# danihae/bio-image-unet

Measured on AMD Instinct MI355X. Metric: voxels/sec fwd+bwd, higher is better.
Workload: dtype bf16; 1 GPU; cfg4: UNet3D(in_channels=1, out_channels=1, n_filter=32) input (4, 1, 128, 128, 128) per GPU, train step = forward + reference loss + backward + Adam; parallelism=dp1

## Files before the change

### bio_image_unet_amd/_lib.py

```python
from __future__ import annotations

import ctypes as C
import os

import torch

_HERE = os.path.dirname(os.path.abspath(__file__))
LIB_PATH = os.environ.get("BIU_LIB_PATH") or os.path.join(_HERE, "libbiu_hip.so")

BIU_F32, BIU_BF16 = 0, 1
BN_MAX_PARTIALS = 1024


class BiuError(RuntimeError):
    pass


class biu_act(C.Structure):
    _fields_ = [("p", C.c_void_p), ("n", C.c_int32), ("d", C.c_int32), ("h", C.c_int32), ("w", C.c_int32),
                ("c", C.c_int32), ("pitch", C.c_int32)]


class biu_pack_job(C.Structure):
    _fields_ = [("w", C.c_void_p), ("packed", C.c_void_p), ("transposed", C.c_int32), ("kind", C.c_int32), ("cin", C.c_int32),
                ("cout", C.c_int32), ("kd", C.c_int32), ("kh", C.c_int32), ("kw", C.c_int32), ("reserved", C.c_int32)]


class biu_xform(C.Structure):
    _fields_ = [("scale", C.c_void_p), ("shift", C.c_void_p), ("slope", C.c_void_p)]


class biu_mo2d_term(C.Structure):
    _fields_ = [("kind", C.c_int32), ("nb", C.c_int32), ("partial_off", C.c_longlong), ("numel", C.c_longlong), ("pixels", C.c_longlong),
                ("p0", C.c_float), ("p1", C.c_float), ("p2", C.c_float), ("weight", C.c_float)]


class biu_aug_params(C.Structure):
    _fields_ = [("flags", C.c_uint32), ("rot_k", C.c_uint32), ("blur_k", C.c_uint32), ("index", C.c_uint32), ("m", C.c_double * 6),
                ("alpha", C.c_float), ("beta", C.c_float), ("noise_a", C.c_float), ("noise_b", C.c_float),
                ("angle", C.c_float), ("scale", C.c_float), ("dx", C.c_float), ("dy", C.c_float)]


class biu_augf_params(C.Structure):
    _fields_ = [("flags", C.c_uint32), ("rot_k", C.c_uint32), ("blur_k", C.c_uint32), ("index", C.c_uint32), ("m", C.c_double * 6),
                ("cos_t", C.c_float), ("sin_t", C.c_float), ("alpha", C.c_float), ("beta", C.c_float), ("shot_s", C.c_float),
                ("gauss_sigma", C.c_float), ("angle", C.c_float), ("scale", C.c_float), ("dx", C.c_float), ("dy", C.c_float)]


_P = C.c_void_p
_A = C.POINTER(biu_act)
_X = C.POINTER(biu_xform)
_I = C.c_int
_F = C.c_float
_D = C.c_double
_Z = C.c_size_t

SIGNATURES = {
    "biu_last_error": (C.c_char_p, []),
    "biu_version": (_I, []),
    "biu_set_fp32_products": (_I, [_I]),
    "biu_set_fp32_products_3d": (_I, [_I]),
    "biu_conv_packed_bytes": (_Z, [_I, _I, _I, _I, _I, _I, _I, _I]),
    "biu_conv_pack": (_I, [_I, _P, _I, _I, _I, _I, _I, _I, _P, _P]),
    "biu_pack_batch": (_I, [_P, _I, _I, _P]),
    "biu_conv_split_workspace": (_Z, [_I, _A, _A, _I, _I, _I, _I, _I]),
    "biu_conv_fwd": (_I, [_A, _X, _P, _P, _P, _I, _I, _I, _I, _A, _P, _Z, _I, _P]),
    "biu_conv_fwd_stats_floats": (_Z, [_A, _I]),
    "biu_conv_fwd_stats": (_I, [_A, _X, _P, _P, _P, _I, _I, _I, _I, _A, _P, _Z, C.POINTER(C.c_int), _P, _Z, _I, _P]),
    "biu_conv_bwd_data": (_I, [_A, _P, _P, _I, _I, _I, _I, _A, _I, _P, _Z, _I, _P]),
    "biu_bwd_data_bnred_floats": (_Z, [_A, _I, _I]),
    "biu_conv_bwd_data_bnred": (_I, [_A, _P, _P, _I, _I, _I, _I, _A, _A, _P, _P, _P, _P, _P, _P, _Z, C.POINTER(C.c_int), _P, _Z, _I, _P]),
    "biu_convt_bwd_data_bnred": (_I, [_A, _P, _P, _I, _A, _A, _P, _P, _P, _P, _P, _P, _Z, C.POINTER(C.c_int), _I, _P]),
    "biu_conv_bwd_weight_workspace": (_Z, [_I, _I, _I, _I, _I, _I]),
    "biu_conv_bwd_weight": (_I, [_A, _X, _A, _I, _I, _I, _I, _P, _P, _P, _Z, _I, _P]),
    "biu_conv_bwd_weight_bn": (_I, [_A, _X, _A, _A, _P, _P, _P, _P, _P, _P, _I, _I, _I, _I, _P, _P, _Z, _I, _P]),
    "biu_bn_stats": (_I, [_A, _P, C.POINTER(C.c_int), _I, _P]),
    "biu_bn_finalize": (_I, [_P, _I, _I, _D, _P, _P, _P, _P, _F, _F, _P, _P, _P, _P, _P]),
    "biu_bn_eval_affine": (_I, [_I, _P, _P, _P, _P, _F, _P, _P, _P]),
    "biu_xform_apply": (_I, [_A, _X, _A, _I, _P]),
    "biu_bn_bwd_reduce": (_I, [_A, _A, _P, _P, _P, _P, _P, _P, C.POINTER(C.c_int), _I, _P]),
    "biu_bn_bwd_finalize": (_I, [_P, _I, _I, _D, _P, _P, _P, _P, _P, _P, _P, _P, _P]),
    "biu_bn_bwd_finalize_eval": (_I, [_P, _I, _I, _P, _P, _P, _P, _P, _P, _P, _P]),
    "biu_bn_bwd_apply": (_I, [_A, _A, _P, _P, _P, _P, _P, _P, _A, _I, _P]),
    "biu_maxpool_fwd": (_I, [_A, _X, _A, _I, _P]),
    "biu_maxpool_bwd": (_I, [_A, _X, _A, _A, _I, _I, _P]),
    "biu_maxpool_bwd_bnred": (_I, [_A, _X, _A, _A, _I, _P, _P, _P, _Z, C.POINTER(C.c_int), _I, _P]),
    "biu_nearest_down_fwd": (_I, [_A, _X, _A, _I, _P]),
    "biu_nearest_down_bwd": (_I, [_A, _A, _I, _I, _P]),
    "biu_nearest_up_fwd": (_I, [_A, _X, _A, _I, _P]),
    "biu_upconv_ok": (_I, [_A, _A, _I]),
    "biu_upconv_packed_bytes": (_Z, [_I, _I, _I, _I]),
    "biu_upconv_pack": (_I, [_I, _P, _I, _I, _I, _P, _P]),
    "biu_upconv_bwd_data": (_I, [_A, _P, _A, _I, _I, _P]),
    "biu_upconv_bwd_weight_workspace": (_Z, [_I, _I, _I]),
    "biu_upconv_bwd_weight_bn": (_I, [_A, _X, _A, _A, _P, _P, _P, _P, _P, _P, _P, _P, _Z, _I, _P]),
    "biu_upconv_fwd_stats_floats": (_Z, [_A, _A]),
    "biu_upconv_fwd": (_I, [_A, _X, _P, _P, _A, _P, _Z, C.POINTER(C.c_int), _I, _P]),
    "biu_nearest_up_bwd": (_I, [_A, _A, _I, _I, _P]),
    "biu_bce_dice_blocks": (_I, [C.c_longlong]),
    "biu_bce_dice_fwd": (_I, [_P, _P, _I, C.c_longlong, _P, _P]),
    "biu_bce_dice_bwd": (_I, [_P, _P, _I, C.c_longlong, _P, _P, _I, _P]),
    "biu_pair_smooth_l1_blocks": (_I, [C.c_longlong]),
    "biu_pair_smooth_l1_fwd": (_I, [_P, _I, C.c_longlong, _P, _P]),
    "biu_pair_smooth_l1_bwd": (_I, [_P, _I, C.c_longlong, _P, _P, _I, _P]),
    "biu_seg_loss_finish": (_I, [_P, _I, _I, C.c_longlong, _P, _I, _F, _F, _F, _I, _F, _F, _F, _I, _F, _P, _P]),
    "biu_seg_loss_coef": (_I, [_P, _P, _I, C.c_longlong, _F, _F, _F, _I, _F, _F, _F, _I, _F, _P, _P, _P]),
    "biu_head_dlogits": (_I, [_P, _P, _P, _I, _I, _I, C.c_longlong, _P, _I, _I, _P]),
    "biu_mo2d_loss_blocks": (_I, [C.c_longlong]),
    "biu_mo2d_loss_fwd": (_I, [_I, _F, _F, _P, _I, _P, _I, _I, _I, _I, _P, _P]),
    "biu_mo2d_loss_finish": (_I, [_P, _I, _P, _P, _P]),
    "biu_mo2d_loss_coef": (_I, [_P, _I, _P, _P, _P, _P]),
    "biu_mo2d_loss_bwd": (_I, [_I, _F, _F, _P, _I, _P, _I, _I, _I, _I, _P, _P, _P]),
    "biu_trilinear_up_fwd": (_I, [_A, _X, _A, _I, _P]),
    "biu_trilinear_up_bwd": (_I, [_A, _A, _I, _I, _P]),
    "biu_bilinear_up_fwd": (_I, [_A, _X, _A, _I, _P]),
    "biu_bilinear_up_bwd": (_I, [_A, _A, _I, _I, _P]),
    "biu_xcorr_fwd": (_I, [_A, _X, _A, _X, _A, _I, _P]),
    "biu_xcorr_bwd": (_I, [_A, _X, _A, _X, _A, _A, _A, _I, _I, _P]),
    "biu_conv_cat_ok": (_I, [_A, _A, _A, _I, _I, _I, _I, _I]),
    "biu_conv_fwd_cat": (_I, [_A, _X, _A, _X, _P, _P, _P, _I, _I, _I, _I, _A, _P, _Z, C.POINTER(C.c_int), _P, _Z, _I, _P]),
    "biu_conv_bwd_data_cat": (_I, [_A, _P, _P, _I, _I, _I, _I, _A, _I, _A, _I, _P, _Z, _I, _P]),
    "biu_conv_bwd_weight_cat": (_I, [_A, _X, _A, _X, _A, _A, _P, _P, _P, _P, _P, _P, _I, _I, _I, _I, _P, _P, _Z, _I, _P]),
    "biu_convt_packed_bytes": (_Z, [_I, _I, _I, _I, _I]),
    "biu_convt_pack": (_I, [_I, _P, _I, _I, _I, _I, _P, _P]),
    "biu_foldt_ok": (_I, [_A, _A, _A, _I]),
    "biu_foldt_packed_bytes": (_Z, [_I, _I, _I, _I]),
    "biu_foldt_pack": (_I, [_P, _P, _P, _P, _I, _I, _I, _I, _I, _P, _P]),
    "biu_foldt_fwd_stats_floats": (_Z, [_A, _A]),
    "biu_foldt_fwd_form": (_I, [_A, _A, _A, _I]),
    "biu_foldt_fwd": (_I, [_A, _X, _A, _X, _P, _A, _P, _Z, C.POINTER(C.c_int), _I, _P]),
    "biu_foldt_bwd_data_bnred_floats": (_Z, [_A]),
    "biu_foldt_bwd_data": (_I, [_A, _P, _A, _I, _A, _I, _A, _P, _P, _P, _P, _P, _P, _Z, C.POINTER(C.c_int), _P, _Z, _I, _P]),
    "biu_foldt_bwd_weight_workspace": (_Z, [_I, _I, _I, _I]),
    "biu_foldt_bwd_weight_bn": (_I, [_A, _X, _A, _X, _A, _A, _P, _P, _P, _P, _P, _P, _P, _P, _P, _P, _I, _P, _P, _P, _P, _Z, _I, _P]),
    "biu_foldt_bwd_weight_bn_phase": (_I, [_A, _X, _A, _X, _A, _A, _P, _P, _P, _P, _P, _P, _P, _P, _P, _P, _I, _P, _P, _P, _P, _Z, _I, _I, _P]),
    "biu_convt_fwd": (_I, [_A, _X, _P, _P, _P, _I, _A, _I, _P]),
    "biu_convt_bwd_data": (_I, [_A, _P, _P, _I, _A, _I, _I, _P]),
    "biu_convt_bwd_weight_workspace": (_Z, [_I, _I, _I, _I]),
    "biu_convt_bwd_weight": (_I, [_A, _X, _A, _I, _P, _P, _P, _Z, _I, _P]),
    "biu_head_fwd": (_I, [_A, _X, _P, _P, _I, _I, _P, _P, _I, _P]),
    "biu_head_bwd_workspace": (_Z, [_I]),
    "biu_head_bwd": (_I, [_A, _X, _P, _I, _P, _A, _P, _P, _P, _Z, _I, _P]),
    "biu_head_bwd_bnred": (_I, [_A, _X, _P, _I, _P, _A, _P, _P, _P, _Z, _P, _P, _P, _Z, C.POINTER(C.c_int), _I, _P]),
    "biu_max_join_fwd": (_I, [_A, _X, _A, _X, _A, _I, _P]),
    "biu_max_join_bwd": (_I, [_A, _X, _A, _X, _A, _A, _A, _I, _I, _P]),
    "biu_act_add": (_I, [_A, _A, _I, _I, _P]),
    "biu_add_relu_fwd": (_I, [_A, _X, _A, _X, _A, _I, _P]),
    "biu_add_relu_bwd": (_I, [_A, _A, _A, _A, _I, _I, _P]),
    "biu_gate_fwd": (_I, [_A, _X, _A, _X, _A, _I, _P]),
    "biu_gate_bwd": (_I, [_A, _X, _A, _X, _A, _A, _I, _A, _I, _P]),
    "biu_from_nchw": (_I, [_P, _A, _I, _P]),
    "biu_from_nchw_u8": (_I, [_P, _F, _A, _I, _P]),
    "biu_u8_to_f32": (_I, [_P, _F, _P, C.c_longlong, _P]),
    "biu_quantize_u8": (_I, [_P, _F, _P, C.c_longlong, _P]),
    "biu_stitch_add": (_I, [_P, _I, _P, _I, _I, _I, _I, _P, _P, _I, _I, _I, _I, _I, _I, _I, _P]),
    "biu_stitch_finish": (_I, [_P, _P, _I, _I, C.c_longlong, _P, _I, _P]),
    "biu_to_nchw": (_I, [_A, _X, _P, _I, _P]),
    "biu_augment_u8": (_I, [_P, _P, _I, _I, _I, _I, _I, _P, _I, _I, C.c_ulonglong, C.c_uint, C.c_uint, _P]),
    "biu_augment_f32": (_I, [_P, _I, _P, _I, _I, _I, _I, _I, _P, _I, C.c_ulonglong, C.c_uint, C.c_uint, _P]),
    "biu_philox_u32": (_I, [_P, C.c_longlong, C.c_ulonglong, C.c_uint, C.c_uint, C.c_uint, C.c_uint, _P]),
    "biu_adam_step": (_I, [_I, _P, _P, _P, _P, _P, _F, _F, _F, _F, _I, _F, _P]),
    "biu_adam_set_hyper": (_I, [_P, _F, _F, _F, _F, _I, _F, _P]),
    "biu_adam_step_hyper": (_I, [_I, _P, _P, _P, _P, _P, _P, _P]),
    "biu_grad_clip_scratch_floats": (_Z, [_I]),
    "biu_grad_clip": (_I, [_I, _P, _P, _F, _P, _Z, _P, _P]),
}


def _load():
    if not os.path.exists(LIB_PATH):
        raise ImportError(
            f"{LIB_PATH} is missing: the HIP kernels are not built. Run `python -c 'import __graft_entry__ as g; "
            f"g.build()'` from the repository root (needs hipcc). There is no CPU fallback.")
    lib = C.CDLL(LIB_PATH)
    for name, (res, args) in SIGNATURES.items():
        fn = getattr(lib, name)
        fn.restype = res
        fn.argtypes = args
    return lib


class _Lib:

    def __init__(self, cdll):
        object.__setattr__(self, "_c", cdll)
        object.__setattr__(self, "prof", None)
        object.__setattr__(self, "watch", None)
# ... 33 lines not shown
```

### bio_image_unet_amd/csrc/biu_api.hip

```cpp
#include "biu_common.h"
#include "biu_internal.h"

#include <stdlib.h>
#include <string.h>

static const char* const kOffTokens[] = {
    "conv_fwd", "conv_dgrad", "conv_wgrad", "convt_fwd", "convt_dgrad", "convt_wgrad", "convt_all", "c1", "c1_mfma", "cat",
    "fused_stats", "wgrad_bn", "dgrad_bnred", "pool_pair", "pool_pipe", "pool_bnred", "head_bnred", "ksplit", "m16", "m16x2", "rr16",
    "wroll", "wroll16", "wroll2d", "upconv", "foldt", "foldall", "foldck8", "foldgemm", "croll", "froll", "prepack", "wsplitbn",
    "capturefork", "sidechain",
};
constexpr int kNumOffTokens = sizeof(kOffTokens) / sizeof(kOffTokens[0]);
static_assert(kNumOffTokens <= 64, "BiuEnv::off holds one bit per token");

static int off_index(const char* tok, size_t n) {
    for (int i = 0; i < kNumOffTokens; ++i)
        if (strlen(kOffTokens[i]) == n && strncmp(kOffTokens[i], tok, n) == 0) return i;
    return -1;
}
static void env_unknown(const char* var, const char* val, int n) {
    fprintf(stderr, "[biu] %s: unknown %s '%.*s' ignored\n", var, strcmp(var, "BIU_DISABLE") == 0 ? "token" : "value", n, val);
}
static bool parse_int(const char* s, int* v) {
    char* end = nullptr;
    const long r = strtol(s, &end, 10);
    if (end == s || *end) return false;
    *v = (int)r;
    return true;
}

const BiuEnv& biu_env() {
    static const BiuEnv env = [] {
        BiuEnv v{0, false, false, 0, 2, 0, 128};
        if (const char* p = getenv("BIU_DISABLE")) {
            while (true) {
                const size_t n = strcspn(p, ",");
                const int i = off_index(p, n);
                if (i >= 0) v.off |= 1ull << i;
                else if (n > 0) env_unknown("BIU_DISABLE", p, (int)n);
                if (!p[n]) break;
                p += n + 1;
            }
        }
        if (const char* e = getenv("BIU_ROLL"); e && *e) {
            if (strcmp(e, "always") == 0) v.roll_always = true;
            else env_unknown("BIU_ROLL", e, (int)strlen(e));
        }
        if (const char* e = getenv("BIU_FOLDT"); e && *e) {
            int n = 0;
            if (strcmp(e, "always") == 0) v.foldt_always = true;
            else if (strncmp(e, "cmax:", 5) == 0 && parse_int(e + 5, &n) && n > 0) v.foldt_cmax = n;
            else if (strcmp(e, "size") != 0) env_unknown("BIU_FOLDT", e, (int)strlen(e));
        }
        if (const char* e = getenv("BIU_FP32_PRODUCTS"); e && *e) {
            if (strcmp(e, "exact") == 0) v.fp32_products = 0;
            else if (strcmp(e, "bf16x3") == 0) v.fp32_products = 1;
            else if (strcmp(e, "bf16x6") != 0) env_unknown("BIU_FP32_PRODUCTS", e, (int)strlen(e));
        }
        if (const char* e = getenv("BIU_FP32_PRODUCTS_3D"); e && *e) {
            if (strcmp(e, "bf16x3") == 0) v.fp32_products_3d = 1;
            else if (strcmp(e, "bf16x6") == 0) v.fp32_products_3d = 2;
            else if (strcmp(e, "exact") != 0) env_unknown("BIU_FP32_PRODUCTS_3D", e, (int)strlen(e));
        }
        if (const char* e = getenv("BIU_FALL_MAXCA"); e && *e) {
            int n = 0;
            if (parse_int(e, &n)) v.fall_maxca = n;
            else env_unknown("BIU_FALL_MAXCA", e, (int)strlen(e));
        }
        return v;
    }();
    return env;
}

bool biu_off(const char* token) {
    const int i = off_index(token, strlen(token));
    return i >= 0 && ((biu_env().off >> i) & 1);
}

static void warn_slow_path(const char* op, const biu_act* x, const biu_act* y, int taps) {
    const double macs = (double)nvox(y) * x->c * y->c * taps;
    if (macs < 4e9) return;
    static int shown = 0;
    if (shown++ < 8)
        fprintf(stderr, "[biu] %s: %d->%d channels on %lld voxels takes the any-shape kernel (%.1f GMAC): expect it to be slow; "
                        "the MFMA path needs channel counts that are multiples of 8 (>= 16), dilation 1, 16-byte aligned slices "
                        "and samples under 4 GB\n", op, x->c, y->c, (long long)nvox(y), macs * 1e-9);
}

static bool conv_args_ok(const biu_act* x, const biu_act* y, int kd, int kh, int kw, int dil) {
    if (!valid_act(x) || !valid_act(y) || !same_space(x, y)) return false;
    if (!((kd == 1 || kd == 3) && kh == 3 && kw == 3) && !(kd == 1 && kh == 1 && kw == 1)) return false;
    return dil >= 1;
}
// ... 82 lines not shown
    warn_slow_path("conv_fwd", x, y, kd * kh * kw);
    return biu_conv_fwd_direct(x, xf, w, bias, kd, kh, kw, dilation, y, dtype, (hipStream_t)stream);
}

extern "C" int biu_conv_bwd_data(const biu_act* dy, const float* w, const void* packed, int kd, int kh, int kw,
                                 int dilation, const biu_act* dx, int accumulate, void* ws, size_t ws_bytes, int dtype, biu_stream stream) {
    BIU_REQUIRE(conv_args_ok(dy, dx, kd, kh, kw, dilation), BIU_ERR_SHAPE, "conv_bwd_data: dy/dx extents differ");
    BIU_REQUIRE(w, BIU_ERR_SHAPE, "conv_bwd_data: null weight");
    if (packed && !biu_off("conv_dgrad") && biu_mfma_conv_ok(dy, dx, kd, kh, kw, dilation, dtype))
        return biu_mfma_conv(dy, nullptr, packed, nullptr, kd, kh, kw, dx, accumulate, nullptr, dtype, (hipStream_t)stream, nullptr, nullptr, ws, ws_bytes);
    warn_slow_path("conv_bwd_data", dx, dy, kd * kh * kw);
    return biu_conv_bwd_data_direct(dy, w, kd, kh, kw, dilation, dx, accumulate, dtype, (hipStream_t)stream);
}

extern "C" size_t biu_bwd_data_bnred_floats(const biu_act* dx, int kd, int transposed) {
    size_t a = (size_t)BIU_BN_MAX_PARTIALS * dx->c * 2;
    size_t b = (size_t)(transposed ? biu_mfma_convt_dgrad_bricks(dx, kd) : biu_mfma_conv_bricks(dx, kd == 3 ? 3 : 1)) * dx->c * 2;
    return a > b ? a : b;
}
extern "C" int biu_conv_bwd_data_bnred(const biu_act* dy, const float* w, const void* packed, int kd, int kh, int kw, int dilation,
                                       const biu_act* dx, const biu_act* y_up, const float* scale, const float* shift,
                                       const float* slope, const float* mean, const float* invstd, float* partial,
                                       size_t partial_floats, int* nblk, void* ws, size_t ws_bytes, int dtype, biu_stream stream) {
    BIU_REQUIRE(conv_args_ok(dy, dx, kd, kh, kw, dilation) && valid_act(y_up) && same_space(y_up, dx) && y_up->c == dx->c, BIU_ERR_SHAPE,
                "conv_bwd_data_bnred: extents differ");
    BIU_REQUIRE(w && scale && shift && mean && invstd && partial && nblk, BIU_ERR_SHAPE, "conv_bwd_data_bnred: null pointer");
    const size_t es = dsize(dtype);
    const bool yok = ((uintptr_t)y_up->p % 16) == 0 && ((size_t)y_up->pitch * es) % 16 == 0;
    if (packed && yok && !biu_off("conv_dgrad") && !biu_off("dgrad_bnred") && biu_mfma_conv_ok(dy, dx, kd, kh, kw, dilation, dtype) &&
        !will_split(dy->c, dx, nullptr, kd, dtype, ws, ws_bytes)) {
        const int nb = biu_mfma_conv_stat_rows(dx, kd, dy, dtype, true);
        if ((size_t)nb * dx->c * 2 <= partial_floats) {
            BnRedFuse red{y_up, scale, shift, slope, mean, invstd};
            int rc = biu_mfma_conv(dy, nullptr, packed, nullptr, kd, kh, kw, dx, 0, partial, dtype, (hipStream_t)stream, &red);
            if (rc == BIU_OK) *nblk = nb;
            return rc;
        }
    }
    int rc = biu_conv_bwd_data(dy, w, packed, kd, kh, kw, dilation, dx, 0, ws, ws_bytes, dtype, stream);
    if (rc != BIU_OK) return rc;
    BIU_REQUIRE(partial_floats >= (size_t)BIU_BN_MAX_PARTIALS * dx->c * 2, BIU_ERR_WORKSPACE, "conv_bwd_data_bnred: partial buffer too small");
    return biu_bn_bwd_reduce(dx, y_up, scale, shift, slope, mean, invstd, partial, nblk, dtype, stream);
}
extern "C" int biu_convt_bwd_data_bnred(const biu_act* dy, const float* w, const void* packed, int kd, const biu_act* dx,
                                        const biu_act* y_up, const float* scale, const float* shift, const float* slope,
                                        const float* mean, const float* invstd, float* partial, size_t partial_floats, int* nblk,
                                        int dtype, biu_stream stream) {
    BIU_REQUIRE(valid_act(dx) && valid_act(dy) && w && biu_convt_shapes_ok(dx, dy, kd) && valid_act(y_up) && same_space(y_up, dx) &&
                    y_up->c == dx->c, BIU_ERR_SHAPE, "convt_bwd_data_bnred: extents differ");
    BIU_REQUIRE(scale && shift && mean && invstd && partial && nblk, BIU_ERR_SHAPE, "convt_bwd_data_bnred: null pointer");
    const size_t es = dsize(dtype);
    const bool yok = ((uintptr_t)y_up->p % 16) == 0 && ((size_t)y_up->pitch * es) % 16 == 0;
    if (packed && yok && !biu_off("convt_dgrad") && !biu_off("dgrad_bnred") && biu_mfma_convt_ok(1, dx, dy, kd, dtype) &&
        biu_convt_all_ok(dx, dy, kd, dtype)) {
        const int nb = biu_convt_all_dgrad_rows(dx, dy, kd);
        if ((size_t)nb * dx->c * 2 <= partial_floats) {
            BnRedFuse red{y_up, scale, shift, slope, mean, invstd};
            int rc = biu_convt_all_dgrad(dy, packed, kd, dx, 0, (hipStream_t)stream, partial, &red);
            if (rc == BIU_OK) *nblk = nb;
            return rc;
        }
    }
    if (packed && yok && !biu_off("convt_dgrad") && !biu_off("dgrad_bnred") && biu_mfma_convt_ok(1, dx, dy, kd, dtype)) {
        const int nb = biu_mfma_convt_dgrad_rows(dx, kd, dy->c, dtype);
        if ((size_t)nb * dx->c * 2 <= partial_floats) {
            BnRedFuse red{y_up, scale, shift, slope, mean, invstd};
            int rc = biu_mfma_convt_dgrad(dy, packed, kd, dx, 0, dtype, (hipStream_t)stream, partial, &red);
            if (rc == BIU_OK) *nblk = nb;
            return rc;
        }
    }
    int rc = biu_convt_bwd_data(dy, w, packed, kd, dx, 0, dtype, stream);
    if (rc != BIU_OK) return rc;
    BIU_REQUIRE(partial_floats >= (size_t)BIU_BN_MAX_PARTIALS * dx->c * 2, BIU_ERR_WORKSPACE, "convt_bwd_data_bnred: partial buffer too small");
    return biu_bn_bwd_reduce(dx, y_up, scale, shift, slope, mean, invstd, partial, nblk, dtype, stream);
}

extern "C" size_t biu_conv_bwd_weight_workspace(int cin, int cout, int kd, int kh, int kw, int dtype) {
    if (cin == 1 && kh == 3 && kw == 3) {
        const size_t a = biu_c1_wgrad_workspace(cout, kd), b = biu_c1m_wgrad_workspace(cout, kd);
        return a > b ? a : b;
    }
    return biu_mfma_wgrad_workspace(cin, cout, kd, kh, kw, dtype);
}

extern "C" int biu_conv_bwd_weight(const biu_act* x, const biu_xform* xf, const biu_act* dy, int kd, int kh, int kw,
                                   int dilation, float* dw, float* dbias, void* ws, size_t ws_bytes, int dtype,
                                   biu_stream stream) {
    BIU_REQUIRE(conv_args_ok(x, dy, kd, kh, kw, dilation), BIU_ERR_SHAPE, "conv_bwd_weight: x/dy extents differ");
    BIU_REQUIRE(dw, BIU_ERR_SHAPE, "conv_bwd_weight: null dw");
    if (!biu_off("c1") && biu_c1m_ok(x, dy, kd, kh, kw, dilation, dtype) && ws && ws_bytes >= biu_c1m_wgrad_workspace(dy->c, kd)) {
        int rc = biu_c1m_wgrad(x, xf, dy, nullptr, kd, dw, ws, ws_bytes, (hipStream_t)stream);
        if (rc == BIU_OK && dbias) rc = biu_chan_sum(dy, dbias, dtype, (hipStream_t)stream);
        return rc;
    }
    if (!biu_off("c1") && biu_c1_conv_ok(x, dy, kd, kh, kw, dilation, dtype) && ws && ws_bytes >= biu_c1_wgrad_workspace(dy->c, kd)) {
        int rc = biu_c1_conv_wgrad(x, xf, dy, kd, dw, ws, ws_bytes, dtype, (hipStream_t)stream);
        if (rc == BIU_OK && dbias) rc = biu_chan_sum(dy, dbias, dtype, (hipStream_t)stream);
        return rc;
    }
    if (!biu_off("conv_wgrad") && biu_mfma_wgrad_ok(x, dy, kd, kh, kw, dilation, dtype)) {
        BIU_REQUIRE(ws && ws_bytes >= biu_mfma_wgrad_workspace(x->c, dy->c, kd, kh, kw, dtype), BIU_ERR_WORKSPACE,
                    "conv_bwd_weight: workspace too small");
        return biu_mfma_wgrad(x, xf, dy, kd, kh, kw, dw, dbias, ws, ws_bytes, dtype, (hipStream_t)stream);
    }
    warn_slow_path("conv_bwd_weight", x, dy, kd * kh * kw);
    return biu_conv_bwd_weight_direct(x, xf, dy, kd, kh, kw, dilation, dw, dbias, dtype, (hipStream_t)stream);
}

extern "C" int biu_conv_bwd_weight_bn(const biu_act* x, const biu_xform* xf, const biu_act* da, const biu_act* y,
                                      const float* scale, const float* shift, const float* slope, const float* coefA,
                                      const float* coefB, const float* coefC, int kd, int kh, int kw, int dilation,
                                      float* dw, void* ws, size_t ws_bytes, int dtype, biu_stream stream) {
    BIU_REQUIRE(conv_args_ok(x, da, kd, kh, kw, dilation) && valid_act(y) && same_space(y, da) && y->c == da->c, BIU_ERR_SHAPE,
                "conv_bwd_weight_bn: extents differ");
    BIU_REQUIRE(dw && scale && shift && coefA && coefB && coefC, BIU_ERR_SHAPE, "conv_bwd_weight_bn: null pointer");
    const size_t es = dsize(dtype);
    const bool yok = ((uintptr_t)y->p % 16) == 0 && ((size_t)y->pitch * es) % 16 == 0 &&
                     (i64)y->d * y->h * y->w * y->pitch * (i64)es < (1LL << 32) - 65536;
    if (!biu_off("c1") && !biu_off("wgrad_bn") && yok && biu_c1m_ok(x, da, kd, kh, kw, dilation, dtype) && ws &&
        ws_bytes >= biu_c1m_wgrad_workspace(da->c, kd)) {
        BnBwdFuse bn{y, scale, shift, slope, coefA, coefB, coefC};
        return biu_c1m_wgrad(x, xf, da, &bn, kd, dw, ws, ws_bytes, (hipStream_t)stream);
    }
    if (!biu_off("conv_wgrad") && !biu_off("wgrad_bn") && yok && biu_mfma_wgrad_ok(x, da, kd, kh, kw, dilation, dtype)) {
        BIU_REQUIRE(ws && ws_bytes >= biu_mfma_wgrad_workspace(x->c, da->c, kd, kh, kw, dtype), BIU_ERR_WORKSPACE,
                    "conv_bwd_weight_bn: workspace too small");
        BnBwdFuse bn{y, scale, shift, slope, coefA, coefB, coefC};
        return biu_mfma_wgrad(x, xf, da, kd, kh, kw, dw, nullptr, ws, ws_bytes, dtype, (hipStream_t)stream, &bn);
    }
    int rc = biu_bn_bwd_apply(da, y, scale, shift, slope, coefA, coefB, coefC, da, dtype, stream);
    if (rc != BIU_OK) return rc;
    return biu_conv_bwd_weight(x, xf, da, kd, kh, kw, dilation, dw, nullptr, ws, ws_bytes, dtype, stream);
}

extern "C" int biu_conv_cat_ok(const biu_act* x0, const biu_act* x1, const biu_act* y, int kd, int kh, int kw, int dilation, int dtype) {
    if (!x0 || !x1 || !y || !valid_act(x0) || !valid_act(x1) || !valid_act(y) || !same_space(x0, y) || !same_space(x1, y)) return 0;
    if (biu_off("conv_fwd") || biu_off("conv_dgrad") || biu_off("conv_wgrad") || biu_off("cat")) return 0;
    return biu_mfma_conv_cat_ok(x0, x1, y, kd, kh, kw, dilation, dtype) ? 1 : 0;
}
extern "C" int biu_conv_fwd_cat(const biu_act* x0, const biu_xform* xf0, const biu_act* x1, const biu_xform* xf1, const float* w,
                                const void* packed, const float* bias, int kd, int kh, int kw, int dilation, const biu_act* y,
                                float* bn_partial, size_t bn_partial_floats, int* bn_nblk, void* ws, size_t ws_bytes, int dtype,
                                biu_stream stream) {
    BIU_REQUIRE(biu_conv_cat_ok(x0, x1, y, kd, kh, kw, dilation, dtype) && w && packed, BIU_ERR_UNSUPPORTED,
                "conv_fwd_cat: shapes not served by the two-source kernels (ask biu_conv_cat_ok)");
    ConvCat cat{x1, xf1, nullptr, 0};
    if (bn_partial && will_split(x0->c + x1->c, y, nullptr, kd, dtype, ws, ws_bytes)) {
        BIU_REQUIRE(bn_nblk, BIU_ERR_SHAPE, "conv_fwd_cat: null bn_nblk");
        int rc = biu_mfma_conv(x0, xf0, packed, bias, kd, kh, kw, y, 0, nullptr, dtype, (hipStream_t)stream, nullptr, &cat, ws, ws_bytes);
        if (rc != BIU_OK) return rc;
        BIU_REQUIRE(bn_partial_floats >= (size_t)BIU_BN_MAX_PARTIALS * y->c * 2, BIU_ERR_WORKSPACE, "conv_fwd_cat: partial buffer too small");
        return biu_bn_stats(y, bn_partial, bn_nblk, dtype, stream);
    }
    if (bn_partial) {
        BIU_REQUIRE(bn_nblk, BIU_ERR_SHAPE, "conv_fwd_cat: null bn_nblk");
        const int nb = dtype == BIU_F32 ? biu_mfma_conv_stat_rows(y, kd, x0, dtype, false, x0->c + x1->c) : biu_mfma_conv_stat_rows(y, kd);
        BIU_REQUIRE((size_t)nb * y->c * 2 <= bn_partial_floats, BIU_ERR_WORKSPACE, "conv_fwd_cat: partial buffer too small");
        int rc = biu_mfma_conv(x0, xf0, packed, bias, kd, kh, kw, y, 0, bn_partial, dtype, (hipStream_t)stream, nullptr, &cat);
        if (rc == BIU_OK) *bn_nblk = nb;
        return rc;
    }
    return biu_mfma_conv(x0, xf0, packed, bias, kd, kh, kw, y, 0, nullptr, dtype, (hipStream_t)stream, nullptr, &cat, ws, ws_bytes);
}
extern "C" int biu_conv_bwd_data_cat(const biu_act* dy, const float* w, const void* packed, int kd, int kh, int kw, int dilation,
                                     const biu_act* dx0, int accumulate0, const biu_act* dx1, int accumulate1, void* ws, size_t ws_bytes,
// ... 218 lines not shown
```

### bio_image_unet_amd/csrc/biu_conv_mfma.hip

```cpp
#include "biu_internal.h"
#include <type_traits>
#include <cstring>
#include <mutex>
#include <cstdlib>

typedef float floatx16 __attribute__((ext_vector_type(16)));
typedef float floatx4 __attribute__((ext_vector_type(4)));
typedef __bf16 bf16x8 __attribute__((ext_vector_type(8)));

template <typename T> struct Frag;
template <> struct Frag<bf16_t> {
    static constexpr int PE = 8;
    __device__ static __forceinline__ void mma(const uint4& a, const uint4& b, floatx16& c) {
        c = __builtin_amdgcn_mfma_f32_32x32x16_bf16(__builtin_bit_cast(bf16x8, a), __builtin_bit_cast(bf16x8, b), c, 0, 0, 0);
    }
    __device__ static __forceinline__ void unpack(const uint4& v, float* f) {
        const unsigned u[4] = {v.x, v.y, v.z, v.w};
#pragma unroll
        for (int i = 0; i < 4; ++i) {
            f[2 * i] = __uint_as_float(u[i] << 16);
            f[2 * i + 1] = __uint_as_float(u[i] & 0xffff0000u);
        }
    }
    __device__ static __forceinline__ uint4 pack(const float* f) {
// ... 2235 lines not shown
}
bool biu_mfma_foldt_worth(const biu_act* x_low, const biu_act* y) {
    const double vox = (double)y->n * y->d * y->h * y->w;
    return vox * 19.0 >= 12.0 * 648.0 * x_low->c;
}
size_t biu_mfma_foldt_packed_bytes(int cin_low, int cskip, int cout, int dtype) { return foldt_blob(cin_low, cskip, cout, dtype).total; }
int biu_mfma_foldt_pack(const float* w_conv, const float* b_conv, const float* w_t, const float* b_t, int cin_low, int cup, int cskip, int cout, int dtype,
                        void* packed, hipStream_t st) {
    const FoldtBlob b = foldt_blob(cin_low, cskip, cout, dtype);
    char* base = (char*)packed;
    float* wfold = (float*)(base + b.wfold);
    const int ccat = cup + cskip;
    if (cup <= cin_low && biu_fold_gemm_ok(cin_low, cup, cout)) {
        float* lay = (float*)(base + b.lay);
        int rc = biu_fold_gemm_layouts(w_conv, ccat, cup, cout, w_t, cin_low, lay, st);
        if (rc == BIU_OK) rc = biu_fold_gemm_compose(lay, cin_low, cup, cout, b_t, wfold, (float*)(base + b.wb), st);
        if (rc != BIU_OK) return rc;
    } else {
        hipLaunchKernelGGL(k_foldt_compose, dim3((cin_low + 31) / 32, (cout + 31) / 32, 64), dim3(256), 0, st, w_conv, ccat, 0, cup, cout, w_t, cin_low, wfold);
        hipLaunchKernelGGL(k_foldt_wb, dim3((27 * cout + 127) / 128), dim3(128), 0, st, w_conv, ccat, 0, cup, cout, b_t, (float*)(base + b.wb));
    }
    hipLaunchKernelGGL(k_foldt_fix, dim3((27 * cout + 127) / 128), dim3(128), 0, st, (const float*)(base + b.wb), cout, b_conv, (float*)(base + b.fix),
                       (float*)(base + b.bias));
    BIU_CHECK_LAUNCH("foldt_compose");
    int rc = biu_mfma_upconv_pack(0, nullptr, cin_low, cout, dtype, base + b.fwd, st, wfold);
    if (rc == BIU_OK) rc = biu_mfma_upconv_pack(1, nullptr, cin_low, cout, dtype, base + b.dg, st, wfold);
    if (rc == BIU_OK) rc = mfma_pack_strided(0, w_conv + (size_t)cup * 27, ccat, cskip, cout, 3, 3, 3, dtype, base + b.sfwd, st);
    if (rc == BIU_OK) rc = mfma_pack_strided(1, w_conv + (size_t)cup * 27, ccat, cskip, cout, 3, 3, 3, dtype, base + b.sdg, st);
    return rc;
}
static bool foldt_roll_ok(const biu_act* x_low, const biu_act* skip, const biu_act* y, int dtype) {
    return !biu_off("froll") && skip && biu_fold_roll_ok(x_low, y, dtype) && biu_conv_roll_ok(skip, y, dtype, false, 1, false);
}
int biu_mfma_foldt_form(const biu_act* x_low, const biu_act* skip, const biu_act* y, int dtype) { return foldt_roll_ok(x_low, skip, y, dtype) ? 1 : 0; }
int biu_mfma_foldt_stat_rows(const biu_act* x_low, const biu_act* y, const biu_act* skip, int dtype) {
    if (skip && foldt_roll_ok(x_low, skip, y, dtype)) return biu_conv_roll_rows(skip, y, dtype);
    return biu_mfma_upconv_stat_rows(x_low, y);
}
int biu_mfma_foldt_fwd(const biu_act* x_low, const biu_xform* xf_low, const biu_act* skip, const biu_xform* xf_skip, const void* packed, const biu_act* y,
                       float* bn_partial, int dtype, hipStream_t st) {
    const FoldtBlob b = foldt_blob(x_low->c, skip->c, y->c, dtype);
    const char* base = (const char*)packed;
    if (foldt_roll_ok(x_low, skip, y, dtype)) {
        int rc = biu_fold_roll(x_low, xf_low, base + b.fwd, (const float*)(base + b.bias), (const float*)(base + b.fix), y, st);
        if (rc != BIU_OK) return rc;
        return biu_mfma_conv(skip, xf_skip, base + b.sfwd, nullptr, 3, 3, 3, y, 1, bn_partial, dtype, st, nullptr, nullptr, nullptr, 0);
    }
    int rc = biu_mfma_conv(skip, xf_skip, base + b.sfwd, (const float*)(base + b.bias), 3, 3, 3, y, 0, nullptr, dtype, st, nullptr, nullptr, nullptr, 0);
    if (rc != BIU_OK) return rc;
    const ShellDims sh = shell_dims(y->n, y->d, y->h, y->w);
    BIU_DISPATCH_DTYPE(dtype, hipLaunchKernelGGL(k_foldt_border_fix<T>, dim3(2048), dim3(256), 0, st, (char*)y->p,
                                                 sh, y->c, y->pitch, (const float*)(base + b.fix)));
    BIU_CHECK_LAUNCH("foldt_border_fix");
    return biu_mfma_upconv_fwd(x_low, xf_low, base + b.fwd, nullptr, y, bn_partial, dtype, st, 1);
}

typedef __bf16 bf16x4 __attribute__((ext_vector_type(4)));

struct WgradArgs {
    const char* pa;
    const char* pb;
    float* ws;
    const float* as_; const float* ab_; const float* al_;
    const float* bs_; const float* bb_; const float* bl_;
    int apitch, bpitch;
    int N, CA, CB;
    int GD, GH, GW;
    int BD, BH, BW;
    int nbd, nbh, nbw, nbricks;
    int njt;
    int jt_begin, jt_count;
    int write_back;
    unsigned long long* diag;
    const char* pb1; int bpitch1; int bsplit;
    const float* bs1_; const float* bb1_; const float* bl1_;
    int bricks_per_block;
    const char* py;
    int ypitch;
    const float* bn_scale; const float* bn_shift; const float* bn_slope;
    const float* bn_cA; const float* bn_cB; const float* bn_cC;
    float* dbias_out;
    int fold_par;
    size_t fold_slice_f;
};

template <typename T, int PE>
__device__ __forceinline__ uint4 apply_xf16(uint4 v, const float* sc, const float* sh, const float* sl) {
    using F = Frag<T>;
    float f[PE];
    F::unpack(v, f);
    lrelu_affine<PE>(f, sc, sh, sl);
    return F::pack(f);
}


constexpr bool wgrad_tab_in_lds(size_t tile_bytes, int pieces) { return tile_bytes + (size_t)pieces * 512 * 4 <= 150 * 1024; }

template <typename T, int KD, int KHW, int S, int TD, int TH, int TW, int KSPLIT, int NI, bool RR16 = false, bool FALL = false>
__global__ __launch_bounds__(512, 2) void k_wgrad_pipe(WgradArgs a) {
    using F = Frag<T>;
    constexpr int NTHR = 512, NWAVE = 8;
    constexpr int PE = F::PE;
    constexpr int CT = 32;
    constexpr int PPV = CT / PE;
    constexpr int XP = SplitOf<T>::parts;
    constexpr bool X3 = XP > 0;
    constexpr bool BFM = sizeof(T) == 2 || X3;
    constexpr int LES = BFM ? 2 : 4;
    constexpr int NPL = X3 ? XP : 1;
    constexpr int CTA = CT * NI, PPVA = CTA / PE, RSA = CTA * LES;
    constexpr int PD = (KD == 3) ? 1 : 0;
    constexpr int PHW = (KHW == 3) ? 1 : 0;
    constexpr bool FOLD = (KD == 2 && KHW == 2 && S == 1);
    constexpr int SD = (KD == 1) ? 1 : S;
    static_assert(!FALL || (FOLD && KSPLIT == 8 && NI == 1 && sizeof(T) == 2), "the all-parity form: bf16 fold, one wave per parity class");
    constexpr int HD = (TD - 1) * SD + (FALL ? 3 : KD), HH = (TH - 1) * S + (FALL ? 3 : KHW), HW = (TW - 1) * S + (FALL ? 3 : KHW);
    constexpr int HV = HD * HH * HW;
    constexpr int BVR = TD * TH * TW;
    constexpr int BV = FALL ? 8 * BVR : BVR;
    constexpr int TAPS = KD * KHW * KHW;
    constexpr int WPQ = NWAVE / KSPLIT;
    constexpr int IPW = (TAPS + WPQ - 1) / WPQ;
    static_assert(NWAVE % KSPLIT == 0, "K split must divide the wave count");
    constexpr int RS = CT * LES;
    constexpr int NA = (BV * PPVA + NTHR - 1) / NTHR;
    constexpr int NB = (HV * PPV + NTHR - 1) / NTHR;
    constexpr int KUNIT = BFM ? 16 : 2;
    constexpr int NKG = BV / KUNIT;
    static_assert(TW % 16 == 0 && NKG % KSPLIT == 0, "brick / split mismatch");

    extern __shared__ __attribute__((aligned(16))) uint4 lds[];
    char* at = (char*)lds;
    char* bt = at + NPL * BV * RSA;
    float* lxf = (float*)(bt + NPL * HV * RS);
    constexpr int LA = 0, LB = 3 * CTA, LBN = 3 * CTA + 3 * CT;
    constexpr bool TAB_LDS = wgrad_tab_in_lds((size_t)NPL * ((size_t)HV * RS + (size_t)BV * RSA), NA + NB);
    unsigned* ltab = (unsigned*)(lxf + LBN + 6 * CTA);
    unsigned xa_[TAB_LDS ? 1 : NA], xb_[TAB_LDS ? 1 : NB];

    const int tid = threadIdx.x, lane = tid & 63;
    const int wave = __builtin_amdgcn_readfirstlane(tid >> 6);
    const int it = blockIdx.y / a.jt_count, jt = a.jt_begin + blockIdx.y % a.jt_count;
    const size_t esz = sizeof(T);
    const int piece = tid % PPV, pieceA = tid % PPVA;
    const int ac0 = it * CTA + pieceA * PE, bc0 = jt * CT + piece * PE;
    const bool apiece_ok = ac0 < a.CA, bpiece_ok = bc0 < a.CB;
    const bool b_src1 = a.pb1 && jt * CT >= a.bsplit;
    const char* pb_ = b_src1 ? a.pb1 : a.pb;
    const int bpitch_ = b_src1 ? a.bpitch1 : a.bpitch;
    const int bc_local = bc0 - (b_src1 ? a.bsplit : 0);
    const float* bs_ = b_src1 ? a.bs1_ : a.bs_;
    const float* bb_ = b_src1 ? a.bb1_ : a.bb_;
    const float* bl_ = b_src1 ? a.bl1_ : a.bl_;
    const bool a_xf = a.as_ != nullptr, b_xf = bs_ != nullptr;
    const bool bn_fused = !FALL && a.py != nullptr;
    if (tid < CTA && bn_fused) {
        const int ca = it * CTA + tid;
        const bool ok = ca < a.CA;
        lxf[LBN + 0 * CTA + tid] = ok ? a.bn_scale[ca] : 1.f;
        lxf[LBN + 1 * CTA + tid] = ok ? a.bn_shift[ca] : 0.f;
        lxf[LBN + 2 * CTA + tid] = (ok && a.bn_slope) ? a.bn_slope[ca] : 1.f;
        lxf[LBN + 3 * CTA + tid] = ok ? a.bn_cA[ca] : 0.f;
        lxf[LBN + 4 * CTA + tid] = ok ? a.bn_cB[ca] : 0.f;
        lxf[LBN + 5 * CTA + tid] = ok ? a.bn_cC[ca] : 0.f;
    }
    if (tid < CTA) {
        const int ca = it * CTA + tid;
// ... 457 lines not shown
                if constexpr (HAS_X) fxx[0] = rd(xbase, RS);
#pragma unroll
                for (int j = 0; j < 3; ++j) ring[j] = rd(bbase + j * HW * RS, RS);
#pragma unroll
                for (int g = 0; g < NG; ++g) {
#pragma unroll
                    for (int j = pf_lo(g, NA, NG); j < pf_lo(g + 1, NA, NG); ++j) issue_a(j);
#pragma unroll
                    for (int j = pf_lo(g, NB, NG); j < pf_lo(g + 1, NB, NG); ++j) issue_b(j);
#pragma unroll
                    for (int kk = 0; kk < KPG; ++kk) {
                        const int r = g * KPG + kk, lh = r % TH;
                        const int r1 = r + 1, ld1 = r1 / TH, lh1 = r1 % TH;
                        if (r1 < NROW) {
                            faa[r1 & 1] = rd(abase + r1 * 16 * RSA, RSA);
                            if constexpr (HAS_X) fxx[r1 & 1] = rd(xbase + ((ld1 * HH + lh1) * HW) * RS, RS);
                            if (lh1 != 0) ring[(lh1 + 2) & 3] = rd(bbase + ((ld1 * HH + lh1 + 2) * HW) * RS, RS);
                        }
#pragma unroll
                        for (int tb = 0; tb < 3; ++tb) acc[tb][0] = __builtin_amdgcn_mfma_f32_32x32x16_bf16(faa[r & 1], ring[(lh + tb) & 3], acc[tb][0], 0, 0, 0);
                        if constexpr (HAS_X) acc[3][0] = __builtin_amdgcn_mfma_f32_32x32x16_bf16(faa[r & 1], fxx[r & 1], acc[3][0], 0, 0, 0);
                        if (r1 < NROW && lh1 == 0) {
#pragma unroll
                            for (int j = 0; j < 3; ++j) ring[j] = rd(bbase + ((ld1 * HH + j) * HW) * RS, RS);
                        }
                    }
                    __builtin_amdgcn_sched_barrier(0);
                }
            };
            if constexpr (RR) {
                using Full = std::integral_constant<int, TD * TH>;
                using Half = std::integral_constant<int, TD * TH / 2>;
                if (rr16) {
                    const char* bb = bt + u16_boff + b_lane16 + (u16_r0 / TH) * (HH * HW * RS);
                    const char* ab = at + a_lane + u16_r0 * 16 * RSA;
                    if (u16_half) rr_phase(std::false_type{}, Half{}, bb, ab); else rr_phase(std::false_type{}, Full{}, bb, ab);
                } else if (wave < 3) {
                    rr_phase(std::true_type{}, Full{}, bt + tapoff[0] + b_lane, at + a_lane);
                } else {
                    rr_phase(std::false_type{}, Full{}, bt + tapoff[0] + b_lane, at + a_lane);
                }
            } else if constexpr (TWO_PHASES) {
                if (!last_tap_live) mfma_phase(std::integral_constant<int, (IPW > 1 ? IPW - 1 : 1)>{});
                else mfma_phase(std::integral_constant<int, IPW>{});
            } else {
                mfma_phase(std::integral_constant<int, IPW>{});
            }
            WSTAMP(1);
#ifdef BIU_DIAG
            dsum_[7] += 1;
            if (!have_next && wdiag && tid == 0) {
                for (int q_ = 0; q_ < 8; ++q_) atomicAdd(wdiag + q_, dsum_[q_]);
                atomicAdd(wdiag + 8, __builtin_readcyclecounter() - t0c_);
                atomicAdd(wdiag + 9, __builtin_amdgcn_s_memrealtime() - t0r_);
            }
#endif
            if (!have_next) break;
            __syncthreads();
            WSTAMP(2);
            commit();
            WSTAMP(3);
            __syncthreads();
            WSTAMP(4);
            brick = nbrick;
            ++kround;
        }
    }

    if constexpr (DBIAS) {
        if (a.dbias_out != nullptr && it == 0) {
            __syncthreads();
            float* lsum = (float*)bt;
            if (tid < CT) lsum[tid] = 0.f;
            __syncthreads();
            if (dbias_on) {
#pragma unroll
                for (int e = 0; e < PE; ++e) atomicAdd(&lsum[piece * PE + e], bsum[e]);
            }
            __syncthreads();
            if (tid < CT && jt * CT + tid < a.CB) atomicAdd(a.dbias_out + jt * CT + tid, lsum[tid]);
        }
    }
    const int hf = lane >> 5;
    if (rr16) {
        const int ch = lane & 15, up = (lane >> 4) & 1;
        const int kd = (u16_unit < 3) ? up : 2, kw = (u16_unit < 3) ? u16_unit : u16_unit - 3;
        if (!(up && u16_unit >= 3)) {
#pragma unroll
            for (int tb = 0; tb < 3; ++tb) {
                const int tap = (kd * 3 + tb) * 3 + kw;
#pragma unroll
                for (int e = 0; e < 16; ++e) {
                    const int ii = it * CTA + (e & 3) + 8 * (e >> 2) + 4 * hf;
                    if (ii < a.CA) atomicAdd(a.ws + ((size_t)tap * a.CA + ii) * a.CB + ch, acc[tb][0][e]);
                }
            }
        }
        return;
    }
    const int jj = jt * CT + (lane & 31);
    float* wsp = a.ws + (FALL ? (size_t)wave * a.fold_slice_f : (size_t)0);
    if (jj < a.CB) {
#pragma unroll
        for (int t2 = 0; t2 < IPW; ++t2) {
            const int tap = tapid[t2];
            if (tap < TAPS) {
#pragma unroll
                for (int ni = 0; ni < NI; ++ni)
#pragma unroll
                    for (int e = 0; e < 16; ++e) {
                        const int ii = it * CTA + ni * CT + (e & 3) + 8 * (e >> 2) + 4 * hf;
                        if (ii < a.CA) atomicAdd(wsp + ((size_t)tap * a.CA + ii) * a.CB + jj, acc[t2][ni][e]);
                    }
            }
        }
    }
}

typedef unsigned v4u_t __attribute__((ext_vector_type(4)));
__device__ __forceinline__ void bload_lds16(unsigned voff, v4u_t rsrc, unsigned lds_base_uniform) {
    unsigned keep;
    asm volatile("s_mov_b32 %0, m0\n\ts_mov_b32 m0, %3\n\ts_nop 0\n\tbuffer_load_dwordx4 %1, %2, 0 offen lds\n\ts_mov_b32 m0, %0"
                 : "=&s"(keep)
                 : "v"(voff), "s"(rsrc), "s"(lds_base_uniform)
                 : "memory");
}
__device__ __forceinline__ v4u_t raw_rsrc(const void* base, unsigned bytes) {
    const unsigned long long pa = (unsigned long long)base;
    v4u_t r;
    r[0] = __builtin_amdgcn_readfirstlane((unsigned)pa);
    r[1] = __builtin_amdgcn_readfirstlane((unsigned)(pa >> 32) & 0xffffu);
    r[2] = __builtin_amdgcn_readfirstlane(bytes);
    r[3] = 0x00020000u;
    return r;
}

#ifndef BIU_WROLL_ABL
#define BIU_WROLL_ABL 0
#endif
#ifndef BIU_DIAG_WAVE
#define BIU_DIAG_WAVE 0
#endif
constexpr int WR_TD = 2, WR_TH = 8, WR_TW = 16;
constexpr int WR_HH = WR_TH + 2, WR_HW = WR_TW + 2, WR_PL = WR_HH * WR_HW;
constexpr int WR_RS = 64;
constexpr int WR_PLB = WR_PL * WR_RS;
constexpr int WR_NBI = 24;
constexpr int WR_PAIRB = WR_NBI * 1024;
constexpr int WR_NPAIR = 4;
constexpr int WR_BV = WR_TD * WR_TH * WR_TW;
constexpr int WR_AB = WR_BV * WR_RS;
constexpr int WR_NAI = WR_AB / 1024;
constexpr int WR_NABUF = 3;
constexpr size_t WR_LDS = (size_t)WR_NPAIR * WR_PAIRB + WR_NABUF * WR_AB + 9 * 32 * sizeof(float);

__device__ __forceinline__ unsigned opaque_s(unsigned x) { asm volatile("" : "+s"(x)); return x; }
template <int N> __device__ __forceinline__ void wait_vmcnt() { asm volatile("s_waitcnt vmcnt(%0)" ::"n"(N) : "memory"); }

template <bool BNF, bool K2D, bool A16 = false>
__global__ __launch_bounds__(512, 2) void k_wgrad_roll(WgradArgs a) {
    static_assert(!(K2D && A16), "the 16-channel plain operand form exists for volumes only");
    using T = bf16_t;
    using F = Frag<T>;
    constexpr int TD = WR_TD, TH = WR_TH, TW = WR_TW, HW = WR_HW, PL = WR_PL, RS = WR_RS, PLB = WR_PLB, PAIRB = WR_PAIRB;
    constexpr int CT = 32, PE = 8, TAPS = K2D ? 9 : 27, IPW = K2D ? 3 : 4, NROW = TD * TH;
    constexpr int NBK = WR_NBI / 8, NAK = A16 ? 1 : WR_NAI / 8;
// ... 296 lines not shown
            const int r1 = r + 1, ld1 = r1 / TH, lh1 = r1 % TH;
            if (r1 < NROW && !(BIU_WROLL_ABL & 2)) {
                faa[r1 & 1] = rd(ab + r1 * 16 * RS);
                if constexpr (HAS_X) fxx[r1 & 1] = rd((ld1 ? x1 : x0) + lh1 * HW * RS);
                if (lh1 != 0) ring[(lh1 + 2) & 3] = rd((ld1 ? b1 : b0) + (lh1 + 2) * HW * RS);
            }
#pragma unroll
            for (int tb = 0; tb < 3; ++tb) acc[tb] = __builtin_amdgcn_mfma_f32_32x32x16_bf16(faa[r & 1], ring[(lh + tb) & 3], acc[tb], 0, 0, 0);
            if constexpr (HAS_X) acc[3] = __builtin_amdgcn_mfma_f32_32x32x16_bf16(faa[r & 1], fxx[r & 1], acc[3], 0, 0, 0);
            if (r1 < NROW && lh1 == 0 && !(BIU_WROLL_ABL & 2)) {
#pragma unroll
                for (int j = 0; j < 3; ++j) ring[j] = rd((ld1 ? b1 : b0) + j * HW * RS);
            }
            if (r % 3 == 1 && r / 3 < NBK + NAK) issue(r / 3);
            if ((r & 1) == 1 || r % 3 == 1) __builtin_amdgcn_sched_barrier(0);
        }
    };

    const int G = gridDim.x;
    const int ncols = a.N * a.nbh * a.nbw, nsteps = (a.GD + TD - 1) / TD;
    auto column_of = [&](int k) -> int {
        if ((G & 7) == 0) return k * G + (int)(blockIdx.x & 7) * (G >> 3) + (int)(blockIdx.x >> 3);
        return k * G + (int)blockIdx.x;
    };
#ifdef BIU_DIAG
    unsigned long long* wdiag = a.diag;
    unsigned long long tprev_ = __builtin_readcyclecounter();
    unsigned long long dsum_[8] = {0, 0, 0, 0, 0, 0, 0, 0};
    const unsigned long long t0c_ = tprev_, t0r_ = __builtin_amdgcn_s_memrealtime();
#define RSTAMP(k_) do { if (wdiag && (tid & 63) == 0 && (tid >> 6) == (BIU_DIAG_WAVE)) { unsigned long long now_ = __builtin_readcyclecounter(); dsum_[k_] += now_ - tprev_; tprev_ = now_; } } while (0)
#else
#define RSTAMP(k_) do { } while (0)
#endif
    auto step = [&](Slot& mine, Slot& other, int s) __attribute__((always_inline)) {
        const bool f2 = (s + 2 < nsteps) && !((BIU_WROLL_ABL & 1) && s >= 1);
        const bool f1 = (s + 1 < nsteps) && !((BIU_WROLL_ABL & 1) && s >= 2);
        RSTAMP(0);
        const FetchCtx fc = fetch_ctx((s + 3) & 3, 2 * s + 5, (s + 2) % 3, 2 * s + 4);
        RSTAMP(1);
        auto issue = [&](int i) __attribute__((always_inline)) { if (f2) fetch_piece(mine, fc, i); };
        if (has_x) mfma_step(std::true_type{}, s & 3, s % 3, issue); else mfma_step(std::false_type{}, s & 3, s % 3, issue);
        __builtin_amdgcn_sched_barrier(0);
        RSTAMP(2);
        if (f1) {
            wait_older(f2);
            RSTAMP(3);
            finish(other, (s + 2) & 3, (s + 1) % 3, 2 * s + 2, true);
        }
        RSTAMP(4);
        __syncthreads();
        RSTAMP(5);
#ifdef BIU_DIAG
        dsum_[7] += 1;
#endif
    };
    __syncthreads();
    for (int kc = 0;; ++kc) {
        const int col = column_of(kc);
        if (col >= ncols) break;
        set_column(col);
        fetch_all(sl0, fetch_ctx(0, -1, 0, 0), false);
        wait_vmcnt<0>();
        finish(sl0, 0, 0, 0, false);
        fetch_all(sl0, fetch_ctx(1, 1, 0, 0), true);
        if (nsteps > 1) fetch_all(sl1, fetch_ctx(2, 3, 1, 2), true);
        wait_vmcnt<0>();
        finish(sl0, 1, 0, 0, true);
        __syncthreads();
        for (int s = 0; s < nsteps; s += 2) {
            step(sl0, sl1, s);
            if (s + 1 < nsteps) step(sl1, sl0, s + 1);
        }
    }

#ifdef BIU_DIAG
    if (wdiag && (tid & 63) == 0 && (tid >> 6) == (BIU_DIAG_WAVE)) {
        for (int q_ = 0; q_ < 8; ++q_) atomicAdd(wdiag + q_, dsum_[q_]);
        atomicAdd(wdiag + 8, __builtin_readcyclecounter() - t0c_);
        atomicAdd(wdiag + 9, __builtin_amdgcn_s_memrealtime() - t0r_);
    }
#endif
    const int hf = lane >> 5;
    const int jj = jt * CT + (lane & 31);
    if constexpr (A16) {
        const int uj = wave & 3;
        if (jj < a.CB) {
#pragma unroll
            for (int u = 0; u < 2; ++u) {
                if (u == 1 && !has_x) break;
                const int kw = u ? 2 : (wave >> 2);
#pragma unroll
                for (int tb = 0; tb < 3; ++tb)
#pragma unroll
                    for (int e = 0; e < 16; ++e) {
                        const int kd = uj - (e >> 3), ii = (e & 3) + 8 * ((e >> 2) & 1) + 4 * hf;
                        if (kd >= 0 && kd <= 2 && ii < a.CA) atomicAdd(a.ws + ((size_t)((kd * 3 + tb) * 3 + kw) * a.CA + ii) * a.CB + jj, acc[u * 3 + tb][e]);
                    }
            }
        }
        return;
    }
    if (jj < a.CB) {
#pragma unroll
        for (int t2 = 0; t2 < IPW; ++t2) {
            const int tap = tapid[t2];
            if (tap < TAPS) {
#pragma unroll
                for (int e = 0; e < 16; ++e) {
                    const int ii = it * CT + (e & 3) + 8 * (e >> 2) + 4 * hf;
                    if (ii < a.CA) atomicAdd(a.ws + ((size_t)tap * a.CA + ii) * a.CB + jj, acc[t2][e]);
                }
            }
        }
    }
}

static bool wroll_fits(const WgradArgs& a) {
    const int ncols = a.N * ((a.GH + WR_TH - 1) / WR_TH) * ((a.GW + WR_TW - 1) / WR_TW);
    return a.GD >= 8 && ncols >= 8;
}
static bool wroll2d_fits(const WgradArgs& a, i64 bytesA, i64 bytesB, i64 bytesY) {
    const int ncols = ((a.GH + WR_TH - 1) / WR_TH) * ((a.GW + WR_TW - 1) / WR_TW);
    return a.N >= 8 && ncols >= 8 && a.CA * a.CB > 1024 && bytesA < BIU_MAX_SAMPLE_BYTES && bytesB < BIU_MAX_SAMPLE_BYTES && bytesY < BIU_MAX_SAMPLE_BYTES;
}

static int launch_wgrad_roll(WgradArgs a, hipStream_t st, bool k2d = false) {
    if (k2d) { a.GD = a.BD = a.N; a.N = 1; }
    const bool a16 = !k2d && a.CA == 16 && !biu_off("wroll16");
    a.nbd = 1;
    a.nbh = (a.GH + WR_TH - 1) / WR_TH;
    a.nbw = (a.GW + WR_TW - 1) / WR_TW;
    const int ncols = a.N * a.nbh * a.nbw;
    a.nbricks = ncols;
    const int nit = (a.CA + 31) / 32;
    a.njt = (a.CB + 31) / 32;
    a.bricks_per_block = 0;
#ifdef BIU_DIAG
    a.diag = biu_diag_buffer;
#else
    a.diag = nullptr;
#endif
    static bool attr_set = false;
    if (!attr_set) {
        if (hipFuncSetAttribute((const void*)k_wgrad_roll<false, false>, hipFuncAttributeMaxDynamicSharedMemorySize, (int)WR_LDS) != hipSuccess ||
            hipFuncSetAttribute((const void*)k_wgrad_roll<true, false>, hipFuncAttributeMaxDynamicSharedMemorySize, (int)WR_LDS) != hipSuccess ||
            hipFuncSetAttribute((const void*)k_wgrad_roll<false, true>, hipFuncAttributeMaxDynamicSharedMemorySize, (int)WR_LDS) != hipSuccess ||
            hipFuncSetAttribute((const void*)k_wgrad_roll<true, true>, hipFuncAttributeMaxDynamicSharedMemorySize, (int)WR_LDS) != hipSuccess ||
            hipFuncSetAttribute((const void*)k_wgrad_roll<false, false, true>, hipFuncAttributeMaxDynamicSharedMemorySize, (int)WR_LDS) != hipSuccess ||
            hipFuncSetAttribute((const void*)k_wgrad_roll<true, false, true>, hipFuncAttributeMaxDynamicSharedMemorySize, (int)WR_LDS) != hipSuccess)
            return biu_fail(BIU_ERR_LAUNCH, "wgrad_roll: cannot reserve %zu bytes of LDS", WR_LDS);
        attr_set = true;
    }
    auto launch = [&](int jt_begin, int jt_count, int write_back, bool with_bn) {
        WgradArgs b = a;
        if (!with_bn) b.py = nullptr;
        b.jt_begin = jt_begin; b.jt_count = jt_count; b.write_back = write_back;
        const int pairs = nit * jt_count;
        int g = num_cus() / pairs;
        if (g >= 16) g = grid_per_column(num_cus(), pairs);
        if (g < 1) g = 1;
        if (g > ncols) g = ncols;
        if (k2d) {
            if (with_bn) hipLaunchKernelGGL((k_wgrad_roll<true, true>), dim3(g, pairs), dim3(512), WR_LDS, st, b);
            else hipLaunchKernelGGL((k_wgrad_roll<false, true>), dim3(g, pairs), dim3(512), WR_LDS, st, b);
        } else if (a16) {
            if (with_bn) hipLaunchKernelGGL((k_wgrad_roll<true, false, true>), dim3(g, pairs), dim3(512), WR_LDS, st, b);
            else hipLaunchKernelGGL((k_wgrad_roll<false, false, true>), dim3(g, pairs), dim3(512), WR_LDS, st, b);
        } else {
            if (with_bn) hipLaunchKernelGGL((k_wgrad_roll<true, false>), dim3(g, pairs), dim3(512), WR_LDS, st, b);
            else hipLaunchKernelGGL((k_wgrad_roll<false, false>), dim3(g, pairs), dim3(512), WR_LDS, st, b);
        }
    };
    if (a.py && a.njt > 1) {
        launch(0, 1, 1, true);
        BIU_CHECK_LAUNCH("wgrad_roll");
        launch(1, a.njt - 1, 0, false);
    } else {
        launch(0, a.njt, a.py ? 1 : 0, a.py != nullptr);
    }
    BIU_CHECK_LAUNCH("wgrad_roll");
    return BIU_OK;
}

__global__ void k_wgrad_finalize(const float* __restrict__ ws, int rows, int cols, int taps, float* __restrict__ dw, int ld_cols = 0, int c_off = 0) {
    const size_t total = (size_t)rows * cols * taps;
    for (size_t i = (size_t)blockIdx.x * blockDim.x + threadIdx.x; i < total; i += (size_t)gridDim.x * blockDim.x) {
        const int tap = (int)(i % taps);
        const size_t r = i / taps;
        const int c = (int)(r % cols);
        const int rr = (int)(r / cols);
        const size_t o = ld_cols > 0 ? ((size_t)rr * ld_cols + c_off + c) * taps + tap : i;
        dw[o] = ws[((size_t)tap * rows + rr) * cols + c];
    }
}

__global__ void k_zero_f32(float* __restrict__ p, size_t n, float* __restrict__ q, int nq) {
    for (size_t i = (size_t)blockIdx.x * blockDim.x + threadIdx.x; i < n; i += (size_t)gridDim.x * blockDim.x) p[i] = 0.f;
    if (q && blockIdx.x == 0)
        for (int i = threadIdx.x; i < nq; i += blockDim.x) q[i] = 0.f;
}
static int zero_ws(void* ws, size_t bytes, float* extra, int nextra, hipStream_t st) {
    const size_t n = bytes / sizeof(float);
    hipLaunchKernelGGL(k_zero_f32, dim3(grid_for((i64)n, 256, 1024)), dim3(256), 0, st, (float*)ws, n, extra, nextra);
    if (hipGetLastError() != hipSuccess) return biu_fail(BIU_ERR_LAUNCH, "wgrad: zero-fill launch failed");
    return BIU_OK;
}

static bool wgrad_chan_ok(int cin, int cout) { return cin >= 16 && cin % 8 == 0 && cout >= 16 && cout % 8 == 0; }

static size_t wgrad_acc_bytes(int cin, int cout, int taps) { return (((size_t)cin * cout * taps * sizeof(float)) + 255) & ~(size_t)255; }

size_t biu_mfma_wgrad_workspace(int cin, int cout, int kd, int kh, int kw, int dtype) {
    if (!wgrad_chan_ok(cin, cout)) return 0;
    const size_t red = biu_chan_sum_workspace(cout);
    if (kh == 3 && kw == 3 && (kd == 1 || kd == 3)) return wgrad_acc_bytes(cin, cout, kd * 9) + red;
    if (kh == 2 && kw == 2 && (kd == 1 || kd == 2)) return wgrad_acc_bytes(cin, cout, kd * 4) + red;
    return 0;
}

static bool wgrad_ptrs_ok(const biu_act* x, const biu_act* dy, int dtype) {
    const size_t es = dsize(dtype);
    if ((uintptr_t)x->p % 16 || (uintptr_t)dy->p % 16 || ((size_t)x->pitch * es) % 16 || ((size_t)dy->pitch * es) % 16) return false;
    if (sample_bytes(x, es) >= BIU_MAX_SAMPLE_BYTES || sample_bytes(dy, es) >= BIU_MAX_SAMPLE_BYTES) return false;
    const i64 plane_x = (i64)x->h * x->w, plane_y = (i64)dy->h * dy->w;
    return 10 * (plane_x > plane_y ? plane_x : plane_y) < (1LL << 24);
}

bool biu_mfma_wgrad_ok(const biu_act* x, const biu_act* dy, int kd, int kh, int kw, int dilation, int dtype) {
    if (dilation != 1 || kh != 3 || kw != 3 || (kd != 1 && kd != 3)) return false;
    if (!wgrad_chan_ok(x->c, dy->c) || !wgrad_ptrs_ok(x, dy, dtype)) return false;
    if (kd == 1 && x->d != 1) return false;
    return true;
}

bool biu_mfma_convt_wgrad_ok(const biu_act* x, const biu_act* dy, int kd, int dtype) {
    return (kd == 1 || kd == 2) && wgrad_chan_ok(x->c, dy->c) && wgrad_ptrs_ok(x, dy, dtype);
}

template <typename T, int KD, int KHW, int S, int TD, int TH, int TW, int KSPLIT, int NI = 1, bool RR16 = false, bool FALL = false>
static int launch_wgrad(WgradArgs a, hipStream_t st) {
    constexpr int SD = (KD == 1) ? 1 : S;
    constexpr int HV = ((TD - 1) * SD + (FALL ? 3 : KD)) * ((TH - 1) * S + (FALL ? 3 : KHW)) * ((TW - 1) * S + (FALL ? 3 : KHW));
    constexpr int BV = (FALL ? 8 : 1) * TD * TH * TW;
    constexpr int PPV_ = 32 / (16 / (int)sizeof(T));
    constexpr int NA_ = (BV * PPV_ * NI + 511) / 512, NB_ = (HV * PPV_ + 511) / 512;
    const size_t tile_bytes = (size_t)(HV + BV * NI) * 32 * (SplitOf<T>::parts ? 2 * SplitOf<T>::parts : sizeof(T));
    const size_t lds_bytes = tile_bytes + (3 + 9 * NI) * 32 * sizeof(float) + (wgrad_tab_in_lds(tile_bytes, NA_ + NB_) ? (size_t)(NA_ + NB_) * 512 * sizeof(unsigned) : 0);
    a.nbd = (a.GD + TD - 1) / TD;
    a.nbh = (a.GH + TH - 1) / TH;
    a.nbw = (a.GW + TW - 1) / TW;
    a.nbricks = a.N * a.nbd * a.nbh * a.nbw;
    const int nit = (a.CA + 32 * NI - 1) / (32 * NI);
    a.njt = (a.CB + 31) / 32;
    a.bricks_per_block = 0;
    auto kern = k_wgrad_pipe<T, KD, KHW, S, TD, TH, TW, KSPLIT, NI, RR16, FALL>;
    static bool attr_set = false;
    if (!attr_set) {
        if (hipFuncSetAttribute((const void*)kern, hipFuncAttributeMaxDynamicSharedMemorySize, (int)lds_bytes) != hipSuccess)
            return biu_fail(BIU_ERR_LAUNCH, "wgrad_pipe: cannot reserve %zu bytes of LDS", lds_bytes);
        attr_set = true;
    }
    auto launch = [&](int jt_begin, int jt_count, int write_back, bool with_bn) {
        WgradArgs b = a;
#ifdef BIU_DIAG
        b.diag = biu_diag_buffer;
#else
        b.diag = nullptr;
#endif
        if (!with_bn) b.py = nullptr;
        b.jt_begin = jt_begin; b.jt_count = jt_count; b.write_back = write_back;
        const int pairs = nit * jt_count;
        int g = num_cus() / pairs;
        if (g >= 16) g = grid_per_column(num_cus(), pairs);
        if (g < 1) g = 1;
        if (g > b.nbricks) g = b.nbricks;
        hipLaunchKernelGGL(kern, dim3(g, pairs), dim3(512), lds_bytes, st, b);
    };
    if (a.py && a.njt > 1) {
        launch(0, 1, 1, true);
        BIU_CHECK_LAUNCH("wgrad_pipe");
        launch(1, a.njt - 1, 0, false);
    } else {
        launch(0, a.njt, a.py ? 1 : 0, a.py != nullptr);
    }
    BIU_CHECK_LAUNCH("wgrad_pipe");
    return BIU_OK;
}

static int wgrad_xf(const biu_xform* xf, const float** s, const float** b, const float** l) {
    const bool has = xf && (xf->scale || xf->shift || xf->slope);
    if (has) BIU_REQUIRE(xf->scale && xf->shift && xf->slope, BIU_ERR_UNSUPPORTED, "wgrad_mfma: partial biu_xform");
    *s = has ? xf->scale : nullptr;
    *b = has ? xf->shift : nullptr;
    *l = has ? xf->slope : nullptr;
    return BIU_OK;
}

int biu_mfma_wgrad(const biu_act* x, const biu_xform* xf, const biu_act* dy, int kd, int kh, int kw, float* dw, float* dbias,
                   void* ws, size_t ws_bytes, int dtype, hipStream_t st, const BnBwdFuse* bn, const biu_act* x1, const biu_xform* xf1,
                   int dw_ld_cols, int dw_c_off) {
    WgradArgs a;
    int rc_ = BIU_OK;
    if (bn && !biu_off("wsplitbn") && dtype == BIU_BF16 && kd == 3 && x->c + (x1 ? x1->c : 0) > 32 && nvox(dy) <= 4 * 32 * 32 * 32) {
        rc_ = biu_bn_bwd_apply(dy, bn->y, bn->scale, bn->shift, bn->slope, bn->cA, bn->cB, bn->cC, dy, dtype, (biu_stream)st);
        if (rc_ != BIU_OK) return rc_;
        bn = nullptr;
    }
    if (bn) {
        a.py = (const char*)bn->y->p; a.ypitch = bn->y->pitch;
        a.bn_scale = bn->scale; a.bn_shift = bn->shift; a.bn_slope = bn->slope;
        a.bn_cA = bn->cA; a.bn_cB = bn->cB; a.bn_cC = bn->cC;
    } else {
        a.py = nullptr; a.ypitch = 0;
        a.bn_scale = a.bn_shift = a.bn_slope = a.bn_cA = a.bn_cB = a.bn_cC = nullptr;
    }
    a.pa = (const char*)dy->p;  a.apitch = dy->pitch;  a.CA = dy->c;
    a.pb = (const char*)x->p;   a.bpitch = x->pitch;   a.CB = x->c;
    a.dbias_out = nullptr;
    a.fold_par = -1;
    a.pb1 = nullptr; a.bpitch1 = 0; a.bsplit = 0; a.bs1_ = a.bb1_ = a.bl1_ = nullptr;
    if (x1) {
        a.pb1 = (const char*)x1->p; a.bpitch1 = x1->pitch; a.bsplit = x->c; a.CB = x->c + x1->c;
        rc_ = wgrad_xf(xf1, &a.bs1_, &a.bb1_, &a.bl1_);
        if (rc_) return rc_;
    }
    a.ws = (float*)ws;
    a.as_ = a.ab_ = a.al_ = nullptr;
    int rc = wgrad_xf(xf, &a.bs_, &a.bb_, &a.bl_);
    if (rc) return rc;
    a.N = x->n;
    a.GD = a.BD = x->d; a.GH = a.BH = x->h; a.GW = a.BW = x->w;
    const int taps = kd * 9;
    const size_t need = wgrad_acc_bytes(a.CA, a.CB, taps);
    BIU_REQUIRE(ws_bytes >= need + (dbias ? biu_chan_sum_workspace(dy->c) : 0), BIU_ERR_WORKSPACE, "wgrad_mfma: workspace %zu too small", ws_bytes);
    if (int zr = zero_ws(ws, need, nullptr, 0, st)) return zr;
    if (dtype == BIU_BF16 && kd == 3 && a.CB == 16 && !x1 && !biu_off("rr16")) rc = launch_wgrad<bf16_t, 3, 3, 1, 4, 8, 16, 1, 1, true>(a, st);
    else if (dtype == BIU_BF16 && kd == 3 && !biu_off("wroll") && wroll_fits(a)) rc = launch_wgrad_roll(a, st);
    else if (dtype == BIU_BF16 && kd == 1 && !biu_off("wroll") && !biu_off("wroll2d") &&
             wroll2d_fits(a, (i64)nvox(dy) * dy->pitch * 2, (i64)nvox(x) * x->pitch * 2 > (x1 ? (i64)nvox(x1) * x1->pitch * 2 : 0) ? (i64)nvox(x) * x->pitch * 2 : (i64)nvox(x1) * x1->pitch * 2,
                          bn ? (i64)nvox(bn->y) * bn->y->pitch * 2 : 0))
        rc = launch_wgrad_roll(a, st, true);
    else if (dtype == BIU_BF16) rc = (kd == 3) ? launch_wgrad<bf16_t, 3, 3, 1, 4, 8, 16, 1>(a, st) : launch_wgrad<bf16_t, 1, 3, 1, 1, 16, 32, 4>(a, st);
    else if (kd == 1 && x3_mode_of(kd, dtype) == 2) rc = launch_wgrad<f32x6_t, 1, 3, 1, 1, 16, 16, 4>(a, st);
    else if (kd == 1 && x3_mode_of(kd, dtype) == 1) rc = launch_wgrad<f32x3_t, 1, 3, 1, 1, 16, 16, 4>(a, st);
    else if (kd == 3 && x3_mode_of(kd, dtype) == 2) rc = launch_wgrad<f32x6_t, 3, 3, 1, 2, 4, 16, 1>(a, st);
    else if (kd == 3 && x3_mode_of(kd, dtype) == 1) rc = launch_wgrad<f32x3_t, 3, 3, 1, 2, 4, 16, 1>(a, st);
    else rc = (kd == 3) ? launch_wgrad<float, 3, 3, 1, 4, 4, 16, 1>(a, st) : launch_wgrad<float, 1, 3, 1, 1, 16, 16, 4>(a, st);
    if (rc != BIU_OK) return rc;
    hipLaunchKernelGGL(k_wgrad_finalize, dim3(grid_for((i64)a.CA * a.CB * taps, 256, 2048)), dim3(256), 0, st, (const float*)ws,
                       a.CA, a.CB, taps, dw, dw_ld_cols, dw_c_off);
    BIU_CHECK_LAUNCH("wgrad_finalize");
    if (dbias) return biu_chan_sum_vec(dy, dbias, (char*)ws + need, dtype, st);
    return BIU_OK;
}

__global__ void k_upconv_wgrad_unfold(const float* __restrict__ ws, size_t slice_f, int cout, int cin, float* __restrict__ dw) {
    const size_t total = (size_t)cout * cin * 27;
    for (size_t idx = (size_t)blockIdx.x * blockDim.x + threadIdx.x; idx < total; idx += (size_t)gridDim.x * blockDim.x) {
        const int k = (int)(idx % 27);
        const size_t r = idx / 27;
        const int ci = (int)(r % cin), co = (int)(r / cin);
        const int kk[3] = {k / 9, (k / 3) % 3, k % 3};
        float sum = 0.f;
        for (int p = 0; p < 8; ++p) {
            int t = 0;
#pragma unroll
            for (int ax = 0; ax < 3; ++ax) {
                const int pa = (p >> (2 - ax)) & 1;
                const int ta = pa == 0 ? (kk[ax] >= 1 ? 1 : 0) : (kk[ax] == 2 ? 1 : 0);
                t |= ta << (2 - ax);
            }
            sum += ws[(size_t)p * slice_f + ((size_t)t * cout + co) * cin + ci];
        }
        dw[idx] = sum;
    }
}
size_t biu_mfma_upconv_wgrad_workspace(int cin, int cout, int dtype) {
    if ((dtype != BIU_BF16 && dtype != BIU_F32) || !wgrad_chan_ok(cin, cout)) return 0;
    return 8 * wgrad_acc_bytes(cout, cin, 8);
}
int biu_mfma_upconv_wgrad(const biu_act* x, const biu_xform* xf, const biu_act* dy, float* dw, void* ws, size_t ws_bytes, int dtype,
                          hipStream_t st, const BnBwdFuse* bn) {
    WgradArgs a;
    if (bn) {
        a.py = (const char*)bn->y->p; a.ypitch = bn->y->pitch;
        a.bn_scale = bn->scale; a.bn_shift = bn->shift; a.bn_slope = bn->slope;
        a.bn_cA = bn->cA; a.bn_cB = bn->cB; a.bn_cC = bn->cC;
    } else {
        a.py = nullptr; a.ypitch = 0;
        a.bn_scale = a.bn_shift = a.bn_slope = a.bn_cA = a.bn_cB = a.bn_cC = nullptr;
    }
    a.pa = (const char*)dy->p;  a.apitch = dy->pitch;  a.CA = dy->c;
    a.pb = (const char*)x->p;   a.bpitch = x->pitch;   a.CB = x->c;
    a.dbias_out = nullptr;
    a.pb1 = nullptr; a.bpitch1 = 0; a.bsplit = 0; a.bs1_ = a.bb1_ = a.bl1_ = nullptr;
    a.as_ = a.ab_ = a.al_ = nullptr;
    int rc = wgrad_xf(xf, &a.bs_, &a.bb_, &a.bl_);
    if (rc) return rc;
    a.N = x->n;
    a.GD = a.BD = x->d; a.GH = a.BH = x->h; a.GW = a.BW = x->w;
    const size_t slice = wgrad_acc_bytes(a.CA, a.CB, 8);
    BIU_REQUIRE(ws_bytes >= 8 * slice, BIU_ERR_WORKSPACE, "upconv_wgrad: workspace %zu too small (need %zu)", ws_bytes, 8 * slice);
    if (int zr = zero_ws(ws, 8 * slice, nullptr, 0, st)) return zr;
    a.fold_slice_f = slice / sizeof(float);
    if (dtype == BIU_BF16 && a.CA <= biu_env().fall_maxca && bn == nullptr && !biu_off("foldall")) {
        a.ws = (float*)ws;
        a.fold_par = 8;
        rc = launch_wgrad<bf16_t, 2, 2, 1, 2, 4, 16, 8, 1, false, true>(a, st);
        if (rc != BIU_OK) return rc;
    } else
    for (int p = 0; p < 8; ++p) {
        a.ws = (float*)((char*)ws + (size_t)p * slice);
        a.fold_par = p;
        if (x3_mode_of(2, dtype) == 2) rc = launch_wgrad<f32x6_t, 2, 2, 1, 4, 4, 16, 1>(a, st);
        else if (x3_mode_of(2, dtype) == 1) rc = launch_wgrad<f32x3_t, 2, 2, 1, 4, 4, 16, 1>(a, st);
        else if (a.CA > 32) rc = dtype == BIU_BF16 ? launch_wgrad<bf16_t, 2, 2, 1, 4, 8, 16, 1, 2>(a, st) : launch_wgrad<float, 2, 2, 1, 4, 4, 16, 1, 2>(a, st);
        else rc = dtype == BIU_BF16 ? launch_wgrad<bf16_t, 2, 2, 1, 4, 8, 16, 1>(a, st) : launch_wgrad<float, 2, 2, 1, 4, 4, 16, 1>(a, st);
        if (rc != BIU_OK) return rc;
    }
    if (!dw) return BIU_OK;
    hipLaunchKernelGGL(k_upconv_wgrad_unfold, dim3(grid_for((i64)a.CA * a.CB * 27, 256, 2048)), dim3(256), 0, st, (const float*)ws, slice / sizeof(float),
                       a.CA, a.CB, dw);
    BIU_CHECK_LAUNCH("upconv_wgrad_unfold");
    return BIU_OK;
}

int biu_mfma_foldt_dgrad(const biu_act* dy, const void* packed, const biu_act* dx_low, int acc_low, const biu_act* dskip, int acc_skip, int dtype,
                         hipStream_t st, float* bn_partial_low, const BnRedFuse* red_low, void* ws, size_t ws_bytes) {
    const FoldtBlob b = foldt_blob(dx_low->c, dskip->c, dy->c, dtype);
    const char* base = (const char*)packed;
    int rc = biu_mfma_conv(dy, nullptr, base + b.sdg, nullptr, 3, 3, 3, dskip, acc_skip, nullptr, dtype, st, nullptr, nullptr, ws, ws_bytes);
    if (rc != BIU_OK) return rc;
    return biu_mfma_upconv_dgrad(dy, base + b.dg, dx_low, acc_low, dtype, st, bn_partial_low, red_low);
}
constexpr int FOLDT_SUM_BLOCKS = 1024;
inline size_t foldt_sum_lds(int c) { return (size_t)27 * (c > 256 ? c : 256) * sizeof(float); }
template <typename T>
__global__ __launch_bounds__(256) void k_foldt_border_sums(const char* __restrict__ dy, ShellDims sd, int c, int pitch, float* __restrict__ partial) {
    extern __shared__ float tab[];
    const int lanes_c = c < 256 ? c : 256, slots = 256 / lanes_c;
    for (int i = threadIdx.x; i < slots * 27 * c; i += 256) tab[i] = 0.f;
    __syncthreads();
    const int cc0 = (int)threadIdx.x % lanes_c, slot = (int)threadIdx.x / lanes_c;
    const long nsv = sd.nA + sd.nB + sd.nC;
    const long stride = (long)gridDim.x * slots;
    if (slot < slots) {
        float* mine = tab + (size_t)slot * 27 * c;
        for (long v = (long)blockIdx.x * slots + slot; v < nsv; v += 4 * stride) {
            const T* p[4]; float* r[4]; bool ok[4];
#pragma unroll
            for (int u = 0; u < 4; ++u) {
                const long vv = v + u * stride;
                ok[u] = vv < nsv;
                long vox = 0; int st = 0;
                if (ok[u]) shell_voxel(sd, vv, vox, st);
                p[u] = (const T*)dy + (size_t)vox * pitch;
                r[u] = mine + st * c;
            }
            for (int cc = cc0; cc < c; cc += lanes_c) {
                float val[4];
#pragma unroll
                for (int u = 0; u < 4; ++u) val[u] = ok[u] ? (float)p[u][cc] : 0.f;
#pragma unroll
                for (int u = 0; u < 4; ++u) if (ok[u]) r[u][cc] += val[u];
            }
        }
    }
    __syncthreads();
    for (int i = threadIdx.x; i < 27 * c; i += 256) {
        float t = 0.f;
        for (int sl = 0; sl < slots; ++sl) t += tab[(size_t)sl * 27 * c + i];
        partial[(size_t)blockIdx.x * 27 * c + i] = t;
    }
}
constexpr int FOLDT_RED_SPLIT = 8;
__global__ __launch_bounds__(256) void k_foldt_reduce_tables(const float* __restrict__ partial, int nblocks, int cout, float* __restrict__ R) {
    __shared__ float red[256];
    const int s_ = (int)blockIdx.x, per = (nblocks + (int)gridDim.y - 1) / (int)gridDim.y;
    const int b0 = (int)blockIdx.y * per, b1 = b0 + per < nblocks ? b0 + per : nblocks;
    for (int c0 = 0; c0 < cout; c0 += 32) {
        const int co = c0 + (int)(threadIdx.x & 31), part = (int)(threadIdx.x >> 5);
        float s4[4] = {0.f, 0.f, 0.f, 0.f};
        if (co < cout) {
            int b = b0 + part;
            for (; b + 24 < b1; b += 32)
#pragma unroll
                for (int u = 0; u < 4; ++u) s4[u] += partial[((size_t)(b + 8 * u) * 27 + s_) * cout + co];
// ... 19 lines not shown
            for (int s_ = 0; s_ < 27; ++s_) {
                const float v = R[((size_t)sp * 27 + s_) * cout + co];
                sum -= (s_ != 13 && tap_outside(k, s_)) ? v : 0.f;
            }
        }
    red[threadIdx.x] = sum;
    __syncthreads();
    if (threadIdx.x < 32 && co < cout) {
        float t = 0.f;
        for (int pp = 0; pp < 8; ++pp) t += red[pp * 32 + threadIdx.x];
        Sk[k * cout + co] = t;
    }
}
__global__ __launch_bounds__(256) void k_foldt_chain_wconv(const float* __restrict__ G, size_t slice_f, const float* __restrict__ wt, int cin_low, int cup, int cout,
                                                           int ccat, float* __restrict__ dwc, const float* __restrict__ bt, const float* __restrict__ Sk) {
    __shared__ long offA[8], offB[8];
    const int k = (int)blockIdx.z;
    if (threadIdx.x < 8) {
        int t, q;
        foldt_tq((int)threadIdx.x, k, t, q);
        offA[threadIdx.x] = (long)threadIdx.x * (long)slice_f + (long)t * cout * cin_low;
        offB[threadIdx.x] = q;
    }
    __syncthreads();
    const int m0 = (int)blockIdx.y * 32, n0 = (int)blockIdx.x * 32;
    float acc[2][2] = {{0.f, 0.f}, {0.f, 0.f}};
    small_gemm_tile(8, cout, cup, cin_low, m0, n0, SgView{G, cin_low, 1}, offA, SgView{wt, (long)cup * 8, 8}, offB, acc);
    const int ty = threadIdx.x >> 4, tx = threadIdx.x & 15;
#pragma unroll
    for (int i = 0; i < 2; ++i)
#pragma unroll
        for (int j = 0; j < 2; ++j) {
            const int co = m0 + 2 * ty + i, c = n0 + 2 * tx + j;
            if (co < cout && c < cup) dwc[((size_t)co * ccat + c) * 27 + k] = bt ? fmaf(bt[c], Sk[k * cout + co], acc[i][j]) : acc[i][j];
        }
}
__global__ __launch_bounds__(256) void k_foldt_chain_wt(const float* __restrict__ G, size_t slice_f, const float* __restrict__ wc, int cin_low, int cup, int cout,
                                                        int ccat, float* __restrict__ dwt) {
    __shared__ long offA[27], offB[27];
    const int q = (int)blockIdx.z;
    if (threadIdx.x < 27) {
        const int k = (int)threadIdx.x, kk[3] = {k / 9, (k / 3) % 3, k % 3};
        int p = 0, t = 0;
#pragma unroll
        for (int ax = 0; ax < 3; ++ax) {
            const int qa = (q >> (2 - ax)) & 1, pa = (qa + kk[ax] + 1) & 1;
            const int ta = pa == 0 ? (kk[ax] >= 1 ? 1 : 0) : (kk[ax] == 2 ? 1 : 0);
            p |= pa << (2 - ax); t |= ta << (2 - ax);
        }
        offA[k] = (long)p * (long)slice_f + (long)t * cout * cin_low;
        offB[k] = k;
    }
    __syncthreads();
    const int m0 = (int)blockIdx.y * 32, n0 = (int)blockIdx.x * 32;
    float acc[2][2] = {{0.f, 0.f}, {0.f, 0.f}};
    small_gemm_tile(27, cin_low, cup, cout, m0, n0, SgView{G, 1, cin_low}, offA, SgView{wc, (long)ccat * 27, 27}, offB, acc);
    const int ty = threadIdx.x >> 4, tx = threadIdx.x & 15;
#pragma unroll
    for (int i = 0; i < 2; ++i)
#pragma unroll
        for (int j = 0; j < 2; ++j) {
            const int ci = m0 + 2 * ty + i, c = n0 + 2 * tx + j;
            if (ci < cin_low && c < cup) dwt[((size_t)ci * cup + c) * 8 + q] = acc[i][j];
        }
}
__global__ __launch_bounds__(256) void k_foldt_chain_bt(const float* __restrict__ Sk, const float* __restrict__ wc, int cup, int cout, int ccat, float* __restrict__ dbt) {
    __shared__ float red[256];
    const int c = (int)blockIdx.x;
    float sum = 0.f;
    for (int i = threadIdx.x; i < cout * 27; i += 256) {
        const int co = i / 27, k = i % 27;
        sum = fmaf(wc[((size_t)co * ccat + c) * 27 + k], Sk[k * cout + co], sum);
    }
    red[threadIdx.x] = sum;
    __syncthreads();
    for (int st = 128; st > 0; st >>= 1) {
        if ((int)threadIdx.x < st) red[threadIdx.x] += red[threadIdx.x + st];
        __syncthreads();
    }
    if (threadIdx.x == 0) dbt[c] = red[0];
}
size_t biu_mfma_foldt_wgrad_workspace(int cin_low, int cskip, int cout, int dtype) {
    if (!wgrad_chan_ok(cin_low, cout) || !wgrad_chan_ok(cskip, cout)) return 0;
    const size_t g = 8 * wgrad_acc_bytes(cout, cin_low, 8), sk = biu_mfma_wgrad_workspace(cskip, cout, 3, 3, 3, dtype);
    return (g > sk ? g : sk) + al256((size_t)FOLDT_SUM_BLOCKS * 27 * cout * sizeof(float)) + al256((size_t)(1 + FOLDT_RED_SPLIT) * 27 * cout * sizeof(float)) +
           al256(biu_fold_gemm_layout_floats(cin_low, cin_low, cout) * sizeof(float));
}
int biu_mfma_foldt_wgrad(const biu_act* x_low, const biu_xform* xf_low, const biu_act* skip, const biu_xform* xf_skip, const biu_act* da, const BnBwdFuse* bn,
                         const float* dy_sum, const float* w_conv, const float* w_t, const float* b_t, int cup, float* dw_conv, float* dw_t, float* db_t, void* ws, size_t ws_bytes,
                         int dtype, hipStream_t st, int phases) {
    const int cin_low = x_low->c, cskip = skip->c, cout = da->c, ccat = cup + cskip;
    const size_t need = biu_mfma_foldt_wgrad_workspace(cin_low, cskip, cout, dtype);
    BIU_REQUIRE(need > 0 && ws_bytes >= need, BIU_ERR_WORKSPACE, "foldt_wgrad: workspace %zu too small (need %zu)", ws_bytes, need);
    const size_t pbytes = al256((size_t)FOLDT_SUM_BLOCKS * 27 * cout * sizeof(float)), sbytes = al256((size_t)(1 + FOLDT_RED_SPLIT) * 27 * cout * sizeof(float));
    const size_t lbytes = al256(biu_fold_gemm_layout_floats(cin_low, cin_low, cout) * sizeof(float));
    const size_t main_bytes = need - pbytes - sbytes - lbytes;
    float* R = (float*)((char*)ws + main_bytes);
    float* Sk = (float*)((char*)ws + main_bytes + pbytes);
    float* lay = (float*)((char*)ws + main_bytes + pbytes + sbytes);
    const bool has_bias = b_t != nullptr || db_t != nullptr;
    if (phases & 1) {
        int rc = biu_mfma_wgrad(skip, xf_skip, da, 3, 3, 3, dw_conv, nullptr, ws, main_bytes, dtype, st, bn, nullptr, nullptr, ccat, cup);
        if (rc != BIU_OK) return rc;
    }
    if (phases & 4) {
        int rc = biu_mfma_upconv_wgrad(x_low, xf_low, da, nullptr, ws, main_bytes, dtype, st, nullptr);
        if (rc != BIU_OK) return rc;
    }
    if (!(phases & 2)) return BIU_OK;
    if (has_bias) {
        const ShellDims sh = shell_dims(da->n, da->d, da->h, da->w);
        BIU_DISPATCH_DTYPE(dtype, hipLaunchKernelGGL(k_foldt_border_sums<T>, dim3(FOLDT_SUM_BLOCKS), dim3(256), foldt_sum_lds(cout), st,
                                                     (const char*)da->p, sh, da->c, da->pitch, R));
        BIU_CHECK_LAUNCH("foldt_border_sums");
        float* Rsum = Sk + 27 * cout;
        hipLaunchKernelGGL(k_foldt_reduce_tables, dim3(27, FOLDT_RED_SPLIT), dim3(256), 0, st, (const float*)R, FOLDT_SUM_BLOCKS, cout, Rsum);
        hipLaunchKernelGGL(k_foldt_inside_sums, dim3(27, (cout + 31) / 32), dim3(256), 0, st, (const float*)Rsum, FOLDT_RED_SPLIT, cout, Sk, dy_sum);
        BIU_CHECK_LAUNCH("foldt_inside_sums");
    }
    const size_t slice_f = wgrad_acc_bytes(cout, cin_low, 8) / sizeof(float);
    if (cup <= cin_low && biu_fold_gemm_ok(cin_low, cup, cout)) {
        int rc = biu_fold_gemm_layouts(w_conv, ccat, cup, cout, w_t, cin_low, lay, st);
        if (rc == BIU_OK) rc = biu_fold_gemm_chain((const float*)ws, slice_f, lay, cin_low, cup, cout, ccat, dw_conv, dw_t, b_t, (const float*)Sk, st);
        if (rc != BIU_OK) return rc;
        if (db_t) hipLaunchKernelGGL(k_foldt_chain_bt, dim3(cup), dim3(256), 0, st, (const float*)Sk, w_conv, cup, cout, ccat, db_t);
        BIU_CHECK_LAUNCH("foldt_chain_bt");
        return BIU_OK;
    }
    hipLaunchKernelGGL(k_foldt_chain_wconv, dim3((cup + 31) / 32, (cout + 31) / 32, 27), dim3(256), 0, st, (const float*)ws, slice_f, w_t, cin_low, cup, cout, ccat,
                       dw_conv, b_t, (const float*)Sk);
    hipLaunchKernelGGL(k_foldt_chain_wt, dim3((cup + 31) / 32, (cin_low + 31) / 32, 8), dim3(256), 0, st, (const float*)ws, slice_f, w_conv, cin_low, cup, cout, ccat,
                       dw_t);
    if (db_t) hipLaunchKernelGGL(k_foldt_chain_bt, dim3(cup), dim3(256), 0, st, (const float*)Sk, w_conv, cup, cout, ccat, db_t);
    BIU_CHECK_LAUNCH("foldt_chain");
    return BIU_OK;
}

int biu_mfma_convt_wgrad(const biu_act* x, const biu_xform* xf, const biu_act* dy, int kd, float* dw, float* dbias, void* ws,
                         size_t ws_bytes, int dtype, hipStream_t st) {
    WgradArgs a;
    a.py = nullptr; a.ypitch = 0;
    a.bn_scale = a.bn_shift = a.bn_slope = a.bn_cA = a.bn_cB = a.bn_cC = nullptr;
    a.pa = (const char*)x->p;   a.apitch = x->pitch;   a.CA = x->c;
    a.pb = (const char*)dy->p;  a.bpitch = dy->pitch;  a.CB = dy->c;
    a.fold_par = -1;
    a.pb1 = nullptr; a.bpitch1 = 0; a.bsplit = 0; a.bs1_ = a.bb1_ = a.bl1_ = nullptr;
    a.ws = (float*)ws;
    int rc = wgrad_xf(xf, &a.as_, &a.ab_, &a.al_);
    if (rc) return rc;
    a.bs_ = a.bb_ = a.bl_ = nullptr;
    a.N = x->n;
    a.GD = x->d; a.GH = x->h; a.GW = x->w;
    a.BD = dy->d; a.BH = dy->h; a.BW = dy->w;
    const int taps = kd * 4;
    const size_t need = wgrad_acc_bytes(a.CA, a.CB, taps);
    BIU_REQUIRE(ws_bytes >= need + (dbias ? biu_chan_sum_workspace(dy->c) : 0), BIU_ERR_WORKSPACE, "convt_wgrad_mfma: workspace %zu too small", ws_bytes);
    a.dbias_out = dbias;
    if (int zr = zero_ws(ws, need, dbias, dbias ? dy->c : 0, st)) return zr;
    const bool wide = a.CA > 32;
    if (dtype == BIU_BF16) {
        if (wide) rc = (kd == 2) ? launch_wgrad<bf16_t, 2, 2, 2, 2, 4, 16, 2, 2>(a, st) : launch_wgrad<bf16_t, 1, 2, 2, 1, 8, 16, 4, 2>(a, st);
        else rc = (kd == 2) ? launch_wgrad<bf16_t, 2, 2, 2, 2, 4, 16, 2>(a, st) : launch_wgrad<bf16_t, 1, 2, 2, 1, 8, 16, 4>(a, st);
    } else {
        if (kd == 1 && x3_mode_of(kd, dtype) == 2) rc = wide ? launch_wgrad<f32x6_t, 1, 2, 2, 1, 8, 16, 4, 2>(a, st) : launch_wgrad<f32x6_t, 1, 2, 2, 1, 8, 16, 4>(a, st);
        else if (kd == 1 && x3_mode_of(kd, dtype) == 1) rc = wide ? launch_wgrad<f32x3_t, 1, 2, 2, 1, 8, 16, 4, 2>(a, st) : launch_wgrad<f32x3_t, 1, 2, 2, 1, 8, 16, 4>(a, st);
        else if (kd == 2 && x3_mode_of(kd, dtype) == 2) rc = launch_wgrad<f32x6_t, 2, 2, 2, 1, 4, 16, 2>(a, st);
        else if (kd == 2 && x3_mode_of(kd, dtype) == 1) rc = launch_wgrad<f32x3_t, 2, 2, 2, 2, 4, 16, 2>(a, st);
// ... 10 lines not shown
```

### bio_image_unet_amd/csrc/biu_extra.hip

```cpp
#include <hip/hip_runtime.h>

#include "biu_common.h"
#include "biu_internal.h"

namespace {

constexpr int TPB = 256;

struct Tap { int i0, i1; float l0, l1; };
__device__ __forceinline__ Tap tap_of(int o, int n_in, bool scaled) {
    if (!scaled) return Tap{o, o, 1.f, 0.f};
    float src = 0.5f * ((float)o + 0.5f) - 0.5f;
    src = src < 0.f ? 0.f : src;
    const int i0 = (int)src;
    const int i1 = i0 + 1 < n_in ? i0 + 1 : n_in - 1;
    const float l1 = src - (float)i0;
    return Tap{i0, i1, 1.f - l1, l1};
}
__device__ __forceinline__ void split(i64 v, int d, int h, int w, int& n, int& z, int& y, int& x) {
    x = (int)(v % w); v /= w;
    y = (int)(v % h); v /= h;
    z = (int)(v % d);
    n = (int)(v / d);
}
// ... 152 lines not shown
    BIU_CHECK_LAUNCH("xcorr_fwd");
    return BIU_OK;
}
extern "C" int biu_xcorr_bwd(const biu_act* cur, const biu_xform* xc, const biu_act* prev, const biu_xform* xp, const biu_act* dout,
                             const biu_act* dcur, const biu_act* dprev, int accumulate, int dtype, biu_stream stream) {
    BIU_REQUIRE(valid_act(cur) && valid_act(prev) && valid_act(dout) && valid_act(dcur) && valid_act(dprev) && same_space(cur, prev) &&
                    same_space(cur, dout) && same_space(cur, dcur) && same_space(cur, dprev) && cur->c == prev->c && cur->c == dout->c &&
                    cur->c == dcur->c && cur->c == dprev->c && cur->d == 1, BIU_ERR_SHAPE, "xcorr_bwd: equal 2-D tensors expected");
    BIU_REQUIRE(!(xc && (xc->scale || xc->shift || xc->slope)) && !(xp && (xp->scale || xp->shift || xp->slope)), BIU_ERR_UNSUPPORTED,
                "xcorr_bwd: operands must be materialised (identity transform); the gradient is taken w.r.t. the stored values");
    hipStream_t st = (hipStream_t)stream;
    const i64 tot = nvox(cur) * cur->c;
    BIU_DISPATCH_DTYPE(dtype, {
        hipLaunchKernelGGL(k_xcorr_bwd<T>, dim3(grid_for(tot, TPB, 16384)), dim3(TPB), 0, st, dact(prev), dxf(xp), dact(dout), dact(dcur), 0, accumulate);
        hipLaunchKernelGGL(k_xcorr_bwd<T>, dim3(grid_for(tot, TPB, 16384)), dim3(TPB), 0, st, dact(cur), dxf(xc), dact(dout), dact(dprev), 1, accumulate);
    });
    BIU_CHECK_LAUNCH("xcorr_bwd");
    return BIU_OK;
}

namespace {
__global__ __launch_bounds__(256) void k_bce_dice_fwd(const float* __restrict__ lg, const float* __restrict__ tg, i64 per_sample,
                                                      float* __restrict__ partial ) {
    const int n = blockIdx.y;
    const float* l = lg + (i64)n * per_sample;
    const float* t = tg + (i64)n * per_sample;
    float s0 = 0.f, s1 = 0.f, s2 = 0.f, s3 = 0.f;
    for (i64 i = (i64)blockIdx.x * blockDim.x + threadIdx.x; i < per_sample; i += (i64)gridDim.x * blockDim.x) {
        const float x = l[i], y = t[i];
        const float e = __expf(-fabsf(x));
        s0 += fmaxf(x, 0.f) - x * y + log1pf(e);
        const float p = x >= 0.f ? 1.f / (1.f + e) : e / (1.f + e);
        s1 += p;
        s2 += y;
        s3 += p * y;
    }
    __shared__ float red[16];
    float* dst = partial + ((i64)n * gridDim.x + blockIdx.x) * 4;
    float r;
    r = block_sum(s0, red); if (threadIdx.x == 0) dst[0] = r;
    r = block_sum(s1, red); if (threadIdx.x == 0) dst[1] = r;
    r = block_sum(s2, red); if (threadIdx.x == 0) dst[2] = r;
    r = block_sum(s3, red); if (threadIdx.x == 0) dst[3] = r;
}
__global__ __launch_bounds__(256) void k_bce_dice_bwd(const float* __restrict__ lg, const float* __restrict__ tg, i64 per_sample,
                                                      const float* __restrict__ coef ,
                                                      float* __restrict__ dl, int accumulate) {
    const int n = blockIdx.y;
    const float cb = coef[n * 3 + 0], cp = coef[n * 3 + 1], cpt = coef[n * 3 + 2];
    const i64 base = (i64)n * per_sample;
    for (i64 i = (i64)blockIdx.x * blockDim.x + threadIdx.x; i < per_sample; i += (i64)gridDim.x * blockDim.x) {
        const float x = lg[base + i], y = tg[base + i];
        const float e = __expf(-fabsf(x));
        const float p = x >= 0.f ? 1.f / (1.f + e) : e / (1.f + e);
        float g = cb * (p - y) + (cp + cpt * y) * p * (1.f - p);
        if (accumulate) g += dl[base + i];
        dl[base + i] = g;
    }
}

__device__ __forceinline__ float sl1(float d) { const float a = fabsf(d); return a < 1.f ? 0.5f * d * d : a - 0.5f; }
__device__ __forceinline__ float dsl1(float d) { return d > 1.f ? 1.f : (d < -1.f ? -1.f : d); }
__global__ __launch_bounds__(256) void k_pair_sl1_fwd(const float* __restrict__ lg, i64 per_sample, i64 pairs, float* __restrict__ partial) {
    float s = 0.f;
    for (i64 i = (i64)blockIdx.x * blockDim.x + threadIdx.x; i < pairs; i += (i64)gridDim.x * blockDim.x) s += sl1(lg[i + per_sample] - lg[i]);
    __shared__ float red[16];
    const float r = block_sum(s, red);
    if (threadIdx.x == 0) partial[blockIdx.x] = r;
}
__global__ __launch_bounds__(256) void k_pair_sl1_bwd(const float* __restrict__ lg, i64 per_sample, i64 total, const float* __restrict__ coef,
                                                      float* __restrict__ dl, int accumulate) {
    const float c = coef[0];
    const i64 pairs = total - per_sample;
    for (i64 j = (i64)blockIdx.x * blockDim.x + threadIdx.x; j < total; j += (i64)gridDim.x * blockDim.x) {
        const float x = lg[j];
        float g = 0.f;
        if (j >= per_sample) g += dsl1(x - lg[j - per_sample]);
        if (j < pairs) g -= dsl1(lg[j + per_sample] - x);
        g *= c;
        dl[j] = accumulate ? dl[j] + g : g;
    }
}

__global__ __launch_bounds__(256) void k_head_dlogits(const float* __restrict__ gl, const float* __restrict__ ga, const float* __restrict__ av,
                                                      int act, int ch, i64 S, float* __restrict__ dst, int ctot, int c0, i64 total) {
    for (i64 i = (i64)blockIdx.x * blockDim.x + threadIdx.x; i < total; i += (i64)gridDim.x * blockDim.x) {
        const i64 s = i % S;
        const i64 t = i / S;
        const int c = (int)(t % ch);
        const i64 n = t / ch;
        float g = gl ? gl[i] : 0.f;
        if (ga) {
            const float a = av ? av[i] : 0.f;
            const float d = act == 1 ? a * (1.f - a) : (act == 2 ? 1.f - a * a : (act == 3 ? (a > 0.f ? 1.f : 0.f) : 1.f));
            g = fmaf(ga[i], d, g);
        }
        dst[(n * ctot + c0 + c) * S + s] = g;
    }
}
}

extern "C" int biu_pair_smooth_l1_blocks(long long pairs) {
    long long b = (pairs + 256 * 8 - 1) / (256 * 8);
    return (int)(b < 1 ? 1 : (b > 1024 ? 1024 : b));
}
extern "C" int biu_pair_smooth_l1_fwd(const float* logits, int n, long long per_sample, float* partial, biu_stream stream) {
    BIU_REQUIRE(logits && partial && n > 1 && per_sample > 0, BIU_ERR_SHAPE, "pair_smooth_l1_fwd: needs at least two batch entries");
    const i64 pairs = (i64)(n - 1) * per_sample;
    hipLaunchKernelGGL(k_pair_sl1_fwd, dim3(biu_pair_smooth_l1_blocks(pairs)), dim3(256), 0, (hipStream_t)stream, logits, (i64)per_sample, pairs, partial);
    BIU_CHECK_LAUNCH("pair_smooth_l1_fwd");
    return BIU_OK;
}
extern "C" int biu_pair_smooth_l1_bwd(const float* logits, int n, long long per_sample, const float* coef, float* dlogits, int accumulate,
                                      biu_stream stream) {
    BIU_REQUIRE(logits && coef && dlogits && n > 1 && per_sample > 0, BIU_ERR_SHAPE, "pair_smooth_l1_bwd: bad arguments");
    const i64 total = (i64)n * per_sample;
    hipLaunchKernelGGL(k_pair_sl1_bwd, dim3(grid_for(total, 256, 4096)), dim3(256), 0, (hipStream_t)stream, logits, (i64)per_sample, total, coef,
                       dlogits, accumulate);
    BIU_CHECK_LAUNCH("pair_smooth_l1_bwd");
    return BIU_OK;
}
extern "C" int biu_head_dlogits(const float* g_logits, const float* g_act, const float* activated, int act, int n, int ch, long long spatial,
                                float* dst, int dst_channels, int dst_c0, biu_stream stream) {
    BIU_REQUIRE((g_logits || g_act) && dst && n > 0 && ch > 0 && spatial > 0 && dst_c0 >= 0 && dst_c0 + ch <= dst_channels, BIU_ERR_SHAPE,
                "head_dlogits: bad arguments");
    BIU_REQUIRE(!g_act || act == 0 || activated, BIU_ERR_SHAPE, "head_dlogits: the activation's gradient needs the activated output");
    const i64 total = (i64)n * ch * spatial;
    hipLaunchKernelGGL(k_head_dlogits, dim3(grid_for(total, 256, 4096)), dim3(256), 0, (hipStream_t)stream, g_logits, g_act, activated, act, ch,
                       (i64)spatial, dst, dst_channels, dst_c0, total);
    BIU_CHECK_LAUNCH("head_dlogits");
    return BIU_OK;
}

struct SegLossCfg { float a_bce, a_dice, smooth; int has_tv; float al, be, sm; int logcosh; float w_time; long long pairs; int nbt; };
namespace {
__global__ __launch_bounds__(256) void k_seg_loss_finish(const float* __restrict__ partial, int n, int nb, long long per,
                                                        const float* __restrict__ pt, SegLossCfg c, float* __restrict__ saved) {
    __shared__ double red[256];
    float* sums = saved + 1;
    for (int idx = threadIdx.x >> 6; idx < n * 4; idx += 4) {
        const int i = idx >> 2, k = idx & 3, lane = threadIdx.x & 63;
        double a = 0.0;
        for (int b = lane; b < nb; b += 64) a += (double)partial[((size_t)i * nb + b) * 4 + k];
#pragma unroll
        for (int o = 32; o > 0; o >>= 1) a += __shfl_down(a, o, 64);
        if (lane == 0) sums[idx] = (float)a;
    }
    __syncthreads();
    double tsum = 0.0;
    if (pt)
        for (int b = threadIdx.x; b < c.nbt; b += 256) tsum += (double)pt[b];
    red[threadIdx.x] = tsum;
    __syncthreads();
    for (int s = 128; s > 0; s >>= 1) {
        if (threadIdx.x < s) red[threadIdx.x] += red[threadIdx.x + s];
        __syncthreads();
    }
    if (threadIdx.x == 0) {
        double loss = 0.0, bce = 0.0, dice = 0.0, tp = 0.0, ps = 0.0, ts = 0.0;
        float* den = saved + 1 + 4 * n;
        for (int i = 0; i < n; ++i) {
            bce += (double)sums[4 * i];
            ps += (double)sums[4 * i + 1]; ts += (double)sums[4 * i + 2]; tp += (double)sums[4 * i + 3];
            const float d = sums[4 * i + 1] + sums[4 * i + 2] + c.smooth;
            den[i] = d;
            dice += 2.0 * ((double)sums[4 * i + 3] + c.smooth) / (double)d;
        }
        if (c.a_bce != 0.f) loss += (double)c.a_bce * bce / ((double)n * (double)per);
        if (c.a_dice != 0.f) loss += (double)c.a_dice * (1.0 - dice / n);
        float* tvs = den + n;
        tvs[0] = tvs[1] = tvs[2] = 0.f;
        if (c.has_tv) {
            const double tden = tp + c.al * (ps - tp) + c.be * (ts - tp) + c.sm;
            const double tv = (tp + c.sm) / tden;
            tvs[0] = (float)tp; tvs[1] = (float)tden; tvs[2] = (float)tv;
            loss += c.logcosh ? log(cosh(1.0 - tv)) : (1.0 - tv);
        }
        if (pt) loss += (double)c.w_time * red[0] / (double)c.pairs;
        saved[0] = (float)loss;
    }
}
__global__ void k_seg_loss_coef(const float* __restrict__ g, const float* __restrict__ saved, int n, long long per, SegLossCfg c,
                                float* __restrict__ coef, float* __restrict__ ctime) {
    const int i = blockIdx.x * blockDim.x + threadIdx.x;
    const float gv = g[0];
    if (i == 0 && ctime) ctime[0] = (n > 1) ? gv * (c.w_time / ((float)(n - 1) * (float)per)) : 0.f;
    if (i >= n) return;
    const float* sums = saved + 1 + 4 * i;
    const float den = saved[1 + 4 * n + i];
    const float* tvs = saved + 1 + 5 * n;
    float c0 = 0.f, c1 = 0.f, c2 = 0.f;
    if (c.a_bce != 0.f) c0 = gv * (c.a_bce / ((float)n * (float)per));
    if (c.a_dice != 0.f) {
        c1 += gv * (c.a_dice / n) * 2.0f * (sums[3] + c.smooth) / (den * den);
        c2 += -gv * (c.a_dice / n) * 2.0f / den;
    }
    if (c.has_tv) {
        const float tp = tvs[0], tden = tvs[1], tv = tvs[2];
        const float outer = -gv * (c.logcosh ? tanhf(1.f - tv) : 1.f);
        const float d_tp = (tden - (tp + c.sm) * (1.f - c.al - c.be)) / (tden * tden);
        const float d_ps = -(tp + c.sm) * c.al / (tden * tden);
        c1 += outer * d_ps;
        c2 += outer * d_tp;
    }
    coef[3 * i] = c0; coef[3 * i + 1] = c1; coef[3 * i + 2] = c2;
}
}

extern "C" int biu_seg_loss_finish(const float* partial, int n, int nb, long long per_sample, const float* time_partial, int nbt,
                                   float a_bce, float a_dice, float smooth, int has_tversky, float tv_alpha, float tv_beta, float tv_smooth,
                                   int logcosh, float w_time, float* saved, biu_stream stream) {
    BIU_REQUIRE(partial && saved && n > 0 && nb > 0 && per_sample > 0 && (!time_partial || (nbt > 0 && n > 1)), BIU_ERR_SHAPE, "seg_loss_finish: bad arguments");
    const SegLossCfg c{a_bce, a_dice, smooth, has_tversky, tv_alpha, tv_beta, tv_smooth, logcosh, w_time, (long long)(n - 1) * per_sample, nbt};
    hipLaunchKernelGGL(k_seg_loss_finish, dim3(1), dim3(256), 0, (hipStream_t)stream, partial, n, nb, per_sample, time_partial, c, saved);
    BIU_CHECK_LAUNCH("seg_loss_finish");
    return BIU_OK;
}
extern "C" int biu_seg_loss_coef(const float* g, const float* saved, int n, long long per_sample, float a_bce, float a_dice, float smooth,
                                 int has_tversky, float tv_alpha, float tv_beta, float tv_smooth, int logcosh, float w_time, float* coef,
                                 float* time_coef, biu_stream stream) {
    BIU_REQUIRE(g && saved && coef && n > 0 && per_sample > 0, BIU_ERR_SHAPE, "seg_loss_coef: bad arguments");
    const SegLossCfg c{a_bce, a_dice, smooth, has_tversky, tv_alpha, tv_beta, tv_smooth, logcosh, w_time, (long long)(n - 1) * per_sample, 0};
    hipLaunchKernelGGL(k_seg_loss_coef, dim3((n + 63) / 64), dim3(64), 0, (hipStream_t)stream, g, saved, n, per_sample, c, coef, time_coef);
    BIU_CHECK_LAUNCH("seg_loss_coef");
    return BIU_OK;
}

extern "C" int biu_bce_dice_blocks(long long per_sample) {
    long long b = (per_sample + 256 * 8 - 1) / (256 * 8);
    return (int)(b < 1 ? 1 : (b > 1024 ? 1024 : b));
}
extern "C" int biu_bce_dice_fwd(const float* logits, const float* target, int n, long long per_sample, float* partial,
                                biu_stream stream) {
    BIU_REQUIRE(logits && target && partial && n > 0 && per_sample > 0, BIU_ERR_SHAPE, "bce_dice_fwd: bad arguments");
    hipLaunchKernelGGL(k_bce_dice_fwd, dim3(biu_bce_dice_blocks(per_sample), n), dim3(256), 0, (hipStream_t)stream, logits, target,
                       (i64)per_sample, partial);
    BIU_CHECK_LAUNCH("bce_dice_fwd");
    return BIU_OK;
}
extern "C" int biu_bce_dice_bwd(const float* logits, const float* target, int n, long long per_sample, const float* coef,
                                float* dlogits, int accumulate, biu_stream stream) {
    BIU_REQUIRE(logits && target && coef && dlogits && n > 0 && per_sample > 0, BIU_ERR_SHAPE, "bce_dice_bwd: bad arguments");
    hipLaunchKernelGGL(k_bce_dice_bwd, dim3(biu_bce_dice_blocks(per_sample), n), dim3(256), 0, (hipStream_t)stream, logits, target,
                       (i64)per_sample, coef, dlogits, accumulate);
    BIU_CHECK_LAUNCH("bce_dice_bwd");
    return BIU_OK;
}
```

### bio_image_unet_amd/csrc/biu_internal.h

```cpp
#pragma once
#include "biu_common.h"

struct BiuEnv {
    unsigned long long off;
    bool roll_always;
    bool foldt_always;
    int foldt_cmax;
    int fp32_products;
    int fp32_products_3d;
    int fall_maxca;
};
const BiuEnv& biu_env();
bool biu_off(const char* token);

#define BIU_HIDDEN __attribute__((visibility("hidden")))
extern "C" BIU_HIDDEN int biu_conv_fwd_direct(const biu_act* x, const biu_xform* xf, const float* w, const float* bias, int kd,
                                   int kh, int kw, int dil, const biu_act* y, int dtype, hipStream_t st);
extern "C" BIU_HIDDEN int biu_conv_bwd_data_direct(const biu_act* dy, const float* w, int kd, int kh, int kw, int dil,
                                        const biu_act* dx, int accumulate, int dtype, hipStream_t st);
extern "C" BIU_HIDDEN int biu_conv_bwd_weight_direct(const biu_act* x, const biu_xform* xf, const biu_act* dy, int kd, int kh,
                                          int kw, int dil, float* dw, float* dbias, int dtype, hipStream_t st);
extern "C" BIU_HIDDEN int biu_convt_fwd_direct(const biu_act* x, const biu_xform* xf, const float* w, const float* bias, int kd,
                                    const biu_act* y, int dtype, hipStream_t st);
extern "C" BIU_HIDDEN int biu_convt_bwd_data_direct(const biu_act* dy, const float* w, int kd, const biu_act* dx, int accumulate,
                                         int dtype, hipStream_t st);
extern "C" BIU_HIDDEN int biu_convt_bwd_weight_direct(const biu_act* x, const biu_xform* xf, const biu_act* dy, int kd, float* dw,
                                           float* dbias, int dtype, hipStream_t st);
int biu_chan_sum(const biu_act* a, float* out, int dtype, hipStream_t st);
bool biu_convt_shapes_ok(const biu_act* lo, const biu_act* hi, int kd);

size_t biu_mfma_packed_bytes(int kind, int cin, int cout, int kd, int kh, int kw, int dilation, int dtype);
int biu_mfma_pack(int kind, const float* w, int cin, int cout, int kd, int kh, int kw, int dtype, void* packed,
                  hipStream_t st);
bool biu_mfma_conv_ok(const biu_act* x, const biu_act* y, int kd, int kh, int kw, int dilation, int dtype);
struct BnRedFuse {
    const biu_act* y;
    const float *scale, *shift, *slope, *mean, *invstd;
};
bool biu_mfma_conv_cat_ok(const biu_act* x0, const biu_act* x1, const biu_act* y, int kd, int kh, int kw, int dilation, int dtype);
struct ConvCat {
    const biu_act* x1; const biu_xform* xf1;
    const biu_act* y1; int accumulate1;
};
int biu_mfma_conv(const biu_act* x, const biu_xform* xf, const void* packed, const float* bias, int kd, int kh, int kw,
                  const biu_act* y, int accumulate, float* bn_partial, int dtype, hipStream_t st, const BnRedFuse* red = nullptr,
                  const ConvCat* cat = nullptr, void* split_ws = nullptr, size_t split_ws_bytes = 0);
bool biu_conv_roll_ok(const biu_act* x, const biu_act* y, int dtype, bool has_cat, int accumulate, bool red);
int biu_conv_roll_mshape(const biu_act* x, const biu_act* y, int dtype);
int biu_conv_roll_rows(const biu_act* x, const biu_act* y, int dtype);
int biu_conv_roll(const biu_act* x, const biu_xform* xf, const void* packed, const float* bias, const biu_act* y, float* bn_partial, const BnRedFuse* red,
                  hipStream_t st, int accumulate = 0);
bool biu_fold_roll_ok(const biu_act* x_low, const biu_act* y, int dtype);
int biu_fold_roll(const biu_act* x_low, const biu_xform* xf, const void* packed_fwd, const float* bias_sum, const float* fix, const biu_act* y, hipStream_t st);
size_t biu_fold_gemm_layout_floats(int cin_low, int cup, int cout);
bool biu_fold_gemm_ok(int cin_low, int cup, int cout);
int biu_fold_gemm_layouts(const float* w_conv, int ccat, int cup, int cout, const float* w_t, int cin_low, float* layouts, hipStream_t st);
int biu_fold_gemm_compose(const float* layouts, int cin_low, int cup, int cout, const float* b_t, float* wfold, float* wb, hipStream_t st);
int biu_fold_gemm_chain(const float* G, size_t slice_f, const float* layouts, int cin_low, int cup, int cout, int ccat, float* dw_conv, float* dw_t,
                        const float* b_t, const float* Sk, hipStream_t st);
size_t biu_mfma_conv_split_bytes(int cin, const biu_act* y, const biu_act* y1, int kd, int dtype);
int biu_mfma_convt_dgrad_bricks(const biu_act* dx, int kd);
int biu_mfma_convt_dgrad_rows(const biu_act* dx, int kd, int cdy, int dtype);
int biu_mfma_pack_batch(const biu_pack_job* jobs_device, int n, int dtype, hipStream_t st);
int biu_mfma_set_fp32_products(int mode);
int biu_mfma_set_fp32_products_3d(int mode);
int biu_mfma_conv_ksplit(int cin, const biu_act* y, int kd, int dtype);
int biu_mfma_conv_stat_rows(const biu_act* y, int kd, const biu_act* x = nullptr, int dtype = -1, bool red = false, int cin = -1);
int biu_mfma_conv_bricks(const biu_act* y, int kd, const biu_act* x = nullptr, int dtype = -1, int cin = -1);
size_t biu_mfma_wgrad_workspace(int cin, int cout, int kd, int kh, int kw, int dtype);
bool biu_mfma_wgrad_ok(const biu_act* x, const biu_act* dy, int kd, int kh, int kw, int dilation, int dtype);
struct BnBwdFuse {
    const biu_act* y;
    const float *scale, *shift, *slope, *cA, *cB, *cC;
};
int biu_mfma_wgrad(const biu_act* x, const biu_xform* xf, const biu_act* dy, int kd, int kh, int kw, float* dw,
                   float* dbias, void* ws, size_t ws_bytes, int dtype, hipStream_t st, const BnBwdFuse* bn = nullptr,
                   const biu_act* x1 = nullptr, const biu_xform* xf1 = nullptr, int dw_ld_cols = 0, int dw_c_off = 0);

size_t biu_mfma_convt_packed_bytes(int kind, int cin, int cout, int kd, int dtype);
int biu_mfma_convt_pack(int kind, const float* w, int cin, int cout, int kd, int dtype, void* packed, hipStream_t st);
bool biu_mfma_upconv_ok(const biu_act* x, const biu_act* y, int dtype);
size_t biu_mfma_upconv_packed_bytes(int kind, int cin, int cout, int dtype);
int biu_mfma_upconv_pack(int kind, const float* w, int cin, int cout, int dtype, void* packed, hipStream_t st, const float* wf = nullptr);
int biu_mfma_upconv_dgrad_rows(const biu_act* dx);
int biu_mfma_upconv_dgrad(const biu_act* dy, const void* packed, const biu_act* dx, int accumulate, int dtype, hipStream_t st, float* bn_partial = nullptr,
                          const BnRedFuse* red = nullptr);
struct BnBwdFuse;
size_t biu_mfma_upconv_wgrad_workspace(int cin, int cout, int dtype);
int biu_mfma_upconv_wgrad(const biu_act* x, const biu_xform* xf, const biu_act* dy, float* dw, void* ws, size_t ws_bytes, int dtype,
                          hipStream_t st, const BnBwdFuse* bn);
int biu_mfma_upconv_stat_rows(const biu_act* x, const biu_act* y);
int biu_mfma_upconv_fwd(const biu_act* x, const biu_xform* xf, const void* packed, const float* bias, const biu_act* y, float* bn_partial,
                        int dtype, hipStream_t st, int accumulate = 0);
bool biu_mfma_foldt_ok(const biu_act* x_low, const biu_act* skip, const biu_act* y, int dtype);
bool biu_mfma_foldt_worth(const biu_act* x_low, const biu_act* y);
size_t biu_mfma_foldt_packed_bytes(int cin_low, int cskip, int cout, int dtype);
int biu_mfma_foldt_pack(const float* w_conv, const float* b_conv, const float* w_t, const float* b_t, int cin_low, int cup, int cskip, int cout, int dtype,
                        void* packed, hipStream_t st);
int biu_mfma_foldt_stat_rows(const biu_act* x_low, const biu_act* y, const biu_act* skip = nullptr, int dtype = -1);
int biu_mfma_foldt_form(const biu_act* x_low, const biu_act* skip, const biu_act* y, int dtype);
int biu_mfma_foldt_fwd(const biu_act* x_low, const biu_xform* xf_low, const biu_act* skip, const biu_xform* xf_skip, const void* packed, const biu_act* y,
                       float* bn_partial, int dtype, hipStream_t st);
int biu_mfma_foldt_dgrad(const biu_act* dy, const void* packed, const biu_act* dx_low, int acc_low, const biu_act* dskip, int acc_skip, int dtype,
                         hipStream_t st, float* bn_partial_low, const BnRedFuse* red_low, void* ws, size_t ws_bytes);
size_t biu_mfma_foldt_wgrad_workspace(int cin_low, int cskip, int cout, int dtype);
int biu_mfma_foldt_wgrad(const biu_act* x_low, const biu_xform* xf_low, const biu_act* skip, const biu_xform* xf_skip, const biu_act* da, const BnBwdFuse* bn,
                         const float* dy_sum, const float* w_conv, const float* w_t, const float* b_t, int cup, float* dw_conv, float* dw_t, float* db_t, void* ws, size_t ws_bytes,
                         int dtype, hipStream_t st, int phases = 7);
bool biu_mfma_convt_ok(int kind, const biu_act* lo, const biu_act* hi, int kd, int dtype);
int biu_mfma_convt_fwd(const biu_act* x, const biu_xform* xf, const void* packed, const float* bias, int kd, const biu_act* y,
                       int dtype, hipStream_t st);
int biu_mfma_convt_dgrad(const biu_act* dy, const void* packed, int kd, const biu_act* dx, int accumulate, int dtype, hipStream_t st,
                         float* bn_partial = nullptr, const BnRedFuse* red = nullptr);
bool biu_mfma_convt_wgrad_ok(const biu_act* x, const biu_act* dy, int kd, int dtype);
int biu_mfma_convt_wgrad(const biu_act* x, const biu_xform* xf, const biu_act* dy, int kd, float* dw, float* dbias, void* ws,
                         size_t ws_bytes, int dtype, hipStream_t st);

bool biu_c1_conv_ok(const biu_act* x, const biu_act* y, int kd, int kh, int kw, int dil, int dtype);
int biu_c1_conv_fwd(const biu_act* x, const biu_xform* xf, const float* w, const float* bias, int kd, const biu_act* y, int dtype, hipStream_t st);
size_t biu_c1_wgrad_workspace(int cout, int kd);
int biu_c1_conv_wgrad(const biu_act* x, const biu_xform* xf, const biu_act* dy, int kd, float* dw, void* ws, size_t ws_bytes, int dtype, hipStream_t st);
bool biu_vec_reduce_ok(const biu_act* a, int dtype);
int biu_bn_stats_vec(const biu_act* y, float* partial, int* nblk_out, int dtype, hipStream_t st);
int biu_bn_bwd_reduce_vec(const biu_act* da, const biu_act* y, const float* scale, const float* shift, const float* slope,
                          const float* mean, const float* invstd, float* partial, int* nblk_out, int dtype, hipStream_t st);
size_t biu_chan_sum_workspace(int c);
int biu_chan_sum_vec(const biu_act* a, float* out, void* ws, int dtype, hipStream_t st);
bool biu_head_bwd_fused_ok(const biu_act* x, const biu_act* dx, int cout, int dtype);
size_t biu_head_bwd_fused_workspace(int cin);
bool biu_head_bwd_bnred_ok(const biu_act* x, const biu_act* dx, int cout, int dtype);
int biu_head_bwd_bnred_fused(const biu_act* x, const biu_xform* xf, const float* w, int cout, const float* dl, const biu_act* dx, float* dw,
                             float* db, void* ws, const float* mean, const float* invstd, float* bn_partial, int* bn_nblk, int dtype,
                             hipStream_t st);
int biu_head_bwd_fused(const biu_act* x, const biu_xform* xf, const float* w, int cout, const float* dl, const biu_act* dx, float* dw,
                       float* db, void* ws, size_t ws_bytes, int dtype, hipStream_t st);
bool biu_rowvec_ok(const biu_act* a, int dtype);
int biu_bn_bwd_apply_rv(const biu_act* da, const biu_act* y, const float* scale, const float* shift, const float* slope,
                        const float* A, const float* B, const float* Cc, const biu_act* dy, int dtype, hipStream_t st);
int biu_xform_apply_rv(const biu_act* x, const biu_xform* xf, const biu_act* out, int dtype, hipStream_t st);
int biu_maxpool_fwd_rv(const biu_act* x, const biu_xform* xf, const biu_act* out, int pd, int dtype, hipStream_t st);
int biu_maxpool_bwd_rv(const biu_act* x, const biu_xform* xf, const biu_act* dout, const biu_act* dx, int pd, int accumulate, int dtype, hipStream_t st);
int biu_maxpool_bwd_bnred_rv(const biu_act* x, const biu_xform* xf, const biu_act* dout, const biu_act* dx, int pd, int accumulate,
                             const float* mean, const float* invstd, float* partial, size_t partial_floats, int* nblk, int dtype,
                             hipStream_t st);
int biu_nearest_rv(int mode, const biu_act* src, const biu_xform* xf, const biu_act* dst, int pd, int accumulate, int dtype, hipStream_t st);

bool biu_convt_all_ok(const biu_act* lo, const biu_act* hi, int kd, int dtype);
int biu_convt_all_fwd(const biu_act* x, const biu_xform* xf, const void* packed, const float* bias, int kd, const biu_act* y, hipStream_t st);
int biu_convt_all_dgrad_rows(const biu_act* dx, const biu_act* dy, int kd);
int biu_convt_all_dgrad(const biu_act* dy, const void* packed, int kd, const biu_act* dx, int accumulate, hipStream_t st,
                        float* bn_partial = nullptr, const BnRedFuse* red = nullptr);

// ... 7 lines not shown
```

### bio_image_unet_amd/engine.py

```python
from __future__ import annotations

import ctypes as C
import os
import weakref
from typing import Dict, List, Optional, Sequence, Tuple

import torch
from torch import nn

from . import _lib
from ._lib import BIU_BF16, BIU_F32, BN_MAX_PARTIALS, biu_act, biu_xform, check, lib

LRELU_SLOPE = 0.1


def _stream():
    return C.c_void_p(torch.cuda.current_stream().cuda_stream)


def _ptr(t: Optional[torch.Tensor]):
    return C.c_void_p(t.data_ptr()) if t is not None else None


def _disabled(token: str, env: Optional[str] = None) -> bool:
# ... 700 lines not shown
        self._keep = []

    def _sample(self, act: Act, tensor: torch.Tensor, n: int) -> biu_act:
        per = act.d * act.h * act.w * act.buf.shape[4] * tensor.element_size()
        return biu_act(tensor.data_ptr() + act.c0 * tensor.element_size() + n * per, 1, act.d, act.h, act.w, act.c, act.buf.shape[4])

    def fwd(self, eng):
        x, st = self.xin, _stream()
        p = float(self.drop.p)
        if self.drop.training and p > 0.0:
            if self.mask_override is not None:
                keep = self.mask_override.to(device=eng.device, dtype=torch.float32)
            else:
                keep = torch.bernoulli(torch.full((x.n, x.c), 1.0 - p, device=eng.device))
            self.factor = keep / (1.0 - p)
        else:
            self.factor = torch.ones((x.n, x.c), device=eng.device)
        sc = (x.vec("scale")[None, :] * self.factor).contiguous()
        sh = (x.vec("shift")[None, :] * self.factor).contiguous()
        sl = x.vec("slope").contiguous()
        self._keep = [sc, sh, sl]
        for n in range(x.n):
            xf = biu_xform(sc[n].data_ptr(), sh[n].data_ptr(), sl.data_ptr())
            a_in, a_out = self._sample(x, x.buf.t, n), self._sample(self.y, self.y.buf.t, n)
            check(lib.biu_xform_apply(C.byref(a_in), C.byref(xf), C.byref(a_out), eng.dtype, st), "dropout_fwd")

    def bwd(self, eng):
        if not self.y.g_written() or not eng.wants_grad(self.xin):
            return
        assert not self.xin.g_written(), "DropoutNode is the only reader of its input"
        st = _stream()
        f = self.factor.contiguous()
        zero, one = torch.zeros_like(f[0]), torch.ones_like(f[0])
        self._keep += [f, zero, one]
        for n in range(self.xin.n):
            xf = biu_xform(f[n].data_ptr(), zero.data_ptr(), one.data_ptr())
            g_out, g_in = self._sample(self.y, self.y.buf.grad(), n), self._sample(self.xin, self.xin.buf.grad(), n)
            check(lib.biu_xform_apply(C.byref(g_out), C.byref(xf), C.byref(g_in), eng.dtype, st), "dropout_bwd")
        self.xin.mark_g()


class AddReluNode(Node):

    def __init__(self, eng, a: Act, b: Act, out: Act):
        self.a_, self.b_, self.y = a, b, out
        a.consumed()
        b.consumed()

    def fwd(self, eng):
        check(lib.biu_add_relu_fwd(self.a_.a(), self.a_.xf(), self.b_.a(), self.b_.xf(), self.y.a(), eng.dtype, _stream()), "add_relu_fwd")

    def bwd(self, eng):
        if not self.y.g_written():
            return
        assert self.a_.g_written() == self.b_.g_written()
        check(lib.biu_add_relu_bwd(self.y.a(), self.y.g(), self.a_.g(), self.b_.g(), int(self.a_.g_written()), eng.dtype, _stream()),
              "add_relu_bwd")
        self.a_.mark_g()
        self.b_.mark_g()


class GateNode(Node):

    def __init__(self, eng, e: Act, psi: Act, out: Act):
        assert psi.c == 1 and e.c == out.c
        self.e_, self.psi_, self.y = e, psi, out
        e.consumed()
        psi.consumed()

    def fwd(self, eng):
        check(lib.biu_gate_fwd(self.e_.a(), self.e_.xf(), self.psi_.a(), self.psi_.xf(), self.y.a(), eng.dtype, _stream()), "gate_fwd")

    def bwd(self, eng):
        if not self.y.g_written():
            return
        assert not self.psi_.g_written()
        check(lib.biu_gate_bwd(self.e_.a(), self.e_.xf(), self.psi_.a(), self.psi_.xf(), self.y.g(), self.e_.g(),
                               int(self.e_.g_written()), self.psi_.g(), eng.dtype, _stream()), "gate_bwd")
        self.e_.mark_g()
        self.psi_.mark_g()


_ACT_CODE = {None: 0, "none": 0, "sigmoid": 1, "tanh": 2, "relu": 3}


class HeadNode(Node):

    def __init__(self, eng, conv: nn.Module, xin: Act, activation, want_logits: bool, want_act: bool):
        self.conv, self.xin = conv, xin
        xin.consumed()
        self.cout = conv.weight.shape[0]
        assert conv.weight.shape[1] == xin.c
        if activation not in _ACT_CODE:
            activation = None
        self.activation = activation
        self.act = _ACT_CODE[activation]
        self.want_logits, self.want_act = want_logits, want_act
        self.params = [conv.weight, conv.bias]
        eng.need_ws(lib.biu_head_bwd_workspace(xin.c))
        self.logits = self.activated = None

    def out_shape(self, eng):
        x = self.xin
        return (x.n, self.cout, x.d, x.h, x.w) if eng.nd == 3 else (x.n, self.cout, x.h, x.w)

    def fwd(self, eng):
        shp = self.out_shape(eng)
        self.logits = torch.empty(shp, dtype=torch.float32, device=eng.device) if self.want_logits else None
        self.activated = torch.empty(shp, dtype=torch.float32, device=eng.device) if self.want_act else None
        w = self.conv.weight.data.reshape(self.cout, self.xin.c)
        check(lib.biu_head_fwd(self.xin.a(), self.xin.xf(), _ptr(w), _ptr(self.conv.bias.data), self.cout, self.act,
                               _ptr(self.logits), _ptr(self.activated), eng.dtype, _stream()), "head_fwd")

    def dlogits(self, eng, g_logits, g_act, a, dst=None, ctot=None, c0=0):
        if g_act is None and dst is None and g_logits.dtype == torch.float32 and g_logits.is_contiguous():
            return g_logits
        shp = self.out_shape(eng)
        n, spatial = shp[0], 1
        for v in shp[2:]:
            spatial *= v
        if dst is None:
            dst, ctot, c0 = torch.empty(shp, dtype=torch.float32, device=eng.device), self.cout, 0
        f32 = lambda t: None if t is None else t.contiguous().float()
        gl, ga = f32(g_logits), f32(g_act)
        self._keep = (gl, ga, a)
        check(lib.biu_head_dlogits(_ptr(gl), _ptr(ga), _ptr(a) if ga is not None else None, self.act, n, self.cout, spatial,
                                   _ptr(dst), ctot, c0, _stream()), "head_dlogits")
        return dst

    def bwd_with(self, eng, dl: Optional[torch.Tensor]):
        if dl is None:
            return
        dl = dl.contiguous().float()
        st = _stream()
        dw, db = eng.new_grad(self.conv.weight), eng.new_grad(self.conv.bias)
        want_dx = eng.wants_grad(self.xin)
        assert not self.xin.g_written(), "heads that share a trunk go through Engine._backward_heads"
        up = self.xin.last_writer_producer() if (want_dx and self.xin.xf() is not None) else None
        if up is not None:
            part = up.red_buffer(eng, up.kd, 0)
            n_up = C.c_int(0)
            check(lib.biu_head_bwd_bnred(self.xin.a(), self.xin.xf(), _ptr(self.conv.weight.data), self.cout, _ptr(dl),
                                         self.xin.g(), _ptr(dw), _ptr(db), _ptr(eng.ws), eng.ws_bytes, _ptr(up.save_mean),
                                         _ptr(up.save_invstd), _ptr(part), part.numel(), C.byref(n_up), eng.dtype, st),
                  "head_bwd_bnred")
            up.red_nblk = n_up.value
        else:
            check(lib.biu_head_bwd(self.xin.a(), self.xin.xf(), _ptr(self.conv.weight.data), self.cout, _ptr(dl),
                                   self.xin.g() if want_dx else None, _ptr(dw), _ptr(db), _ptr(eng.ws), eng.ws_bytes,
                                   eng.dtype, st), "head_bwd")
        eng.add_grad(self.conv.weight, dw)
        eng.add_grad(self.conv.bias, db)
        if want_dx:
            self.xin.mark_g()


class Engine:

    def __init__(self, device, tdtype, nd: int):
        if torch.device(device).type != "cuda":
            raise RuntimeError("bio_image_unet_amd executes only through its HIP kernels on an MI355X; "
                               f"got device '{device}'. There is no CPU fallback.")
        self.device, self.tdtype, self.nd = torch.device(device), tdtype, nd
        self.dtype = {torch.float32: BIU_F32, torch.bfloat16: BIU_BF16}[tdtype]
        self.nodes: List[Node] = []
        self.heads: List[HeadNode] = []
        self.bufs: List[Buf] = []
        self.inputs: List[Act] = []
        self._partial_c = 0
        self.ws_bytes = 0
        self.partial = self.ws = None
        self.coef = None
        self.grads: Dict[nn.Parameter, torch.Tensor] = {}
        self.nbt_bump: List[torch.Tensor] = []
        self.grad_mode = False
        self.module_training = True
        self.input_requires_grad = False
        self._packed: Dict[int, dict] = {}
        self._zero_flat, self._zero_used = None, 0
        self._slots: List[dict] = []
        self._job_key, self._job_tab = None, None
        self.grad_hook = None
        self.grad_alloc = None
        self.trace = None
        self.generation = 0
        self._live = None
        self._side = None
        self._deferred = []
        self._fold_ev = None

    def busy(self) -> bool:
        return self._live is not None and self._live() is not None

    def invalidate_packed(self):
        for s in self._slots:
            s["ver"] = None
        for nd_ in self.nodes:
            for name in ("fold_slot", "fold_dg_slot"):
# ... 254 lines not shown
        if not live:
            return
        groups: Dict[int, list] = {}
        for h, g in live:
            groups.setdefault(id(h.xin), []).append((h, g))
        for grp in groups.values():
            self._backward_head_group(grp)

    def _backward_head_group(self, live):
        if len(live) == 1:
            h, (gl, ga, a) = live[0]
            h.bwd_with(self, h.dlogits(self, gl, ga, a))
            return
        x = live[0][0].xin
        assert all(h.xin is x for h, _ in live)
        cout = sum(h.cout for h, _ in live)
        shp = live[0][0].out_shape(self)
        dl = torch.empty((shp[0], cout) + tuple(shp[2:]), dtype=torch.float32, device=self.device)
        key = tuple(id(h) for h, _ in live)
        if not hasattr(self, "_stack_w"):
            self._stack_w = {}
        if key not in self._stack_w:
            self._stack_w[key] = torch.empty((cout, x.c), dtype=torch.float32, device=self.device)
        w, o = self._stack_w[key], 0
        for h, (gl, ga, a) in live:
            w[o:o + h.cout].copy_(h.conv.weight.data.reshape(h.cout, x.c))
            h.dlogits(self, gl, ga, a, dst=dl, ctot=cout, c0=o)
            o += h.cout
        dw = torch.empty_like(w)
        db = torch.empty(cout, dtype=torch.float32, device=self.device)
        up = None
        if self.wants_grad(x) and x.xf() is not None and not x.g_written() and len(x.leaves) == 1:
            k = x.leaves[0]
            cand = x.buf.producer.get(k)
            if (x.buf.ncons.get(k, 0) == len(live) and cand is not None and getattr(cand, "batch_stats", False)
                    and cand.y.c == x.c and cand.y.c0 == x.c0):
                up = cand
        if up is not None:
            part = up.red_buffer(self, up.kd, 0)
            n_up = C.c_int(0)
            check(lib.biu_head_bwd_bnred(x.a(), x.xf(), _ptr(w), cout, _ptr(dl), x.g(), _ptr(dw), _ptr(db), _ptr(self.ws), self.ws_bytes,
                                         _ptr(up.save_mean), _ptr(up.save_invstd), _ptr(part), part.numel(), C.byref(n_up), self.dtype,
                                         _stream()), "head_bwd_bnred(stacked)")
            up.red_nblk = n_up.value
        else:
            check(lib.biu_head_bwd(x.a(), x.xf(), _ptr(w), cout, _ptr(dl), x.g(), _ptr(dw), _ptr(db), _ptr(self.ws),
                                   self.ws_bytes, self.dtype, _stream()), "head_bwd(stacked)")
        x.mark_g()
        o = 0
        for h, _ in live:
            self.add_grad(h.conv.weight, dw[o:o + h.cout].reshape(h.conv.weight.shape).clone())
            self.add_grad(h.conv.bias, db[o:o + h.cout].clone())
            o += h.cout

    def input_grads(self) -> List[Optional[torch.Tensor]]:
        outs = []
        st = _stream()
        for act in self.inputs:
            if not self.input_requires_grad or not act.g_written():
                outs.append(None)
                continue
            shp = (act.n, act.c, act.d, act.h, act.w) if self.nd == 3 else (act.n, act.c, act.h, act.w)
            t = torch.empty(shp, dtype=torch.float32, device=self.device)
            ga = biu_act(act.buf.grad().data_ptr(), act.n, act.d, act.h, act.w, act.c, act.buf.shape[4])
            check(lib.biu_to_nchw(C.byref(ga), None, _ptr(t), self.dtype, st), "to_nchw")
            outs.append(t)
        return outs


class _Token:
    __slots__ = ("__weakref__",)


class _NetFn(torch.autograd.Function):

    @staticmethod
    def forward(ctx, eng: Engine, n_inputs: int, out_spec, *tensors):
        xs, ctx.n_inputs = tensors[:n_inputs], n_inputs
        if eng.busy():
            raise RuntimeError("engine re-entered while an earlier forward still awaits its backward (models take a second "
                               "engine for that case: this is a bug in the caller of engine.run)")
        eng.load_inputs(xs)
        eng.forward()
        ctx.eng, ctx.out_spec = eng, out_spec
        ctx.generation = eng.generation
        if eng.grad_mode:
            ctx.token = _Token()
            eng._live = weakref.ref(ctx.token)
        else:
            eng._live = None
        outs = []
        for hi, kind in out_spec:
            h = eng.heads[hi]
            outs.append(h.logits if kind == "logits" else h.activated)
        ctx.act_slot = {hi: i for i, (hi, kind) in enumerate(out_spec) if kind == "act"}
        ctx.save_for_backward(*[outs[i] for i in ctx.act_slot.values()])
        for h in eng.heads:
            h.logits = h.activated = None
        return tuple(outs)

    @staticmethod
    def backward(ctx, *gouts):
        eng: Engine = ctx.eng
        if ctx.generation != eng.generation:
            raise RuntimeError("backward of a forward whose activations were overwritten: the engine ran another forward of the "
                               "same input shape in between (generation %d, now %d)" % (ctx.generation, eng.generation))
        per_head: Dict[int, List[Optional[torch.Tensor]]] = {}
        for (hi, kind), g in zip(ctx.out_spec, gouts):
            slot = per_head.setdefault(hi, [None, None])
            slot[0 if kind == "logits" else 1] = g
        saved = dict(zip(ctx.act_slot.keys(), ctx.saved_tensors))
        head_grads = []
        for hi, h in enumerate(eng.heads):
            gl, ga = per_head.get(hi, [None, None])
            head_grads.append((gl, ga, saved.get(hi)) if (gl is not None or ga is not None) else None)
        grads = eng.backward(head_grads)
        dxs = eng.input_grads()
        pg = [grads.pop(p, None) for p in eng.params]
        eng.grads = {}
        del grads
        ctx.token = None
        eng._live = None
        eng.generation += 1
        return (None, None, None, *dxs, *pg)


def run(eng: Engine, xs: Sequence[torch.Tensor], out_spec):
    eng.grad_mode = torch.is_grad_enabled()
    eng.input_requires_grad = eng.grad_mode and any(x.requires_grad for x in xs)
    return _NetFn.apply(eng, len(xs), tuple(out_spec), *xs, *eng.params)
```

### bio_image_unet_amd/losses.py

```python
import torch
from torch import nn


class BCELoss2d(nn.Module):
    def __init__(self, weight=None, size_average=True):
        super().__init__()
        self.bce_loss = nn.BCEWithLogitsLoss(weight=weight, reduction="mean" if size_average else "sum")

    def forward(self, logits, targets):
        return self.bce_loss(logits, targets)


class SoftDiceLoss(nn.Module):
    def __init__(self, smooth=1.0):
        super().__init__()
        self.smooth = smooth

    def forward(self, logits, targets):
        n = targets.size(0)
        p = torch.sigmoid(logits).view(n, -1)
        t = targets.view(n, -1)
        score = 2.0 * ((p * t).sum(1) + self.smooth) / (p.sum(1) + t.sum(1) + self.smooth)
        return 1 - score.mean()


def _fusable(logits, targets):
    return (logits.is_cuda and logits.dtype == torch.float32 and targets.dtype == torch.float32 and logits.shape == targets.shape
            and logits.is_contiguous() and targets.is_contiguous() and logits.numel() > 0)


class _FusedSegLoss(torch.autograd.Function):

    @staticmethod
    def _scalars(cfg):
        tv = cfg.get("tversky")
        return (float(cfg.get("bce", 0.0)), float(cfg.get("dice", 0.0)), float(cfg.get("smooth", 1.0)), 1 if tv else 0,
                float(tv[0]) if tv else 0.0, float(tv[1]) if tv else 0.0, float(tv[2]) if tv else 0.0, 1 if (tv and tv[3]) else 0,
                float(cfg.get("time", 0.0)))

    @staticmethod
    def forward(ctx, logits, targets, cfg):
        import ctypes as C
        from ._lib import check, lib
        n = targets.size(0)
        per = logits.numel() // n
        st = C.c_void_p(torch.cuda.current_stream().cuda_stream)
        nb = lib.biu_bce_dice_blocks(per)
        partial = torch.empty((n, nb, 4), dtype=torch.float32, device=logits.device)
        check(lib.biu_bce_dice_fwd(C.c_void_p(logits.data_ptr()), C.c_void_p(targets.data_ptr()), n, per,
                                   C.c_void_p(partial.data_ptr()), st), "bce_dice_fwd")
        sc = _FusedSegLoss._scalars(cfg)
        w_time = sc[8]
        pt, nbt = None, 0
        if w_time and n > 1:
            nbt = lib.biu_pair_smooth_l1_blocks((n - 1) * per)
            pt = torch.empty(nbt, dtype=torch.float32, device=logits.device)
            check(lib.biu_pair_smooth_l1_fwd(C.c_void_p(logits.data_ptr()), n, per, C.c_void_p(pt.data_ptr()), st), "pair_smooth_l1_fwd")
        saved = torch.empty(1 + 5 * n + 3, dtype=torch.float32, device=logits.device)
        check(lib.biu_seg_loss_finish(C.c_void_p(partial.data_ptr()), n, nb, per, C.c_void_p(pt.data_ptr()) if pt is not None else None, nbt,
                                      *sc, C.c_void_p(saved.data_ptr()), st), "seg_loss_finish")
        loss = saved[0]
        if w_time and n <= 1:
            loss = loss + float("nan")
        ctx.save_for_backward(logits, targets)
        ctx.saved, ctx.cfg, ctx.np = saved, cfg, (n, per)
        return loss

    @staticmethod
    def backward(ctx, g):
        import ctypes as C
        from ._lib import check, lib
        logits, targets = ctx.saved_tensors
        cfg, saved, (n, per) = ctx.cfg, ctx.saved, ctx.np
        st = C.c_void_p(torch.cuda.current_stream().cuda_stream)
        sc = _FusedSegLoss._scalars(cfg)
        w_time = sc[8]
        g = g.reshape(1).to(torch.float32).contiguous()
        coef = torch.empty((n, 3), dtype=torch.float32, device=logits.device)
        ct = torch.empty(1, dtype=torch.float32, device=logits.device) if (w_time and n > 1) else None
        check(lib.biu_seg_loss_coef(C.c_void_p(g.data_ptr()), C.c_void_p(saved.data_ptr()), n, per, *sc, C.c_void_p(coef.data_ptr()),
                                    C.c_void_p(ct.data_ptr()) if ct is not None else None, st), "seg_loss_coef")
        dl = torch.empty_like(logits)
        check(lib.biu_bce_dice_bwd(C.c_void_p(logits.data_ptr()), C.c_void_p(targets.data_ptr()), n, per,
                                   C.c_void_p(coef.data_ptr()), C.c_void_p(dl.data_ptr()), 0, st), "bce_dice_bwd")
        if ct is not None:
            check(lib.biu_pair_smooth_l1_bwd(C.c_void_p(logits.data_ptr()), n, per, C.c_void_p(ct.data_ptr()), C.c_void_p(dl.data_ptr()), 1, st),
                  "pair_smooth_l1_bwd")
        return dl, None, None


class BCEDiceLoss(nn.Module):
    def __init__(self, alpha, beta):
        super().__init__()
        self.bce, self.dice, self.alpha, self.beta = BCELoss2d(), SoftDiceLoss(), alpha, beta

    def forward(self, logits, targets, time_weight: float = 0.0):
        if _fusable(logits, targets):
            return _FusedSegLoss.apply(logits, targets, dict(bce=float(self.alpha), dice=float(self.beta), smooth=float(self.dice.smooth),
                                                             time=float(time_weight)))
        loss = self.alpha * self.bce(logits, targets) + self.beta * self.dice(logits, targets)
        if time_weight:
            loss = loss + nn.functional.smooth_l1_loss(logits[1:], logits[:-1]) * time_weight
        return loss


class logcoshDiceLoss(nn.Module):
    def __init__(self):
        super().__init__()
        self.dice = SoftDiceLoss()

    def forward(self, logits, targets):
        x = self.dice(logits, targets)
        return torch.log((torch.exp(x) + torch.exp(-x)) / 2)


def _tversky_index(logits, targets, alpha, beta, smooth):
    p = torch.sigmoid(logits).view(-1)
    t = targets.view(-1)
    tp = (p * t).sum()
    fp = ((1 - t) * p).sum()
    fn = (t * (1 - p)).sum()
    return (tp + smooth) / (tp + alpha * fp + beta * fn + smooth)


class TverskyLoss(nn.Module):
    def __init__(self, alpha=0.5, beta=0.5, smooth=1):
        super().__init__()
        self.alpha, self.beta, self.smooth = alpha, beta, smooth

    _logcosh = False

    def forward(self, inputs, targets, time_weight: float = 0.0):
        if _fusable(inputs, targets):
            return _FusedSegLoss.apply(inputs, targets, dict(tversky=(float(self.alpha), float(self.beta), float(self.smooth), self._logcosh),
                                                             time=float(time_weight)))
        x = 1 - _tversky_index(inputs, targets, self.alpha, self.beta, self.smooth)
        loss = torch.log(torch.cosh(x)) if self._logcosh else x
        if time_weight:
            loss = loss + nn.functional.smooth_l1_loss(inputs[1:], inputs[:-1]) * time_weight
        return loss


class logcoshTverskyLoss(TverskyLoss):
    _logcosh = True


class weightedBCELoss(nn.Module):

    def __init__(self, alpha=1, beta=0.1):
        super().__init__()
        self.alpha, self.beta = alpha, beta

    def forward(self, logits, targets):
        probs = torch.sigmoid(logits)
        weights = torch.where(targets >= 0.5, torch.full_like(targets, self.alpha), torch.full_like(targets, self.beta))
        return torch.mean(nn.functional.binary_cross_entropy(probs, targets, reduction="none") * weights)


class BCELoss2dProb(nn.Module):

    def __init__(self, weight=None, reduction="mean", **kwargs):
        super().__init__()
        self.bce_loss = nn.BCELoss(weight, reduction=reduction)

    def forward(self, logits, targets):
        return self.bce_loss(torch.sigmoid(logits).view(-1), targets.view(-1))


class BCEDiceLossSiam(nn.Module):

# ... 26 lines not shown
```

### include/biu.h

```cpp
#ifndef BIU_H
#define BIU_H

#include <stddef.h>
#include <stdint.h>

#ifdef __cplusplus
extern "C" {
#endif

typedef void* biu_stream;

enum { BIU_F32 = 0, BIU_BF16 = 1 };

typedef enum {
    BIU_OK = 0,
    BIU_ERR_SHAPE = -1,
    BIU_ERR_UNSUPPORTED = -2,
    BIU_ERR_ALIGN = -3,
    BIU_ERR_WORKSPACE = -4,
    BIU_ERR_LAUNCH = -5
} biu_status;

typedef struct {
    void*   p;
    int32_t n, d, h, w;
    int32_t c;
    int32_t pitch;
} biu_act;

typedef struct {
    const float* scale;
    const float* shift;
    const float* slope;
} biu_xform;

const char* biu_last_error(void);
int  biu_version(void);

int  biu_set_fp32_products(int mode);

int  biu_set_fp32_products_3d(int mode);


size_t biu_conv_packed_bytes(int kind, int cin, int cout, int kd, int kh, int kw, int dilation, int dtype);
int    biu_conv_pack(int kind, const float* w, int cin, int cout, int kd, int kh, int kw, int dtype,
                     void* packed, biu_stream stream);

typedef struct biu_pack_job {
    const void* w;
    void* packed;
    int32_t transposed, kind, cin, cout, kd, kh, kw, reserved;
} biu_pack_job;
int biu_pack_batch(const biu_pack_job* jobs, int n, int dtype, biu_stream stream);

size_t biu_conv_split_workspace(int cin, const biu_act* y, const biu_act* y1, int kd, int kh, int kw, int dilation, int dtype);

int biu_conv_fwd(const biu_act* x, const biu_xform* xf, const float* w, const void* packed,
                 const float* bias, int kd, int kh, int kw, int dilation,
                 const biu_act* y, void* ws, size_t ws_bytes, int dtype, biu_stream stream);

size_t biu_conv_fwd_stats_floats(const biu_act* y, int kd);
int biu_conv_fwd_stats(const biu_act* x, const biu_xform* xf, const float* w, const void* packed,
                       const float* bias, int kd, int kh, int kw, int dilation, const biu_act* y,
                       float* bn_partial, size_t bn_partial_floats, int* bn_nblk, void* ws, size_t ws_bytes, int dtype,
                       biu_stream stream);

int biu_conv_bwd_data(const biu_act* dy, const float* w, const void* packed,
                      int kd, int kh, int kw, int dilation,
                      const biu_act* dx, int accumulate, void* ws, size_t ws_bytes, int dtype, biu_stream stream);

size_t biu_bwd_data_bnred_floats(const biu_act* dx, int kd, int transposed);
int biu_conv_bwd_data_bnred(const biu_act* dy, const float* w, const void* packed, int kd, int kh, int kw, int dilation,
                            const biu_act* dx, const biu_act* y_up, const float* scale, const float* shift,
                            const float* slope, const float* mean, const float* invstd, float* partial,
                            size_t partial_floats, int* nblk, void* ws, size_t ws_bytes, int dtype, biu_stream stream);
int biu_convt_bwd_data_bnred(const biu_act* dy, const float* w, const void* packed, int kd, const biu_act* dx,
                             const biu_act* y_up, const float* scale, const float* shift, const float* slope,
                             const float* mean, const float* invstd, float* partial, size_t partial_floats, int* nblk,
                             int dtype, biu_stream stream);

size_t biu_conv_bwd_weight_workspace(int cin, int cout, int kd, int kh, int kw, int dtype);
int biu_conv_bwd_weight(const biu_act* x, const biu_xform* xf, const biu_act* dy,
                        int kd, int kh, int kw, int dilation,
                        float* dw, float* dbias, void* ws, size_t ws_bytes, int dtype, biu_stream stream);

int biu_conv_bwd_weight_bn(const biu_act* x, const biu_xform* xf, const biu_act* da, const biu_act* y,
                           const float* scale, const float* shift, const float* slope, const float* coefA,
                           const float* coefB, const float* coefC, int kd, int kh, int kw, int dilation,
                           float* dw, void* ws, size_t ws_bytes, int dtype, biu_stream stream);

#define BIU_BN_MAX_PARTIALS 1024
int biu_bn_stats(const biu_act* y, float* partial, int* nblk_out, int dtype, biu_stream stream);

int biu_bn_finalize(const float* partial, int nblk, int c, double count,
                    const float* gamma, const float* beta, float* running_mean, float* running_var,
                    float momentum, float eps, float* scale, float* shift,
                    float* save_mean, float* save_invstd, biu_stream stream);

int biu_bn_eval_affine(int c, const float* gamma, const float* beta, const float* running_mean,
                       const float* running_var, float eps, float* scale, float* shift, biu_stream stream);

int biu_xform_apply(const biu_act* x, const biu_xform* xf, const biu_act* out, int dtype, biu_stream stream);

int biu_bn_bwd_reduce(const biu_act* da, const biu_act* y, const float* scale, const float* shift,
                      const float* slope, const float* save_mean, const float* save_invstd,
                      float* partial, int* nblk_out, int dtype, biu_stream stream);
int biu_bn_bwd_finalize(const float* partial, int nblk, int c, double count,
                        const float* scale, const float* save_mean, const float* save_invstd,
                        float* dgamma, float* dbeta, float* coefA, float* coefB, float* coefC,
                        biu_stream stream);
int biu_bn_bwd_finalize_eval(const float* partial, int nblk, int c, const float* scale,
                             float* dgamma, float* dbeta, float* dbias, float* coefA, float* coefB, float* coefC,
                             biu_stream stream);
int biu_bn_bwd_apply(const biu_act* da, const biu_act* y, const float* scale, const float* shift,
                     const float* slope, const float* coefA, const float* coefB, const float* coefC,
                     const biu_act* dy, int dtype, biu_stream stream);

int biu_maxpool_fwd(const biu_act* x, const biu_xform* xf, const biu_act* out, int dtype, biu_stream stream);
int biu_maxpool_bwd(const biu_act* x, const biu_xform* xf, const biu_act* dout, const biu_act* dx,
                    int accumulate, int dtype, biu_stream stream);
int biu_maxpool_bwd_bnred(const biu_act* x, const biu_xform* xf, const biu_act* dout, const biu_act* dx, int accumulate,
                          const float* mean, const float* invstd, float* partial, size_t partial_floats, int* nblk,
                          int dtype, biu_stream stream);
int biu_nearest_down_fwd(const biu_act* x, const biu_xform* xf, const biu_act* out, int dtype, biu_stream stream);
int biu_nearest_down_bwd(const biu_act* dout, const biu_act* dx, int accumulate, int dtype, biu_stream stream);
int biu_nearest_up_fwd(const biu_act* x, const biu_xform* xf, const biu_act* out, int dtype, biu_stream stream);
int biu_nearest_up_bwd(const biu_act* dout, const biu_act* dx, int accumulate, int dtype, biu_stream stream);

int    biu_upconv_ok(const biu_act* x, const biu_act* y, int dtype);
size_t biu_upconv_packed_bytes(int kind, int cin, int cout, int dtype);
int    biu_upconv_pack(int kind, const float* w, int cin, int cout, int dtype, void* packed, biu_stream stream);
int    biu_upconv_bwd_data(const biu_act* dy, const void* packed, const biu_act* dx, int accumulate, int dtype, biu_stream stream);
size_t biu_upconv_bwd_weight_workspace(int cin, int cout, int dtype);
int    biu_upconv_bwd_weight_bn(const biu_act* x, const biu_xform* xf, const biu_act* da, const biu_act* y, const float* scale,
                                const float* shift, const float* slope, const float* coefA, const float* coefB, const float* coefC,
                                float* dw, void* ws, size_t ws_bytes, int dtype, biu_stream stream);
size_t biu_upconv_fwd_stats_floats(const biu_act* x, const biu_act* y);
int    biu_upconv_fwd(const biu_act* x, const biu_xform* xf, const void* packed, const float* bias, const biu_act* y,
                      float* bn_partial, size_t bn_partial_floats, int* bn_nblk, int dtype, biu_stream stream);

int biu_bce_dice_blocks(long long per_sample);
int biu_bce_dice_fwd(const float* logits, const float* target, int n, long long per_sample, float* partial, biu_stream stream);
int biu_bce_dice_bwd(const float* logits, const float* target, int n, long long per_sample, const float* coef, float* dlogits,
                     int accumulate, biu_stream stream);

int biu_pair_smooth_l1_blocks(long long pairs);
int biu_pair_smooth_l1_fwd(const float* logits, int n, long long per_sample, float* partial, biu_stream stream);
int biu_pair_smooth_l1_bwd(const float* logits, int n, long long per_sample, const float* coef, float* dlogits, int accumulate,
                           biu_stream stream);
int biu_seg_loss_finish(const float* partial, int n, int nb, long long per_sample, const float* time_partial, int nbt,
                        float a_bce, float a_dice, float smooth, int has_tversky, float tv_alpha, float tv_beta, float tv_smooth,
                        int logcosh, float w_time, float* saved, biu_stream stream);
int biu_seg_loss_coef(const float* g, const float* saved, int n, long long per_sample, float a_bce, float a_dice, float smooth,
                      int has_tversky, float tv_alpha, float tv_beta, float tv_smooth, int logcosh, float w_time, float* coef,
                      float* time_coef, biu_stream stream);
int biu_head_dlogits(const float* g_logits, const float* g_act, const float* activated, int act, int n, int ch, long long spatial,
                     float* dst, int dst_channels, int dst_c0, biu_stream stream);

#define BIU_MO2D_MAX_LEVELS 4
#define BIU_MO2D_MAX_TERMS 32
#define BIU_MO2D_SLOTS 8
typedef struct biu_mo2d_term {
    int kind, nb;
    long long partial_off;
    long long numel, pixels;
    float p0, p1, p2, weight;
} biu_mo2d_term;
int biu_mo2d_loss_blocks(long long numel);
int biu_mo2d_loss_fwd(int kind, float ea, float eb, const float* const* pred, int nlev, const float* target, int n, int c, int h, int w,
                      float* partial, biu_stream stream);
int biu_mo2d_loss_finish(const biu_mo2d_term* terms, int nterms, const float* workspace, float* saved, biu_stream stream);
int biu_mo2d_loss_coef(const biu_mo2d_term* terms, int nterms, const float* g, const float* saved, float* coef, biu_stream stream);
int biu_mo2d_loss_bwd(int kind, float ea, float eb, const float* const* pred, int nlev, const float* target, int n, int c, int h, int w,
                      const float* coef, float* const* dpred, biu_stream stream);

int biu_trilinear_up_fwd(const biu_act* x, const biu_xform* xf, const biu_act* out, int dtype, biu_stream stream);
int biu_trilinear_up_bwd(const biu_act* dout, const biu_act* dx, int accumulate, int dtype, biu_stream stream);

int biu_bilinear_up_fwd(const biu_act* x, const biu_xform* xf, const biu_act* out, int dtype, biu_stream stream);
int biu_bilinear_up_bwd(const biu_act* dout, const biu_act* dx, int accumulate, int dtype, biu_stream stream);

int biu_xcorr_fwd(const biu_act* cur, const biu_xform* xc, const biu_act* prev, const biu_xform* xp, const biu_act* out,
                  int dtype, biu_stream stream);
int biu_xcorr_bwd(const biu_act* cur, const biu_xform* xc, const biu_act* prev, const biu_xform* xp, const biu_act* dout,
                  const biu_act* dcur, const biu_act* dprev, int accumulate, int dtype, biu_stream stream);

int biu_conv_cat_ok(const biu_act* x0, const biu_act* x1, const biu_act* y, int kd, int kh, int kw, int dilation, int dtype);
int biu_conv_fwd_cat(const biu_act* x0, const biu_xform* xf0, const biu_act* x1, const biu_xform* xf1, const float* w,
                     const void* packed, const float* bias, int kd, int kh, int kw, int dilation, const biu_act* y,
                     float* bn_partial, size_t bn_partial_floats, int* bn_nblk, void* ws, size_t ws_bytes, int dtype,
                     biu_stream stream);
int biu_conv_bwd_data_cat(const biu_act* dy, const float* w, const void* packed, int kd, int kh, int kw, int dilation,
                          const biu_act* dx0, int accumulate0, const biu_act* dx1, int accumulate1, void* ws, size_t ws_bytes,
                          int dtype, biu_stream stream);
int biu_conv_bwd_weight_cat(const biu_act* x0, const biu_xform* xf0, const biu_act* x1, const biu_xform* xf1,
                            const biu_act* da, const biu_act* y, const float* scale, const float* shift, const float* slope,
                            const float* coefA, const float* coefB, const float* coefC, int kd, int kh, int kw, int dilation,
                            float* dw, void* ws, size_t ws_bytes, int dtype, biu_stream stream);

size_t biu_convt_packed_bytes(int kind, int cin, int cout, int kd, int dtype);
int    biu_convt_pack(int kind, const float* w, int cin, int cout, int kd, int dtype, void* packed, biu_stream stream);
int biu_convt_fwd(const biu_act* x, const biu_xform* xf, const float* w, const void* packed, const float* bias,
                  int kd, const biu_act* y, int dtype, biu_stream stream);
int biu_convt_bwd_data(const biu_act* dy, const float* w, const void* packed, int kd, const biu_act* dx,
                       int accumulate, int dtype, biu_stream stream);
size_t biu_convt_bwd_weight_workspace(int cin, int cout, int kd, int dtype);
int biu_convt_bwd_weight(const biu_act* x, const biu_xform* xf, const biu_act* dy, int kd, float* dw, float* dbias,
                         void* ws, size_t ws_bytes, int dtype, biu_stream stream);

int    biu_foldt_ok(const biu_act* x_low, const biu_act* skip, const biu_act* y, int dtype);
size_t biu_foldt_packed_bytes(int cin_low, int cskip, int cout, int dtype);
int    biu_foldt_pack(const float* w_conv, const float* b_conv, const float* w_t, const float* b_t, int cin_low, int cup, int cskip, int cout,
                      int dtype, void* packed, biu_stream stream);
size_t biu_foldt_fwd_stats_floats(const biu_act* x_low, const biu_act* y);
int    biu_foldt_fwd_form(const biu_act* x_low, const biu_act* skip, const biu_act* y, int dtype);
int    biu_foldt_fwd(const biu_act* x_low, const biu_xform* xf_low, const biu_act* skip, const biu_xform* xf_skip, const void* packed,
                     const biu_act* y, float* bn_partial, size_t bn_partial_floats, int* bn_nblk, int dtype, biu_stream stream);
size_t biu_foldt_bwd_data_bnred_floats(const biu_act* dx_low);
int    biu_foldt_bwd_data(const biu_act* dy, const void* packed, const biu_act* dx_low, int acc_low, const biu_act* dskip, int acc_skip,
                          const biu_act* y_low, const float* scale, const float* shift, const float* slope, const float* mean,
                          const float* invstd, float* partial, size_t partial_floats, int* nblk, void* ws, size_t ws_bytes, int dtype,
                          biu_stream stream);
size_t biu_foldt_bwd_weight_workspace(int cin_low, int cskip, int cout, int dtype);
int    biu_foldt_bwd_weight_bn(const biu_act* x_low, const biu_xform* xf_low, const biu_act* skip, const biu_xform* xf_skip, const biu_act* da,
                               const biu_act* y, const float* scale, const float* shift, const float* slope, const float* coefA,
                               const float* coefB, const float* coefC, const float* dy_sum, const float* w_conv, const float* w_t, const float* b_t,
                               int cup, float* dw_conv, float* dw_t, float* db_t, void* ws, size_t ws_bytes, int dtype, biu_stream stream);
int    biu_foldt_bwd_weight_bn_phase(const biu_act* x_low, const biu_xform* xf_low, const biu_act* skip, const biu_xform* xf_skip, const biu_act* da,
                                     const biu_act* y, const float* scale, const float* shift, const float* slope, const float* coefA,
                                     const float* coefB, const float* coefC, const float* dy_sum, const float* w_conv, const float* w_t,
                                     const float* b_t, int cup, float* dw_conv, float* dw_t, float* db_t, void* ws, size_t ws_bytes, int dtype,
                                     int phases, biu_stream stream);

int biu_head_fwd(const biu_act* x, const biu_xform* xf, const float* w, const float* bias, int cout,
                 int act, float* logits, float* activated, int dtype, biu_stream stream);
size_t biu_head_bwd_workspace(int cin);
int biu_head_bwd(const biu_act* x, const biu_xform* xf, const float* w, int cout, const float* dlogits,
                 const biu_act* dx, float* dw, float* dbias, void* ws, size_t ws_bytes, int dtype,
// ... 91 lines not shown
```

Before: 758.5 million voxels/s.

## Write per-block wgrad slabs with deterministic reduce; fuse segmentation loss kernels

For bf16 3x3x3 weight gradients, each wgrad block now writes its partial accumulators to a private workspace slab. A separate reduce kernel then sums the slabs into dw, replacing the previous shared accumulation scheme. Separately, the BCE/Dice and pair smooth-L1 loss forward and backward passes are fused into single kernels with one buffer allocation, and autograd grad materialization is disabled. The slab path needs a larger workspace plus an extra reduce pass and more global traffic, in exchange for avoiding atomics or zero-fill and cutting loss-stage launches.

New measurement: 758.4 million voxels/s, median of 2. About the same (-0.0%).

```diff
diff --git a/bio_image_unet_amd/_lib.py b/bio_image_unet_amd/_lib.py
--- a/bio_image_unet_amd/_lib.py
+++ b/bio_image_unet_amd/_lib.py
@@ -72,6 +72,7 @@
     "biu_conv_bwd_data_bnred": (_I, [_A, _P, _P, _I, _I, _I, _I, _A, _A, _P, _P, _P, _P, _P, _P, _Z, C.POINTER(C.c_int), _P, _Z, _I, _P]),
     "biu_convt_bwd_data_bnred": (_I, [_A, _P, _P, _I, _A, _A, _P, _P, _P, _P, _P, _P, _Z, C.POINTER(C.c_int), _I, _P]),
     "biu_conv_bwd_weight_workspace": (_Z, [_I, _I, _I, _I, _I, _I]),
+    "biu_conv_bwd_weight_form": (_I, [_A, _A, _I, _I]),
     "biu_conv_bwd_weight": (_I, [_A, _X, _A, _I, _I, _I, _I, _P, _P, _P, _Z, _I, _P]),
     "biu_conv_bwd_weight_bn": (_I, [_A, _X, _A, _A, _P, _P, _P, _P, _P, _P, _I, _I, _I, _I, _P, _P, _Z, _I, _P]),
     "biu_bn_stats": (_I, [_A, _P, C.POINTER(C.c_int), _I, _P]),
@@ -103,6 +104,9 @@
     "biu_pair_smooth_l1_blocks": (_I, [C.c_longlong]),
     "biu_pair_smooth_l1_fwd": (_I, [_P, _I, C.c_longlong, _P, _P]),
     "biu_pair_smooth_l1_bwd": (_I, [_P, _I, C.c_longlong, _P, _P, _I, _P]),
+    "biu_seg_loss_blocks": (_I, [C.c_longlong]),
+    "biu_seg_loss_fwd": (_I, [_P, _P, _I, C.c_longlong, _I, _P, _P, _P]),
+    "biu_seg_loss_bwd": (_I, [_P, _P, _I, C.c_longlong, _P, _P, _P, _I, _P]),
     "biu_seg_loss_finish": (_I, [_P, _I, _I, C.c_longlong, _P, _I, _F, _F, _F, _I, _F, _F, _F, _I, _F, _P, _P]),
     "biu_seg_loss_coef": (_I, [_P, _P, _I, C.c_longlong, _F, _F, _F, _I, _F, _F, _F, _I, _F, _P, _P, _P]),
     "biu_head_dlogits": (_I, [_P, _P, _P, _I, _I, _I, C.c_longlong, _P, _I, _I, _P]),
diff --git a/bio_image_unet_amd/csrc/biu_api.hip b/bio_image_unet_amd/csrc/biu_api.hip
--- a/bio_image_unet_amd/csrc/biu_api.hip
+++ b/bio_image_unet_amd/csrc/biu_api.hip
@@ -8,7 +8,7 @@
     "conv_fwd", "conv_dgrad", "conv_wgrad", "convt_fwd", "convt_dgrad", "convt_wgrad", "convt_all", "c1", "c1_mfma", "cat",
     "fused_stats", "wgrad_bn", "dgrad_bnred", "pool_pair", "pool_pipe", "pool_bnred", "head_bnred", "ksplit", "m16", "m16x2", "rr16",
     "wroll", "wroll16", "wroll2d", "upconv", "foldt", "foldall", "foldck8", "foldgemm", "croll", "froll", "prepack", "wsplitbn",
-    "capturefork", "sidechain",
+    "wslab", "wslabfall", "capturefork", "sidechain",
 };
 constexpr int kNumOffTokens = sizeof(kOffTokens) / sizeof(kOffTokens[0]);
 static_assert(kNumOffTokens <= 64, "BiuEnv::off holds one bit per token");
@@ -257,6 +257,11 @@
         return a > b ? a : b;
     }
     return biu_mfma_wgrad_workspace(cin, cout, kd, kh, kw, dtype);
+}
+
+extern "C" int biu_conv_bwd_weight_form(const biu_act* x, const biu_act* dy, int kd, int dtype) {
+    if (!x || !dy || !conv_args_ok(x, dy, kd, 3, 3, 1) || biu_off("conv_wgrad") || !biu_mfma_wgrad_ok(x, dy, kd, 3, 3, 1, dtype)) return 0;
+    return biu_mfma_wgrad_form(x, dy, kd, dtype);
 }
 
 extern "C" int biu_conv_bwd_weight(const biu_act* x, const biu_xform* xf, const biu_act* dy, int kd, int kh, int kw,
diff --git a/bio_image_unet_amd/csrc/biu_conv_mfma.hip b/bio_image_unet_amd/csrc/biu_conv_mfma.hip
--- a/bio_image_unet_amd/csrc/biu_conv_mfma.hip
+++ b/bio_image_unet_amd/csrc/biu_conv_mfma.hip
@@ -2341,7 +2341,10 @@
     float* dbias_out;
     int fold_par;
     size_t fold_slice_f;
+    unsigned slab_f = 0, slab_base = 0;
 };
+constexpr unsigned WSLAB_F = 27 * 32 * 32;
+constexpr unsigned WSLAB_FALL_F = 64 * 32 * 32;
 
 template <typename T, int PE>
 __device__ __forceinline__ uint4 apply_xf16(uint4 v, const float* sc, const float* sh, const float* sl) {
@@ -2965,6 +2968,70 @@
         }
     }
     const int hf = lane >> 5;
+    constexpr bool SLABK = sizeof(T) == 2 && KD == 3 && KHW == 3 && S == 1 && KSPLIT == 1 && NI == 1 && !FALL;
+    if constexpr (SLABK) if (a.slab_f) {
+        float* sp = a.ws + ((size_t)a.slab_base + (size_t)blockIdx.y * gridDim.x + blockIdx.x) * a.slab_f;
+        if (rr16) {
+            float* lc = (float*)at;
+            __syncthreads();
+            if (wave >= 6) {
+#pragma unroll
+                for (int tb = 0; tb < 3; ++tb)
+#pragma unroll
+                    for (int e = 0; e < 16; ++e) lc[(((wave - 6) * 3 + tb) * 16 + e) * 64 + lane] = acc[tb][0][e];
+            }
+            __syncthreads();
+            if (wave < 2) {
+#pragma unroll
+                for (int tb = 0; tb < 3; ++tb)
+#pragma unroll
+                    for (int e = 0; e < 16; ++e) acc[tb][0][e] += lc[((wave * 3 + tb) * 16 + e) * 64 + lane];
+            }
+            const int ch = lane & 15, up = (lane >> 4) & 1;
+            const int kd = (u16_unit < 3) ? up : 2, kw = (u16_unit < 3) ? u16_unit : u16_unit - 3;
+            if (wave < 6 && !(up && u16_unit >= 3)) {
+#pragma unroll
+                for (int tb = 0; tb < 3; ++tb) {
+                    const int tap = (kd * 3 + tb) * 3 + kw;
+#pragma unroll
+                    for (int e = 0; e < 16; ++e) {
+                        const int il = (e & 3) + 8 * (e >> 2) + 4 * hf;
+                        if (it * CTA + il < a.CA) sp[(tap * CT + il) * CT + ch] = acc[tb][0][e];
+                    }
+                }
+            }
+            return;
+        }
+        if (jt * CT + (lane & 31) < a.CB) {
+#pragma unroll
+            for (int t2 = 0; t2 < IPW; ++t2) {
+                const int tap = tapid[t2];
+                if (tap < TAPS) {
+#pragma unroll
+                    for (int e = 0; e < 16; ++e) {
+                        const int il = (e & 3) + 8 * (e >> 2) + 4 * hf;
+                        if (it * CTA + il < a.CA) sp[(tap * CT + il) * CT + (lane & 31)] = acc[t2][0][e];
+                    }
+                }
+            }
+        }
+        return;
+    }
+    if constexpr (FALL) if (a.slab_f) {
+        float* sp = a.ws + ((size_t)a.slab_base + (size_t)blockIdx.y * gridDim.x + blockIdx.x) * a.slab_f + (size_t)wave * (TAPS * CT * CT);
+        if (jt * CT + (lane & 31) < a.CB) {
+#pragma unroll
+            for (int t2 = 0; t2 < IPW; ++t2) {
+                const int tap = tapid[t2];
+#pragma unroll
+                for (int e = 0; e < 16; ++e) {
+                    const int il = (e & 3) + 8 * (e >> 2) + 4 * hf;
+                    if (it * CTA + il < a.CA) sp[(tap * CT + il) * CT + (lane & 31)] = acc[t2][0][e];
+                }
+            }
+        }
+        return;
+    }
     if (rr16) {
         const int ch = lane & 15, up = (lane >> 4) & 1;
         const int kd = (u16_unit < 3) ? up : 2, kw = (u16_unit < 3) ? u16_unit : u16_unit - 3;
@@ -3427,6 +3494,39 @@
 #endif
     const int hf = lane >> 5;
     const int jj = jt * CT + (lane & 31);
+    if constexpr (!K2D) if (a.slab_f) {
+        float* sp = a.ws + ((size_t)a.slab_base + (size_t)blockIdx.y * gridDim.x + blockIdx.x) * a.slab_f;
+        if (jj < a.CB) {
+            if constexpr (A16) {
+                const int uj = wave & 3;
+#pragma unroll
+                for (int u = 0; u < 2; ++u) {
+                    if (u == 1 && !has_x) break;
+                    const int kw = u ? 2 : (wave >> 2);
+#pragma unroll
+                    for (int tb = 0; tb < 3; ++tb)
+#pragma unroll
+                        for (int e = 0; e < 16; ++e) {
+                            const int pl = e >> 3, kd = uj - pl, il = (e & 3) + 8 * ((e >> 2) & 1) + 4 * hf;
+                            if (kd >= 0 && kd <= 2 && il < a.CA) sp[((pl * TAPS + (kd * 3 + tb) * 3 + kw) * 16 + il) * CT + (lane & 31)] = acc[u * 3 + tb][e];
+                        }
+                }
+            } else {
+#pragma unroll
+                for (int t2 = 0; t2 < IPW; ++t2) {
+                    const int tap = tapid[t2];
+                    if (tap < TAPS) {
+#pragma unroll
+                        for (int e = 0; e < 16; ++e) {
+                            const int il = (e & 3) + 8 * (e >> 2) + 4 * hf;
+                            if (it * CT + il < a.CA) sp[(tap * CT + il) * CT + (lane & 31)] = acc[t2][e];
+                        }
+                    }
+                }
+            }
+        }
+        return;
+    }
     if constexpr (A16) {
         const int uj = wave & 3;
         if (jj < a.CB) {
@@ -3469,7 +3569,9 @@
     return a.N >= 8 && ncols >= 8 && a.CA * a.CB > 1024 && bytesA < BIU_MAX_SAMPLE_BYTES && bytesB < BIU_MAX_SAMPLE_BYTES && bytesY < BIU_MAX_SAMPLE_BYTES;
 }
 
-static int launch_wgrad_roll(WgradArgs a, hipStream_t st, bool k2d = false) {
+struct WslabPlan { int jt_split, g0, g1, base1; };
+
+static int launch_wgrad_roll(WgradArgs a, hipStream_t st, bool k2d = false, WslabPlan* plan = nullptr) {
     if (k2d) { a.GD = a.BD = a.N; a.N = 1; }
     const bool a16 = !k2d && a.CA == 16 && !biu_off("wroll16");
     a.nbd = 1;
@@ -3496,10 +3598,11 @@
             return biu_fail(BIU_ERR_LAUNCH, "wgrad_roll: cannot reserve %zu bytes of LDS", WR_LDS);
         attr_set = true;
     }
-    auto launch = [&](int jt_begin, int jt_count, int write_back, bool with_bn) {
+    auto launch = [&](int jt_begin, int jt_count, int write_back, bool with_bn, int slab_base) -> int {
         WgradArgs b = a;
         if (!with_bn) b.py = nullptr;
         b.jt_begin = jt_begin; b.jt_count = jt_count; b.write_back = write_back;
+        b.slab_f = plan ? WSLAB_F : 0; b.slab_base = (unsigned)slab_base;
         const int pairs = nit * jt_count;
         int g = num_cus() / pairs;
         if (g >= 16) g = grid_per_column(num_cus(), pairs);
@@ -3515,13 +3618,16 @@
             if (with_bn) hipLaunchKernelGGL((k_wgrad_roll<true, false>), dim3(g, pairs), dim3(512), WR_LDS, st, b);
             else hipLaunchKernelGGL((k_wgrad_roll<false, false>), dim3(g, pairs), dim3(512), WR_LDS, st, b);
         }
+        return g;
     };
     if (a.py && a.njt > 1) {
-        launch(0, 1, 1, true);
+        const int g0 = launch(0, 1, 1, true, 0);
         BIU_CHECK_LAUNCH("wgrad_roll");
-        launch(1, a.njt - 1, 0, false);
+        const int g1 = launch(1, a.njt - 1, 0, false, nit * g0);
+        if (plan) *plan = WslabPlan{1, g0, g1, nit * g0};
     } else {
-        launch(0, a.njt, a.py ? 1 : 0, a.py != nullptr);
+        const int g = launch(0, a.njt, a.py ? 1 : 0, a.py != nullptr, 0);
+        if (plan) *plan = WslabPlan{0, 0, g, 0};
     }
     BIU_CHECK_LAUNCH("wgrad_roll");
     return BIU_OK;
@@ -3539,6 +3645,61 @@
     }
 }
 
+struct WslabReduceArgs {
+    const float* ws; float* dw;
+    int rows, cols, taps, ld_cols, c_off;
+    int njt, half;
+    WslabPlan plan;
+    unsigned slab_f;
+    size_t fold_slice_f;
+};
+__global__ __launch_bounds__(256) void k_wgrad_slab_reduce(WslabReduceArgs a) {
+    __shared__ float red[8][32];
+    const int rows_t = a.half ? 16 : 32;
+    const int tap = blockIdx.x / rows_t, il = blockIdx.x % rows_t;
+    const int it = blockIdx.y / a.njt, jt = blockIdx.y % a.njt;
+    const int jl = threadIdx.x & 31, grp = threadIdx.x >> 5;
+    const int i = it * 32 + il, j = jt * 32 + jl;
+    int first, cnt;
+    if (jt < a.plan.jt_split) { first = (it * a.plan.jt_split + jt) * a.plan.g0; cnt = a.plan.g0; }
+    else { first = a.plan.base1 + (it * (a.njt - a.plan.jt_split) + (jt - a.plan.jt_split)) * a.plan.g1; cnt = a.plan.g1; }
+    const int units = a.half ? 2 * cnt : cnt;
+    const int per = (units + 7) / 8;
+    const int lo = grp * per, hi = (lo + per < units) ? lo + per : units;
+    const size_t tile_off = (size_t)(tap * rows_t + il) * 32 + jl, plane_f = (size_t)a.taps * 16 * 32;
+    auto at = [&](int u) -> float {
+        const size_t off = a.half ? (size_t)(first + (u >> 1)) * a.slab_f + (size_t)(u & 1) * plane_f : (size_t)(first + u) * a.slab_f;
+        return a.ws[off + tile_off];
+    };
+    float s = 0.f;
+    if (i < a.rows && j < a.cols) {
+        int u = lo;
+        for (; u + 8 <= hi; u += 8) {
+            float v[8];
+#pragma unroll
+            for (int k = 0; k < 8; ++k) v[k] = at(u + k);
+#pragma unroll
+            for (int k = 0; k < 8; ++k) s += v[k];
+        }
+        for (; u < hi; ++u) s += at(u);
+    }
+    red[grp][jl] = s;
+    __syncthreads();
+    if (grp == 0 && i < a.rows && j < a.cols) {
+        const float t = ((red[0][jl] + red[1][jl]) + (red[2][jl] + red[3][jl])) + ((red[4][jl] + red[5][jl]) + (red[6][jl] + red[7][jl]));
+        const size_t o = a.fold_slice_f ? (size_t)(tap >> 3) * a.fold_slice_f + ((size_t)(tap & 7) * a.rows + i) * a.cols + j
+                         : a.ld_cols > 0 ? ((size_t)i * a.ld_cols + a.c_off + j) * a.taps + tap : ((size_t)i * a.cols + j) * a.taps + tap;
+        a.dw[o] = t;
+    }
+}
+static size_t wslab_blocks(int pairs) { const int n = num_cus(); return (size_t)(pairs > n ? pairs : n); }
+static size_t wslab_bytes(int ca, int cb) {
+    const int nit = (ca + 31) / 32, njt = (cb + 31) / 32;
+    const size_t one = wslab_blocks(nit * njt), two = njt > 1 ? wslab_blocks(nit) + wslab_blocks(nit * (njt - 1)) : 0;
+    return (one > two ? one : two) * WSLAB_F * sizeof(float);
+}
+static bool wslab_on(int dtype, int kd) { return dtype == BIU_BF16 && kd == 3 && !biu_off("wslab"); }
+
 __global__ void k_zero_f32(float* __restrict__ p, size_t n, float* __restrict__ q, int nq) {
     for (size_t i = (size_t)blockIdx.x * blockDim.x + threadIdx.x; i < n; i += (size_t)gridDim.x * blockDim.x) p[i] = 0.f;
     if (q && blockIdx.x == 0)
@@ -3558,6 +3719,7 @@
 size_t biu_mfma_wgrad_workspace(int cin, int cout, int kd, int kh, int kw, int dtype) {
     if (!wgrad_chan_ok(cin, cout)) return 0;
     const size_t red = biu_chan_sum_workspace(cout);
+    if (kh == 3 && kw == 3 && kd == 3 && wslab_on(dtype, kd)) return wslab_bytes(cout, cin) + red;
     if (kh == 3 && kw == 3 && (kd == 1 || kd == 3)) return wgrad_acc_bytes(cin, cout, kd * 9) + red;
     if (kh == 2 && kw == 2 && (kd == 1 || kd == 2)) return wgrad_acc_bytes(cin, cout, kd * 4) + red;
     return 0;
@@ -3582,8 +3744,20 @@
     return (kd == 1 || kd == 2) && wgrad_chan_ok(x->c, dy->c) && wgrad_ptrs_ok(x, dy, dtype);
 }
 
+static int wgrad3_form(const WgradArgs& a, bool cat) {
+    if (a.CB == 16 && !cat && !biu_off("rr16")) return 4;
+    if (!biu_off("wroll") && wroll_fits(a)) return (a.CA == 16 && !biu_off("wroll16")) ? 3 : 2;
+    return 1;
+}
+int biu_mfma_wgrad_form(const biu_act* x, const biu_act* dy, int kd, int dtype) {
+    if (dtype != BIU_BF16 || kd != 3) return 0;
+    WgradArgs a;
+    a.N = x->n; a.GD = x->d; a.GH = x->h; a.GW = x->w; a.CA = dy->c; a.CB = x->c;
+    return wgrad3_form(a, false) | (wslab_on(dtype, kd) ? 8 : 0);
+}
+
 template <typename T, int KD, int KHW, int S, int TD, int TH, int TW, int KSPLIT, int NI = 1, bool RR16 = false, bool FALL = false>
-static int launch_wgrad(WgradArgs a, hipStream_t st) {
+static int launch_wgrad(WgradArgs a, hipStream_t st, WslabPlan* plan = nullptr) {
     constexpr int SD = (KD == 1) ? 1 : S;
     constexpr int HV = ((TD - 1) * SD + (FALL ? 3 : KD)) * ((TH - 1) * S + (FALL ? 3 : KHW)) * ((TW - 1) * S + (FALL ? 3 : KHW));
     constexpr int BV = (FALL ? 8 : 1) * TD * TH * TW;
@@ -3605,8 +3779,9 @@
             return biu_fail(BIU_ERR_LAUNCH, "wgrad_pipe: cannot reserve %zu bytes of LDS", lds_bytes);
         attr_set = true;
     }
-    auto launch = [&](int jt_begin, int jt_count, int write_back, bool with_bn) {
+    auto launch = [&](int jt_begin, int jt_count, int write_back, bool with_bn, int slab_base) -> int {
         WgradArgs b = a;
+        b.slab_f = plan ? (FALL ? WSLAB_FALL_F : WSLAB_F) : 0; b.slab_base = (unsigned)slab_base;
 #ifdef BIU_DIAG
         b.diag = biu_diag_buffer;
 #else
@@ -3620,13 +3795,16 @@
         if (g < 1) g = 1;
         if (g > b.nbricks) g = b.nbricks;
         hipLaunchKernelGGL(kern, dim3(g, pairs), dim3(512), lds_bytes, st, b);
+        return g;
     };
     if (a.py && a.njt > 1) {
-        launch(0, 1, 1, true);
+        const int g0 = launch(0, 1, 1, true, 0);
         BIU_CHECK_LAUNCH("wgrad_pipe");
-        launch(1, a.njt - 1, 0, false);
+        const int g1 = launch(1, a.njt - 1, 0, false, nit * g0);
+        if (plan) *plan = WslabPlan{1, g0, g1, nit * g0};
     } else {
-        launch(0, a.njt, a.py ? 1 : 0, a.py != nullptr);
+        const int g = launch(0, a.njt, a.py ? 1 : 0, a.py != nullptr, 0);
+        if (plan) *plan = WslabPlan{0, 0, g, 0};
     }
     BIU_CHECK_LAUNCH("wgrad_pipe");
     return BIU_OK;
@@ -3676,11 +3854,28 @@
     a.N = x->n;
     a.GD = a.BD = x->d; a.GH = a.BH = x->h; a.GW = a.BW = x->w;
     const int taps = kd * 9;
-    const size_t need = wgrad_acc_bytes(a.CA, a.CB, taps);
+    const bool slab = wslab_on(dtype, kd);
+    const size_t need = slab ? wslab_bytes(a.CA, a.CB) : wgrad_acc_bytes(a.CA, a.CB, taps);
     BIU_REQUIRE(ws_bytes >= need + (dbias ? biu_chan_sum_workspace(dy->c) : 0), BIU_ERR_WORKSPACE, "wgrad_mfma: workspace %zu too small", ws_bytes);
+    if (slab) {
+        WslabPlan plan{0, 0, 0, 0};
+        const int form = wgrad3_form(a, x1 != nullptr);
+        const bool half = form == 3;
+        if (form == 4) rc = launch_wgrad<bf16_t, 3, 3, 1, 4, 8, 16, 1, 1, true>(a, st, &plan);
+        else if (form >= 2) rc = launch_wgrad_roll(a, st, false, &plan);
+        else rc = launch_wgrad<bf16_t, 3, 3, 1, 4, 8, 16, 1>(a, st, &plan);
+        if (rc != BIU_OK) return rc;
+        const int nit = (a.CA + 31) / 32, njt = (a.CB + 31) / 32;
+        WslabReduceArgs r{(const float*)ws, dw, a.CA, a.CB, taps, dw_ld_cols, dw_c_off, njt, half ? 1 : 0, plan, WSLAB_F, 0};
+        hipLaunchKernelGGL(k_wgrad_slab_reduce, dim3(taps * (half ? 16 : 32), nit * njt), dim3(256), 0, st, r);
+        BIU_CHECK_LAUNCH("wgrad_slab_reduce");
+        if (dbias) return biu_chan_sum_vec(dy, dbias, (char*)ws + need, dtype, st);
+        return BIU_OK;
+    }
     if (int zr = zero_ws(ws, need, nullptr, 0, st)) return zr;
-    if (dtype == BIU_BF16 && kd == 3 && a.CB == 16 && !x1 && !biu_off("rr16")) rc = launch_wgrad<bf16_t, 3, 3, 1, 4, 8, 16, 1, 1, true>(a, st);
-    else if (dtype == BIU_BF16 && kd == 3 && !biu_off("wroll") && wroll_fits(a)) rc = launch_wgrad_roll(a, st);
+    const int form3 = (dtype == BIU_BF16 && kd == 3) ? wgrad3_form(a, x1 != nullptr) : 0;
+    if (form3 == 4) rc = launch_wgrad<bf16_t, 3, 3, 1, 4, 8, 16, 1, 1, true>(a, st);
+    else if (form3 >= 2) rc = launch_wgrad_roll(a, st);
     else if (dtype == BIU_BF16 && kd == 1 && !biu_off("wroll") && !biu_off("wroll2d") &&
              wroll2d_fits(a, (i64)nvox(dy) * dy->pitch * 2, (i64)nvox(x) * x->pitch * 2 > (x1 ? (i64)nvox(x1) * x1->pitch * 2 : 0) ? (i64)nvox(x) * x->pitch * 2 : (i64)nvox(x1) * x1->pitch * 2,
                           bn ? (i64)nvox(bn->y) * bn->y->pitch * 2 : 0))
@@ -3720,9 +3915,11 @@
         dw[idx] = sum;
     }
 }
+static bool fall_slab_on(int ca, int dtype) { return dtype == BIU_BF16 && ca <= biu_env().fall_maxca && !biu_off("foldall") && !biu_off("wslab") && !biu_off("wslabfall"); }
+static size_t fall_slab_bytes(int ca, int cb) { return wslab_blocks(((ca + 31) / 32) * ((cb + 31) / 32)) * WSLAB_FALL_F * sizeof(float); }
 size_t biu_mfma_upconv_wgrad_workspace(int cin, int cout, int dtype) {
     if ((dtype != BIU_BF16 && dtype != BIU_F32) || !wgrad_chan_ok(cin, cout)) return 0;
-    return 8 * wgrad_acc_bytes(cout, cin, 8);
+    return 8 * wgrad_acc_bytes(cout, cin, 8) + (fall_slab_on(cout, dtype) ? fall_slab_bytes(cout, cin) : 0);
 }
 int biu_mfma_upconv_wgrad(const biu_act* x, const biu_xform* xf, const biu_act* dy, float* dw, void* ws, size_t ws_bytes, int dtype,
                           hipStream_t st, const BnBwdFuse* bn) {
@@ -3746,8 +3943,25 @@
     a.GD = a.BD = x->d; a.GH = a.BH = x->h; a.GW = a.BW = x->w;
     const size_t slice = wgrad_acc_bytes(a.CA, a.CB, 8);
     BIU_REQUIRE(ws_bytes >= 8 * slice, BIU_ERR_WORKSPACE, "upconv_wgrad: workspace %zu too small (need %zu)", ws_bytes, 8 * slice);
+    a.fold_slice_f = slice / sizeof(float);
+    if (bn == nullptr && fall_slab_on(a.CA, dtype)) {
+        BIU_REQUIRE(ws_bytes >= 8 * slice + fall_slab_bytes(a.CA, a.CB), BIU_ERR_WORKSPACE, "upconv_wgrad: workspace %zu too small for the slabs", ws_bytes);
+        WslabPlan plan{0, 0, 0, 0};
+        a.ws = (float*)((char*)ws + 8 * slice);
+        a.fold_par = 8;
+        rc = launch_wgrad<bf16_t, 2, 2, 1, 2, 4, 16, 8, 1, false, true>(a, st, &plan);
+        if (rc != BIU_OK) return rc;
+        const int nit = (a.CA + 31) / 32, njt = (a.CB + 31) / 32;
+        WslabReduceArgs r{(const float*)a.ws, (float*)ws, a.CA, a.CB, 64, 0, 0, njt, 0, plan, WSLAB_FALL_F, a.fold_slice_f};
+        hipLaunchKernelGGL(k_wgrad_slab_reduce, dim3(64 * 32, nit * njt), dim3(256), 0, st, r);
+        BIU_CHECK_LAUNCH("wgrad_slab_reduce(fold)");
+        if (!dw) return BIU_OK;
+        hipLaunchKernelGGL(k_upconv_wgrad_unfold, dim3(grid_for((i64)a.CA * a.CB * 27, 256, 2048)), dim3(256), 0, st, (const float*)ws, slice / sizeof(float),
+                           a.CA, a.CB, dw);
+        BIU_CHECK_LAUNCH("upconv_wgrad_unfold");
+        return BIU_OK;
+    }
     if (int zr = zero_ws(ws, 8 * slice, nullptr, 0, st)) return zr;
-    a.fold_slice_f = slice / sizeof(float);
     if (dtype == BIU_BF16 && a.CA <= biu_env().fall_maxca && bn == nullptr && !biu_off("foldall")) {
         a.ws = (float*)ws;
         a.fold_par = 8;
@@ -3933,7 +4147,7 @@
 }
 size_t biu_mfma_foldt_wgrad_workspace(int cin_low, int cskip, int cout, int dtype) {
     if (!wgrad_chan_ok(cin_low, cout) || !wgrad_chan_ok(cskip, cout)) return 0;
-    const size_t g = 8 * wgrad_acc_bytes(cout, cin_low, 8), sk = biu_mfma_wgrad_workspace(cskip, cout, 3, 3, 3, dtype);
+    const size_t g = biu_mfma_upconv_wgrad_workspace(cin_low, cout, dtype), sk = biu_mfma_wgrad_workspace(cskip, cout, 3, 3, 3, dtype);
     return (g > sk ? g : sk) + al256((size_t)FOLDT_SUM_BLOCKS * 27 * cout * sizeof(float)) + al256((size_t)(1 + FOLDT_RED_SPLIT) * 27 * cout * sizeof(float)) +
            al256(biu_fold_gemm_layout_floats(cin_low, cin_low, cout) * sizeof(float));
 }
diff --git a/bio_image_unet_amd/csrc/biu_extra.hip b/bio_image_unet_amd/csrc/biu_extra.hip
--- a/bio_image_unet_amd/csrc/biu_extra.hip
+++ b/bio_image_unet_amd/csrc/biu_extra.hip
@@ -258,6 +258,67 @@
     }
 }
 
+__global__ __launch_bounds__(256) void k_seg_loss_fwd(const float* __restrict__ lg, const float* __restrict__ tg, i64 per_sample, int n, int with_time,
+                                                      float* __restrict__ partial , float* __restrict__ tpart ) {
+    __shared__ float red[16];
+    const i64 chunk = (((per_sample + gridDim.x - 1) / gridDim.x) + 255) & ~(i64)255;
+    const i64 lo = (i64)blockIdx.x * chunk, hi = lo + chunk < per_sample ? lo + chunk : per_sample;
+    float st = 0.f;
+    for (int k = 0; k < n; ++k) {
+        const float* l = lg + (i64)k * per_sample;
+        const float* t = tg + (i64)k * per_sample;
+        float s0 = 0.f, s1 = 0.f, s2 = 0.f, s3 = 0.f;
+#pragma unroll 4
+        for (i64 i = lo + threadIdx.x; i < hi; i += 256) {
+            const float x = l[i], y = t[i];
+            const float e = __expf(-fabsf(x));
+            s0 += fmaxf(x, 0.f) - x * y + log1pf(e);
+            const float p = x >= 0.f ? 1.f / (1.f + e) : e / (1.f + e);
+            s1 += p;
+            s2 += y;
+            s3 += p * y;
+            if (with_time && k > 0) st += sl1(x - l[i - per_sample]);
+        }
+        float* dst = partial + ((i64)k * gridDim.x + blockIdx.x) * 4;
+        float r;
+        r = block_sum(s0, red); if (threadIdx.x == 0) dst[0] = r;
+        r = block_sum(s1, red); if (threadIdx.x == 0) dst[1] = r;
+        r = block_sum(s2, red); if (threadIdx.x == 0) dst[2] = r;
+        r = block_sum(s3, red); if (threadIdx.x == 0) dst[3] = r;
+    }
+    if (with_time) {
+        const float r = block_sum(st, red);
+        if (threadIdx.x == 0) tpart[blockIdx.x] = r;
+    }
+}
+__global__ __launch_bounds__(256) void k_seg_loss_bwd(const float* __restrict__ lg, const float* __restrict__ tg, i64 per_sample, int n,
+                                                      const float* __restrict__ coef , const float* __restrict__ tcoef ,
+                                                      float* __restrict__ dl, int accumulate) {
+    const bool timed = tcoef != nullptr && n > 1;
+    const float ct = timed ? tcoef[0] : 0.f;
+    for (i64 i = (i64)blockIdx.x * blockDim.x + threadIdx.x; i < per_sample; i += (i64)gridDim.x * blockDim.x) {
+        float xp = 0.f, x = lg[i];
+        for (int k = 0; k < n; ++k) {
+            const i64 j = (i64)k * per_sample + i;
+            const float xn = (k + 1 < n) ? lg[j + per_sample] : 0.f;
+            const float y = tg[j];
+            const float cb = coef[k * 3 + 0], cp = coef[k * 3 + 1], cpt = coef[k * 3 + 2];
+            const float e = __expf(-fabsf(x));
+            const float p = x >= 0.f ? 1.f / (1.f + e) : e / (1.f + e);
+            float g = cb * (p - y) + (cp + cpt * y) * p * (1.f - p);
+            if (accumulate) g += dl[j];
+            if (timed) {
+                float gt = 0.f;
+                if (k > 0) gt += dsl1(x - xp);
+                if (k + 1 < n) gt -= dsl1(xn - x);
+                g += gt * ct;
+            }
+            dl[j] = g;
+            xp = x; x = xn;
+        }
+    }
+}
+
 __global__ __launch_bounds__(256) void k_head_dlogits(const float* __restrict__ gl, const float* __restrict__ ga, const float* __restrict__ av,
                                                       int act, int ch, i64 S, float* __restrict__ dst, int ctot, int c0, i64 total) {
     for (i64 i = (i64)blockIdx.x * blockDim.x + threadIdx.x; i < total; i += (i64)gridDim.x * blockDim.x) {
@@ -310,28 +371,35 @@
 
 struct SegLossCfg { float a_bce, a_dice, smooth; int has_tv; float al, be, sm; int logcosh; float w_time; long long pairs; int nbt; };
 namespace {
-__global__ __launch_bounds__(256) void k_seg_loss_finish(const float* __restrict__ partial, int n, int nb, long long per,
+__global__ __launch_bounds__(512) void k_seg_loss_finish(const float* __restrict__ partial, int n, int nb, long long per,
                                                         const float* __restrict__ pt, SegLossCfg c, float* __restrict__ saved) {
-    __shared__ double red[256];
+    __shared__ double tsum_s;
     float* sums = saved + 1;
-    for (int idx = threadIdx.x >> 6; idx < n * 4; idx += 4) {
-        const int i = idx >> 2, k = idx & 3, lane = threadIdx.x & 63;
-        double a = 0.0;
-        for (int b = lane; b < nb; b += 64) a += (double)partial[((size_t)i * nb + b) * 4 + k];
+    const int lane = threadIdx.x & 63, nw = blockDim.x >> 6;
+    for (int it = threadIdx.x >> 6; it < n + 1; it += nw) {
+        if (it < n) {
+            double a[4] = {0.0, 0.0, 0.0, 0.0};
+            const float4* rows = (const float4*)partial + (size_t)it * nb;
+            for (int b = lane; b < nb; b += 64) {
+                const float4 v = rows[b];
+                a[0] += (double)v.x; a[1] += (double)v.y; a[2] += (double)v.z; a[3] += (double)v.w;
+            }
 #pragma unroll
-        for (int o = 32; o > 0; o >>= 1) a += __shfl_down(a, o, 64);
-        if (lane == 0) sums[idx] = (float)a;
+            for (int k = 0; k < 4; ++k) {
+#pragma unroll
+                for (int o = 32; o > 0; o >>= 1) a[k] += __shfl_down(a[k], o, 64);
+                if (lane == 0) sums[it * 4 + k] = (float)a[k];
+            }
+        } else {
+            double ts = 0.0;
+            if (pt)
+                for (int b = lane; b < c.nbt; b += 64) ts += (double)pt[b];
+#pragma unroll
+            for (int o = 32; o > 0; o >>= 1) ts += __shfl_down(ts, o, 64);
+            if (lane == 0) tsum_s = ts;
+        }
     }
     __syncthreads();
-    double tsum = 0.0;
-    if (pt)
-        for (int b = threadIdx.x; b < c.nbt; b += 256) tsum += (double)pt[b];
-    red[threadIdx.x] = tsum;
-    __syncthreads();
-    for (int s = 128; s > 0; s >>= 1) {
-        if (threadIdx.x < s) red[threadIdx.x] += red[threadIdx.x + s];
-        __syncthreads();
-    }
     if (threadIdx.x == 0) {
         double loss = 0.0, bce = 0.0, dice = 0.0, tp = 0.0, ps = 0.0, ts = 0.0;
         float* den = saved + 1 + 4 * n;
@@ -352,7 +420,7 @@
             tvs[0] = (float)tp; tvs[1] = (float)tden; tvs[2] = (float)tv;
             loss += c.logcosh ? log(cosh(1.0 - tv)) : (1.0 - tv);
         }
-        if (pt) loss += (double)c.w_time * red[0] / (double)c.pairs;
+        if (pt) loss += (double)c.w_time * tsum_s / (double)c.pairs;
         saved[0] = (float)loss;
     }
 }
@@ -387,8 +455,9 @@
                                    float a_bce, float a_dice, float smooth, int has_tversky, float tv_alpha, float tv_beta, float tv_smooth,
                                    int logcosh, float w_time, float* saved, biu_stream stream) {
     BIU_REQUIRE(partial && saved && n > 0 && nb > 0 && per_sample > 0 && (!time_partial || (nbt > 0 && n > 1)), BIU_ERR_SHAPE, "seg_loss_finish: bad arguments");
+    BIU_REQUIRE(((uintptr_t)partial & 15) == 0, BIU_ERR_SHAPE, "seg_loss_finish: partial must be 16-byte aligned (rows are read as float4)");
     const SegLossCfg c{a_bce, a_dice, smooth, has_tversky, tv_alpha, tv_beta, tv_smooth, logcosh, w_time, (long long)(n - 1) * per_sample, nbt};
-    hipLaunchKernelGGL(k_seg_loss_finish, dim3(1), dim3(256), 0, (hipStream_t)stream, partial, n, nb, per_sample, time_partial, c, saved);
+    hipLaunchKernelGGL(k_seg_loss_finish, dim3(1), dim3(512), 0, (hipStream_t)stream, partial, n, nb, per_sample, time_partial, c, saved);
     BIU_CHECK_LAUNCH("seg_loss_finish");
     return BIU_OK;
 }
@@ -422,3 +491,22 @@
     BIU_CHECK_LAUNCH("bce_dice_bwd");
     return BIU_OK;
 }
+
+extern "C" int biu_seg_loss_blocks(long long per_sample) { return biu_bce_dice_blocks(per_sample); }
+extern "C" int biu_seg_loss_fwd(const float* logits, const float* target, int n, long long per_sample, int with_time, float* partial,
+                                float* time_partial, biu_stream stream) {
+    BIU_REQUIRE(logits && target && partial && n > 0 && per_sample > 0, BIU_ERR_SHAPE, "seg_loss_fwd: bad arguments");
+    BIU_REQUIRE(!with_time || (n > 1 && time_partial), BIU_ERR_SHAPE, "seg_loss_fwd: the time term needs at least two batch entries and its partial buffer");
+    hipLaunchKernelGGL(k_seg_loss_fwd, dim3(biu_seg_loss_blocks(per_sample)), dim3(256), 0, (hipStream_t)stream, logits, target, (i64)per_sample, n,
+                       with_time ? 1 : 0, partial, time_partial);
+    BIU_CHECK_LAUNCH("seg_loss_fwd");
+    return BIU_OK;
+}
+extern "C" int biu_seg_loss_bwd(const float* logits, const float* target, int n, long long per_sample, const float* coef, const float* time_coef,
+                                float* dlogits, int accumulate, biu_stream stream) {
+    BIU_REQUIRE(logits && target && coef && dlogits && n > 0 && per_sample > 0, BIU_ERR_SHAPE, "seg_loss_bwd: bad arguments");
+    hipLaunchKernelGGL(k_seg_loss_bwd, dim3(grid_for((i64)per_sample, 256, 8192)), dim3(256), 0, (hipStream_t)stream, logits, target, (i64)per_sample, n,
+                       coef, time_coef, dlogits, accumulate);
+    BIU_CHECK_LAUNCH("seg_loss_bwd");
+    return BIU_OK;
+}
diff --git a/bio_image_unet_amd/csrc/biu_internal.h b/bio_image_unet_amd/csrc/biu_internal.h
--- a/bio_image_unet_amd/csrc/biu_internal.h
+++ b/bio_image_unet_amd/csrc/biu_internal.h
@@ -68,6 +68,7 @@
 int biu_mfma_conv_stat_rows(const biu_act* y, int kd, const biu_act* x = nullptr, int dtype = -1, bool red = false, int cin = -1);
 int biu_mfma_conv_bricks(const biu_act* y, int kd, const biu_act* x = nullptr, int dtype = -1, int cin = -1);
 size_t biu_mfma_wgrad_workspace(int cin, int cout, int kd, int kh, int kw, int dtype);
+int biu_mfma_wgrad_form(const biu_act* x, const biu_act* dy, int kd, int dtype);
 bool biu_mfma_wgrad_ok(const biu_act* x, const biu_act* dy, int kd, int kh, int kw, int dilation, int dtype);
 struct BnBwdFuse {
     const biu_act* y;
diff --git a/bio_image_unet_amd/engine.py b/bio_image_unet_amd/engine.py
--- a/bio_image_unet_amd/engine.py
+++ b/bio_image_unet_amd/engine.py
@@ -806,6 +806,7 @@
 
 
 _ACT_CODE = {None: 0, "none": 0, "sigmoid": 1, "tanh": 2, "relu": 3}
+HEAD_DLOGITS_SHORTCUT = True
 
 
 class HeadNode(Node):
@@ -837,7 +838,7 @@
                                _ptr(self.logits), _ptr(self.activated), eng.dtype, _stream()), "head_fwd")
 
     def dlogits(self, eng, g_logits, g_act, a, dst=None, ctot=None, c0=0):
-        if g_act is None and dst is None and g_logits.dtype == torch.float32 and g_logits.is_contiguous():
+        if HEAD_DLOGITS_SHORTCUT and g_act is None and dst is None and g_logits.dtype == torch.float32 and g_logits.is_contiguous():
             return g_logits
         shp = self.out_shape(eng)
         n, spatial = shp[0], 1
@@ -1258,6 +1259,7 @@
                                "engine for that case: this is a bug in the caller of engine.run)")
         eng.load_inputs(xs)
         eng.forward()
+        ctx.set_materialize_grads(False)
         ctx.eng, ctx.out_spec = eng, out_spec
         ctx.generation = eng.generation
         if eng.grad_mode:
diff --git a/bio_image_unet_amd/losses.py b/bio_image_unet_amd/losses.py
--- a/bio_image_unet_amd/losses.py
+++ b/bio_image_unet_amd/losses.py
@@ -45,17 +45,15 @@
         n = targets.size(0)
         per = logits.numel() // n
         st = C.c_void_p(torch.cuda.current_stream().cuda_stream)
-        nb = lib.biu_bce_dice_blocks(per)
-        partial = torch.empty((n, nb, 4), dtype=torch.float32, device=logits.device)
-        check(lib.biu_bce_dice_fwd(C.c_void_p(logits.data_ptr()), C.c_void_p(targets.data_ptr()), n, per,
-                                   C.c_void_p(partial.data_ptr()), st), "bce_dice_fwd")
+        nb = lib.biu_seg_loss_blocks(per)
         sc = _FusedSegLoss._scalars(cfg)
         w_time = sc[8]
-        pt, nbt = None, 0
-        if w_time and n > 1:
-            nbt = lib.biu_pair_smooth_l1_blocks((n - 1) * per)
-            pt = torch.empty(nbt, dtype=torch.float32, device=logits.device)
-            check(lib.biu_pair_smooth_l1_fwd(C.c_void_p(logits.data_ptr()), n, per, C.c_void_p(pt.data_ptr()), st), "pair_smooth_l1_fwd")
+        timed = bool(w_time) and n > 1
+        buf = torch.empty(n * nb * 4 + (nb if timed else 0), dtype=torch.float32, device=logits.device)
+        partial = buf[:n * nb * 4]
+        pt, nbt = (buf[n * nb * 4:], nb) if timed else (None, 0)
+        check(lib.biu_seg_loss_fwd(C.c_void_p(logits.data_ptr()), C.c_void_p(targets.data_ptr()), n, per, 1 if timed else 0,
+                                   C.c_void_p(partial.data_ptr()), C.c_void_p(pt.data_ptr()) if timed else None, st), "seg_loss_fwd")
         saved = torch.empty(1 + 5 * n + 3, dtype=torch.float32, device=logits.device)
         check(lib.biu_seg_loss_finish(C.c_void_p(partial.data_ptr()), n, nb, per, C.c_void_p(pt.data_ptr()) if pt is not None else None, nbt,
                                       *sc, C.c_void_p(saved.data_ptr()), st), "seg_loss_finish")
@@ -81,11 +79,8 @@
         check(lib.biu_seg_loss_coef(C.c_void_p(g.data_ptr()), C.c_void_p(saved.data_ptr()), n, per, *sc, C.c_void_p(coef.data_ptr()),
                                     C.c_void_p(ct.data_ptr()) if ct is not None else None, st), "seg_loss_coef")
         dl = torch.empty_like(logits)
-        check(lib.biu_bce_dice_bwd(C.c_void_p(logits.data_ptr()), C.c_void_p(targets.data_ptr()), n, per,
-                                   C.c_void_p(coef.data_ptr()), C.c_void_p(dl.data_ptr()), 0, st), "bce_dice_bwd")
-        if ct is not None:
-            check(lib.biu_pair_smooth_l1_bwd(C.c_void_p(logits.data_ptr()), n, per, C.c_void_p(ct.data_ptr()), C.c_void_p(dl.data_ptr()), 1, st),
-                  "pair_smooth_l1_bwd")
+        check(lib.biu_seg_loss_bwd(C.c_void_p(logits.data_ptr()), C.c_void_p(targets.data_ptr()), n, per, C.c_void_p(coef.data_ptr()),
+                                   C.c_void_p(ct.data_ptr()) if ct is not None else None, C.c_void_p(dl.data_ptr()), 0, st), "seg_loss_bwd")
         return dl, None, None
 
 
diff --git a/include/biu.h b/include/biu.h
--- a/include/biu.h
+++ b/include/biu.h
@@ -80,6 +80,7 @@
                              int dtype, biu_stream stream);
 
 size_t biu_conv_bwd_weight_workspace(int cin, int cout, int kd, int kh, int kw, int dtype);
+int    biu_conv_bwd_weight_form(const biu_act* x, const biu_act* dy, int kd, int dtype);
 int biu_conv_bwd_weight(const biu_act* x, const biu_xform* xf, const biu_act* dy,
                         int kd, int kh, int kw, int dilation,
                         float* dw, float* dbias, void* ws, size_t ws_bytes, int dtype, biu_stream stream);
@@ -154,6 +155,11 @@
 int biu_seg_loss_coef(const float* g, const float* saved, int n, long long per_sample, float a_bce, float a_dice, float smooth,
                       int has_tversky, float tv_alpha, float tv_beta, float tv_smooth, int logcosh, float w_time, float* coef,
                       float* time_coef, biu_stream stream);
+int biu_seg_loss_blocks(long long per_sample);
+int biu_seg_loss_fwd(const float* logits, const float* target, int n, long long per_sample, int with_time, float* partial,
+                     float* time_partial, biu_stream stream);
+int biu_seg_loss_bwd(const float* logits, const float* target, int n, long long per_sample, const float* coef, const float* time_coef,
+                     float* dlogits, int accumulate, biu_stream stream);
 int biu_head_dlogits(const float* g_logits, const float* g_act, const float* activated, int act, int n, int ch, long long spatial,
                      float* dst, int dst_channels, int dst_c0, biu_stream stream);
 
```
